# insitro/FastVim

Measured on AMD Instinct MI355X. Metric: images/sec FastVim-T 224px bs=128/GPU fwd+bwd (+all-reduce +AdamW +EMA), whole job, higher is better.
Workload: dtype bf16; 1 GPU; FastVim-T 224x224 bs=128/GPU bf16 training step, synthetic ImageNet tensors (BASELINE configs[1]); global_batch=128, parallelism=dp1, hip_graph=True, optimizer_in_step=True, final_loss_hex=0x1.779ca20000000p+0

## Files before the change

### fastvim_amd/_lib.py

```python
import ctypes
import os
import threading

import torch

_PKG = os.path.dirname(os.path.abspath(__file__))
LIB_PATH = os.path.join(_PKG, "libfastvim_hip.so")

FV_F32, FV_BF16, FV_F16 = 0, 1, 2
_DTYPES = {torch.float32: FV_F32, torch.bfloat16: FV_BF16, torch.float16: FV_F16}

_lib = None

C_ABI_SYMBOLS = (
    "fv_last_error", "fv_version",
    "fv_selective_scan_fwd", "fv_selective_scan_bwd_workspace", "fv_selective_scan_bwd",
    "fv_causal_conv1d_fwd", "fv_causal_conv1d_bwd", "fv_scan_expand_skip_fwd",
    "fv_mixer_conv_pool_fwd", "fv_mixer_scan_fwd", "fv_mixer_xproj_scan_fwd_ok", "fv_mixer_xproj_scan_fwd", "fv_mixer_combine_fwd",
    "fv_mixer_bwd_blocks", "fv_mixer_combine_bwd", "fv_mixer_scan_bwd_chunks", "fv_mixer_scan_bwd_chunks_b",
    "fv_mixer_scan_bwd_ckpt_floats", "fv_mixer_scan_bwd_partials", "fv_mixer_scan_bwd", "fv_mixer_scan_bwd_dir", "fv_mixer_scan_bwd_ckpt", "fv_mixer_scan_bwd_segments", "fv_mixer_scan_bwd_seg_floats", "fv_mixer_scan_bwd_seg_partials", "fv_mixer_scan_bwd_seg_chunks", "fv_mixer_scan_bwd_seg", "fv_mixer_scan_fwd_ckpt", "fv_mixer_scan_ckpt_floats", "fv_mixer_scan_fwd_segments", "fv_mixer_scan_fwd_seg_floats", "fv_mixer_scan_fwd_seg", "fv_rows_segment_sum", "fv_rows_gather", "fv_mixer_conv_pool_bwd", "fv_mixer_conv_pool_bwd2_ok", "fv_mixer_conv_pool_bwd2", "fv_mixer_scan_bwd_xproj_ok", "fv_mixer_scan_bwd_xproj", "fv_chunk_rows_bf16", "fv_reduce_partials", "fv_reduce_partials_multi",
    "fv_add_norm_blocks", "fv_add_norm_fwd", "fv_add_norm_bwd", "fv_gemm_bf16", "fv_gemm_bf16_tn_grouped", "fv_gemm_bf16_tn_grouped_ld", "fv_mixer_xproj_fwd", "fv_mixer_xproj_bwd_slices", "fv_mixer_xproj_bwd", "fv_mixer_xproj_bwd2", "fv_mixer_xproj_bwd3_ok", "fv_mixer_xproj_bwd3", "fv_adamw_flat", "fv_soft_target_ce",
    "fv_patch_unfold", "fv_gemm_bf16_rowbias", "fv_mean_pool_fwd", "fv_mean_pool_bwd", "fv_droppath_table", "fv_scale_cast",
    "fv_column_sum", "fv_gemm_bf16_addnorm", "fv_gemm_bf16_dgrad_addnorm_blocks", "fv_gemm_bf16_dgrad_addnorm_bwd", "fv_gemm_bf16_dgrad_addnorm_bwd2", "fv_gemm_bf16_addnorm2", "fv_mixer_combine_out_proj_addnorm_ok", "fv_mixer_combine_out_proj_addnorm", "fv_gemm_f32",
    "fv_mixer_conv_pool_bwd_dgrad_ok", "fv_mixer_conv_pool_bwd_dgrad_blocks", "fv_mixer_conv_pool_bwd_dgrad", "fv_transpose_bf16_batched", "fv_gemm_bf16_tn_grouped_wide8",
    "fv_grad_sumsq_blocks", "fv_grad_sumsq_partials", "fv_adamw_flat_groups",
)


_tls = threading.local()


class _DeviceGuarded:

    def __init__(self, cdll):
        self._cdll = cdll
        self._wrapped = {}

    def __getattr__(self, name):
        w = self._wrapped.get(name)
        if w is None:
            fn = getattr(self._cdll, name)

            def call(*args, _fn=fn):
                dev = getattr(_tls, "dev", None)
                if dev is None or dev == torch.cuda.current_device():
                    return _fn(*args)
                with torch.cuda.device(dev):
                    return _fn(*args)

            w = self._wrapped[name] = call
        return w


def lib():
    global _lib
    if _lib is None:
        if not os.path.exists(LIB_PATH):
            raise RuntimeError(
                f"{LIB_PATH} is missing: build it with `python -m fastvim_amd.build` "
                "(or __graft_entry__.build()). fastvim_amd has no CPU / eager fallback.")
        cdll = ctypes.CDLL(LIB_PATH)
        cdll.fv_last_error.restype = ctypes.c_char_p
        cdll.fv_selective_scan_bwd_workspace.restype = ctypes.c_size_t
        cdll.fv_mixer_scan_bwd_ckpt_floats.restype = ctypes.c_size_t
        cdll.fv_mixer_scan_ckpt_floats.restype = ctypes.c_size_t
        cdll.fv_mixer_scan_fwd_seg_floats.restype = ctypes.c_size_t
        cdll.fv_mixer_scan_bwd_seg_floats.restype = ctypes.c_size_t
        _lib = _DeviceGuarded(cdll)
    return _lib


def dtype_code(dt):
    try:
        return _DTYPES[dt]
    except KeyError:
        raise RuntimeError(f"fastvim_amd: unsupported dtype {dt}") from None


def ptr(t):
    return ctypes.c_void_p(0 if t is None else t.data_ptr())


def stream_of(t):
    _tls.dev = t.device.index
    return ctypes.c_void_p(torch.cuda.current_stream(t.device).cuda_stream)


def require_gpu(*tensors):
    for t in tensors:
        if t is not None and not t.is_cuda:
            raise RuntimeError("fastvim_amd ops run on the GPU only (HIP kernels); got a CPU tensor")


def check(rc, what):
    if rc != 0:
        msg = lib().fv_last_error().decode()
        raise RuntimeError(f"{what}: {msg} (code {rc})")


def i32(v):
    return ctypes.c_int(int(v))
```

### fastvim_amd/csrc/combine_gemm.hip

```cpp
#include "mixer_common.h"
#include "packed.h"

namespace {

typedef __bf16 cg_bf16x8 __attribute__((ext_vector_type(8)));
typedef float cg_f32x4 __attribute__((ext_vector_type(4)));

constexpr int CG_K = 384, CG_N = 192, CG_BM = 64, CG_NT = 256;
constexpr int CG_RSA = CG_K * 2 + 16;
constexpr int CG_RSB = CG_N * 2 + 16;
constexpr int CG_PD = 6;
constexpr int CG_KS = CG_K / 32;
#ifndef CG_DBG
#define CG_DBG 0
#endif

struct CgParams {
  const void* xz;
  const void* skip;
  const float* yc;
  const float *lnw, *lnb;
  void* g;
  float *mean, *rstd_ln;
  float ln_eps;
  Geo geo;
  int B;
  const bf16_t* W;
  long ldw;
  const float* residual;
  const float* nw;
  const float* row_scale;
  int rows_per_scale;
  float* res_out;
  bf16_t* y;
  float* rstd;
  float eps;
  int M;
  int d_in;
};

__device__ __forceinline__ float cg_hsum(f2 v) { return v.x + v.y; }

__global__ __launch_bounds__(CG_NT, 2) void combine_out_proj_addnorm_kernel(CgParams p) {
  extern __shared__ __attribute__((aligned(16))) char smem[];
  typedef PairVec<bf16_t, 3> P;
  const int tid = threadIdx.x, lane = tid & 63;
  const int wv = __builtin_amdgcn_readfirstlane(tid >> 6);
  const Geo g = p.geo;
  const int tiles = (g.rows + 3) / 4;
  const int bimg = blockIdx.x / tiles, i0 = (blockIdx.x - bimg * tiles) * 4;
  const int mimg = bimg * g.L;
  auto tok_of = [&](int rl) {
    const int w = rl >> 4, j = rl & 15;
    return (i0 + w < g.rows && j < g.cols) ? mimg + (i0 + w) * g.s_i + j * g.s_j : -1;
  };

  const int lr = lane % 16, gr = lane / 16;
  const int fn = lane & 15, fk = lane >> 4;
  const bf16_t* wrow[3];
  cg_bf16x8 fb[CG_PD][3];
  float4 ne_r[2][2][3], ne_w[3];
  float ne_sc[2][2];
  {
#pragma clang fp reassociate(off) contract(off)
    const int lc = lane * 6, voff = lc * 2;
    const int tok_x = 2 * CG_K * 2, tok_s = CG_K * 2;
    const bool has_ln = p.lnw != nullptr;
    const float inv_d = 1.f / (float)p.d_in;
    const size_t ydir = (size_t)p.B * g.rows * CG_K;
    const __amdgpu_buffer_rsrc_t bz = fv_make_buf((const bf16_t*)p.xz + CG_K, (size_t)p.M * tok_x - tok_s);
    const __amdgpu_buffer_rsrc_t bs = fv_make_buf(p.skip, (size_t)p.M * tok_s);
    const __amdgpu_buffer_rsrc_t bg = fv_make_buf(p.g, (size_t)p.M * tok_s);
    const __amdgpu_buffer_rsrc_t bmean = fv_make_buf(has_ln ? (const void*)p.mean : p.g, has_ln ? (size_t)p.M * 4 : 0);
    const __amdgpu_buffer_rsrc_t brstd = fv_make_buf(has_ln ? (const void*)p.rstd_ln : p.g, has_ln ? (size_t)p.M * 4 : 0);
    const int irow = i0 + wv;
    const bool wlive = irow < g.rows;
    const int irc = wlive ? irow : g.rows - 1;
    const int mbase = mimg + irc * g.s_i;
    char* arow = smem + (wv * 16) * CG_RSA + lane * 12;
    constexpr int TT = 2;
    const int npair = (g.cols + TT - 1) / TT;
    f2 ysum[3], ysf[3], ysb[3];
    {
      const float* yr = p.yc + ((size_t)bimg * g.rows + irc) * CG_K + lc;
#pragma unroll
      for (int q = 0; q < 3; ++q) {
        ysf[q] = *reinterpret_cast<const f2*>(yr + 2 * q);
        ysb[q] = *reinterpret_cast<const f2*>(yr + ydir + 2 * q);
      }
    }
    struct Pre { P sk[TT], z[TT]; };
    Pre pa, pb;
    auto fetch = [&](Pre& r, int j0) {
#pragma unroll
      for (int t = 0; t < TT; ++t) {
        const int m = mbase + min(j0 + t, g.cols - 1) * g.s_j;
        r.sk[t].load(bs, voff, m * tok_s);
        r.z[t].load(bz, voff, m * tok_x);
      }
    };
    fetch(pa, 0);
    fetch(pb, TT);
    __builtin_amdgcn_sched_barrier(0);
    f2 lw[3], lb[3];
    {
      const float* lwp = has_ln ? p.lnw : p.yc;
      const float* lbp = has_ln ? p.lnb : p.yc;
#pragma unroll
      for (int q = 0; q < 3; ++q) {
        lw[q] = *reinterpret_cast<const f2*>(lwp + lc + 2 * q);
        lb[q] = *reinterpret_cast<const f2*>(lbp + lc + 2 * q);
      }
    }
    __builtin_amdgcn_sched_barrier(0);
#pragma unroll
    for (int nb = 0; nb < 3; ++nb) wrow[nb] = p.W + (long)(wv * 48 + nb * 16 + fn) * p.ldw + fk * 8;
#pragma unroll
    for (int s = 0; s < CG_PD; s += 2)
#pragma unroll
      for (int nb = 0; nb < 3; ++nb)
#pragma unroll
        for (int h = 0; h < 2; ++h) fb[s + h][nb] = *reinterpret_cast<const cg_bf16x8*>(wrow[nb] + (s + h) * 32);
    __builtin_amdgcn_sched_barrier(0);
#pragma unroll
    for (int q = 0; q < 3; ++q) ysum[q] = ysf[q] + ysb[q];
    auto process = [&](Pre& r, int j0) {
      f2 o[TT][3], z[TT][3];
      float s1[TT], mean[TT], rstd[TT];
#pragma unroll
      for (int t = 0; t < TT; ++t)
#pragma unroll
        for (int q = 0; q < 3; ++q) {
          o[t][q] = r.sk[t].get(q);
          z[t][q] = r.z[t].get(q);
        }
      fetch(r, j0 + 2 * TT);
      __builtin_amdgcn_sched_barrier(0);
#pragma unroll
      for (int t = 0; t < TT; ++t) {
        f2 acc = splat(0.f);
#pragma unroll
        for (int q = 0; q < 3; ++q) {
          o[t][q] = (ysum[q] + o[t][q]) * 0.5f;
          acc += o[t][q];
        }
        s1[t] = cg_hsum(acc);
      }
      if (has_ln) {
#pragma unroll
        for (int t = 0; t < TT; ++t) s1[t] = wave_sum_uniform(s1[t]);
#pragma unroll
        for (int t = 0; t < TT; ++t) {
          mean[t] = s1[t] * inv_d;
          f2 acc = splat(0.f);
#pragma unroll
          for (int q = 0; q < 3; ++q) {
            const f2 d = o[t][q] - mean[t];
            acc = fma2(d, d, acc);
          }
          s1[t] = cg_hsum(acc);
        }
#pragma unroll
        for (int t = 0; t < TT; ++t) s1[t] = wave_sum_uniform(s1[t]);
#pragma unroll
        for (int t = 0; t < TT; ++t) rstd[t] = rsqrtf(s1[t] * inv_d + p.ln_eps);
      } else {
#pragma unroll
        for (int t = 0; t < TT; ++t) { mean[t] = 0.f; rstd[t] = 1.f; }
      }
#pragma unroll
      for (int t = 0; t < TT; ++t) {
        const bool live = wlive && j0 + t < g.cols;
        const int m = mbase + min(j0 + t, g.cols - 1) * g.s_j;
        f2 out[3];
#pragma unroll
        for (int q = 0; q < 3; ++q) {
          const f2 w_ = has_ln ? lw[q] : splat(1.f), b_ = has_ln ? lb[q] : splat(0.f);
          out[q] = fma2((o[t][q] - mean[t]) * rstd[t], w_, b_) * silu2(z[t][q]);
        }
        uint32_t pk[3];
#pragma unroll
        for (int q = 0; q < 3; ++q) pk[q] = live ? pack_bf16x2(out[q].x, out[q].y) : 0u;
        if (CG_DBG != 4) {
          fv_buf_store_words<3>(bg, live ? voff : 0x7ffffff0, m * tok_s, pk);
          const int so = (has_ln && live && lane == 0) ? 0 : 0x7ffffff0;
          const uint32_t mv[1] = {__float_as_uint(mean[t])}, rv[1] = {__float_as_uint(rstd[t])};
          fv_buf_store_words<1>(bmean, so, m * 4, mv);
          fv_buf_store_words<1>(brstd, so, m * 4, rv);
        }
        uint32_t* ar = reinterpret_cast<uint32_t*>(arow + (j0 + t) * CG_RSA);
        ar[0] = pk[0]; ar[1] = pk[1]; ar[2] = pk[2];
      }
    };
#pragma unroll 1
    for (int pr = 0; pr < (CG_DBG == 1 ? 0 : 8); pr += 2) {
      process(pa, pr * TT);
      process(pb, (pr + 1) * TT);
    }
    (void)npair;
#pragma unroll
    for (int it = 0; it < 2; ++it)
#pragma unroll
      for (int u = 0; u < 2; ++u) {
        const int m = tok_of(wv * 16 + it * 8 + u * 4 + gr), rowc = m >= 0 ? m : mimg;
#pragma unroll
        for (int k = 0; k < 3; ++k)
          ne_r[it][u][k] = *reinterpret_cast<const float4*>(p.residual + (size_t)rowc * CG_N + (k * 16 + lr) * 4);
        ne_sc[it][u] = (p.row_scale ? p.row_scale : p.nw)[p.row_scale ? rowc / p.rows_per_scale : 0];
      }
#pragma unroll
    for (int k = 0; k < 3; ++k) ne_w[k] = *reinterpret_cast<const float4*>(p.nw + (k * 16 + lr) * 4);
    __builtin_amdgcn_sched_barrier(0);
  }
  __syncthreads();

  cg_f32x4 acc[3][4];
#pragma unroll
  for (int a = 0; a < 3; ++a)
#pragma unroll
    for (int b = 0; b < 4; ++b) acc[a][b] = (cg_f32x4){0.f, 0.f, 0.f, 0.f};
  const char* afrag = smem + (lane & 15) * CG_RSA + (lane >> 4) * 16;
  static_assert(CG_PD % 2 == 0 && CG_KS % 2 == 0, "the weight ring is refilled in line pairs");
#pragma unroll
  for (int kp = 0; kp < (CG_DBG == 2 ? 0 : CG_KS); kp += 2) {
    cg_bf16x8 cur[2][3];
#pragma unroll
    for (int h = 0; h < 2; ++h)
#pragma unroll
      for (int nb = 0; nb < 3; ++nb) cur[h][nb] = fb[(kp + h) % CG_PD][nb];
    if (kp + CG_PD < CG_KS) {
#pragma unroll
      for (int nb = 0; nb < 3; ++nb)
#pragma unroll
        for (int h = 0; h < 2; ++h)
          fb[(kp + h) % CG_PD][nb] = *reinterpret_cast<const cg_bf16x8*>(wrow[nb] + (kp + h + CG_PD) * 32);
    }
    __builtin_amdgcn_sched_barrier(0);
#pragma unroll
    for (int h = 0; h < 2; ++h) {
      cg_bf16x8 fa[4];
#pragma unroll
      for (int mb = 0; mb < 4; ++mb) fa[mb] = *reinterpret_cast<const cg_bf16x8*>(afrag + mb * 16 * CG_RSA + (kp + h) * 64);
#pragma unroll
      for (int a = 0; a < 3; ++a)
#pragma unroll
        for (int b = 0; b < 4; ++b) acc[a][b] = __builtin_amdgcn_mfma_f32_16x16x32_bf16(cur[h][a], fa[b], acc[a][b], 0, 0, 0);
    }
    __builtin_amdgcn_sched_barrier(0);
  }
  __syncthreads();

#pragma unroll
  for (int b = 0; b < 4; ++b)
#pragma unroll
    for (int a = 0; a < 3; ++a) {
      const cg_f32x4 v = acc[a][b];
      uint2 pk = {pack_bf16x2(v[0], v[1]), pack_bf16x2(v[2], v[3])};
      *reinterpret_cast<uint2*>(smem + (b * 16 + (lane & 15)) * CG_RSB + (wv * 48 + a * 16 + (lane >> 4) * 4) * 2) = pk;
    }
  __syncthreads();
  if (CG_DBG == 3) return;
  constexpr int LPR = 16, RPW = 4, RU = 2, RW = CG_BM / 4;
  const float inv_n = 1.f / (float)CG_N;
  float w[3][4];
#pragma unroll
  for (int k = 0; k < 3; ++k) {
    const float4 t = ne_w[k];
    w[k][0] = t.x; w[k][1] = t.y; w[k][2] = t.z; w[k][3] = t.w;
  }
#pragma unroll
  for (int it = 0; it < RW / (RPW * RU); ++it) {
    float v[RU][3][4], r[RU][3][4], sc_u[RU];
#pragma unroll
    for (int u = 0; u < RU; ++u) {
      const int rl = wv * RW + it * (RPW * RU) + u * RPW + gr;
      sc_u[u] = p.row_scale ? ne_sc[it][u] : 1.f;
#pragma unroll
      for (int k = 0; k < 3; ++k) {
        const int c = (k * LPR + lr) * 4;
        const uint2 xb = *reinterpret_cast<const uint2*>(smem + rl * CG_RSB + c * 2);
        v[u][k][0] = __uint_as_float(xb.x << 16); v[u][k][1] = __uint_as_float(xb.x & 0xffff0000u);
        v[u][k][2] = __uint_as_float(xb.y << 16); v[u][k][3] = __uint_as_float(xb.y & 0xffff0000u);
        const float4 t = ne_r[it][u][k];
        r[u][k][0] = t.x; r[u][k][1] = t.y; r[u][k][2] = t.z; r[u][k][3] = t.w;
      }
    }
#pragma unroll
    for (int u = 0; u < RU; ++u) {
      const int row = tok_of(wv * RW + it * (RPW * RU) + u * RPW + gr);
      const bool live = row >= 0;
      const size_t base = (size_t)(live ? row : mimg) * CG_N;
      const float sc = sc_u[u];
#pragma unroll
      for (int k = 0; k < 3; ++k) {
        const int c = (k * LPR + lr) * 4;
#pragma unroll
        for (int e = 0; e < 4; ++e) v[u][k][e] = fmaf(v[u][k][e], sc, r[u][k][e]);
        if (live) *reinterpret_cast<float4*>(p.res_out + base + c) = make_float4(v[u][k][0], v[u][k][1], v[u][k][2], v[u][k][3]);
      }
      float q = 0.f;
#pragma unroll
      for (int k = 0; k < 3; ++k)
#pragma unroll
        for (int e = 0; e < 4; ++e) q = fmaf(v[u][k][e], v[u][k][e], q);
#define FV_DPP_ADD(ctrl) q += __int_as_float(__builtin_amdgcn_update_dpp(0, __float_as_int(q), ctrl, 0xf, 0xf, true))
      FV_DPP_ADD(0xB1);
      FV_DPP_ADD(0x4E);
      FV_DPP_ADD(0x141);
      FV_DPP_ADD(0x140);
#undef FV_DPP_ADD
      const float rstd = rsqrtf(q * inv_n + p.eps);
      if (lr == 0 && live) p.rstd[row] = rstd;
#pragma unroll
      for (int k = 0; k < 3; ++k) {
        const int c = (k * LPR + lr) * 4;
        float o[4];
#pragma unroll
        for (int e = 0; e < 4; ++e) {
          float t = v[u][k][e] * rstd;
          asm volatile("" : "+v"(t));
          o[e] = t * w[k][e];
        }
        uint2 pk = {pack_bf16x2(o[0], o[1]), pack_bf16x2(o[2], o[3])};
        if (live) *reinterpret_cast<uint2*>(p.y + base + c) = pk;
      }
    }
  }
}

}

extern "C" int fv_mixer_combine_out_proj_addnorm_ok(int batch, int rows, int cols, int tokens_per_patch, int d_inner,
                                                    int d_model, int dtype) {
  return dtype == FV_BF16 && d_inner == CG_K && d_model == CG_N && tokens_per_patch == 1 && batch > 0 && rows > 0 &&
         cols > 0 && cols <= 16 && (long)batch * rows * cols * CG_K * 4 < 0x7fffffffL;
}

extern "C" int fv_mixer_combine_out_proj_addnorm(const void* xz, const void* skip, const float* yc, const float* ln_w,
                                                 const float* ln_b, float ln_eps, void* g, float* mean, float* rstd_ln,
                                                 int batch, int rows, int cols, int tok_stride_row, int tok_stride_col,
                                                 const void* W, long ldw, const float* residual,
                                                 const float* norm_weight, const float* row_scale, int rows_per_scale,
                                                 void* y, float* residual_out, float* rstd, float eps,
                                                 fv_stream_t stream) {
  FV_CHECK(xz && skip && yc && g && W && residual && norm_weight && y && residual_out && rstd,
           "mixer_combine_out_proj_addnorm: null pointer");
  FV_CHECK(!ln_w || (ln_b && mean && rstd_ln), "mixer_combine_out_proj_addnorm: LayerNorm needs weight, bias, mean, rstd");
  FV_CHECK(fv_mixer_combine_out_proj_addnorm_ok(batch, rows, cols, 1, CG_K, CG_N, FV_BF16),
           "mixer_combine_out_proj_addnorm: shape not built (fv_mixer_combine_out_proj_addnorm_ok)");
  FV_CHECK((tok_stride_row == cols && tok_stride_col == 1) || (tok_stride_row == 1 && tok_stride_col == rows),
           "mixer_combine_out_proj_addnorm: token strides (%d,%d) are neither row-major nor transposed for a %dx%d grid",
           tok_stride_row, tok_stride_col, rows, cols);
  FV_CHECK(((uintptr_t)W & 15) == 0 && ldw % 8 == 0 && ldw >= CG_K, "mixer_combine_out_proj_addnorm: weight rows must be 16-byte aligned");
  FV_CHECK(((uintptr_t)residual & 15) == 0 && ((uintptr_t)residual_out & 15) == 0 && ((uintptr_t)y & 7) == 0 &&
               ((uintptr_t)norm_weight & 15) == 0, "mixer_combine_out_proj_addnorm: row operands must be 16-byte aligned");
  FV_CHECK(!row_scale || rows_per_scale > 0, "mixer_combine_out_proj_addnorm: rows_per_scale must be positive");
  CgParams p{};
  p.xz = xz; p.skip = skip; p.yc = yc; p.lnw = ln_w; p.lnb = ln_b; p.g = g; p.mean = mean; p.rstd_ln = rstd_ln;
  p.ln_eps = ln_eps;
  p.geo = make_geo(rows, cols, tok_stride_row, tok_stride_col, 1);
  p.B = batch;
  p.W = (const bf16_t*)W; p.ldw = ldw; p.residual = residual; p.nw = norm_weight; p.row_scale = row_scale;
  p.rows_per_scale = rows_per_scale; p.res_out = residual_out; p.y = (bf16_t*)y; p.rstd = rstd; p.eps = eps;
  p.M = batch * rows * cols;
  p.d_in = CG_K;
  const size_t smem = (size_t)CG_BM * CG_RSA;
  hipLaunchKernelGGL(combine_out_proj_addnorm_kernel, dim3(batch * fv_cdiv(rows, 4)), dim3(CG_NT), smem, (hipStream_t)stream, p);
  FV_LAUNCH_CHECK();
  return FV_OK;
}
```

### fastvim_amd/csrc/convpool_dgrad.hip

```cpp
#include "mixer_common.h"
#include "packed.h"
#include "gemm_tiles.h"

namespace {

constexpr int CD_DI = 384, CD_N = 192, CD_K = 2 * CD_DI, CD_BM = 64, CD_NT = 256, CD_NCH = CD_DI / 128;
constexpr int CD_RSA = CD_DI * 2 + 16;
constexpr int CD_RSB = CD_N * 2 + 16;
#ifndef CD_PDEPTH
#define CD_PDEPTH 4
#endif
#ifndef CD_SB_EVERY
#define CD_SB_EVERY 1
#endif
#ifndef CD_W2_PIPE
#define CD_W2_PIPE 1
#endif
constexpr int CD_PD = CD_PDEPTH;
constexpr int CD_KS = CD_K / 32;
constexpr int CD_ZST = CD_BM * BK * 2;
constexpr int CD_NZ = CD_DI / BK;
constexpr int CD_O_RING = CD_BM * CD_RSA;
constexpr int CD_SLOT = 12 * 128;
constexpr int CD_O_B = (CD_BM * CD_RSB + 255) / 256 * 256, CD_O_S = CD_O_B + 2 * 128 * BK * 2;
constexpr int CD_SMEM = CD_O_S + 4 * 32 * (64 * 2 + 16);
static_assert(CD_O_RING + 3 * CD_ZST <= CD_SMEM && CD_O_RING + 4 * CD_SLOT * 4 <= CD_SMEM, "LDS regions");
static_assert(2 * CD_SMEM <= 160 * 1024, "two workgroups per CU");
#ifndef CD_DBG
#define CD_DBG 0
#endif

struct CdParams {
  const void* xz;
  const void* dob;
  const float* dxc;
  const void* dxc2;
  const float *wf, *bf, *wb, *bb, *Df, *Db;
  void* dxz;
  float* part;
  float pool_scale;
  Geo geo;
  int B;
  const bf16_t* Wt;
  long ldwt;
  const float* dres_out;
  const float* r;
  const float* rstd;
  const float* nw;
  const float* row_scale;
  int rows_per_scale;
  bf16_t* dx;
  float* dres_in;
  float* pw;
  const bf16_t* W2;
  long ldw2;
  bf16_t* C2;
  int N2;
  int M;
};

__device__ __forceinline__ void cd_dma16(const void* base, uint32_t voff, uint32_t lds_dst) {
  asm volatile("s_mov_b32 m0, %2\n\ts_nop 0\n\tglobal_load_lds_dwordx4 %0, %1" ::"v"(voff), "s"(base), "s"(lds_dst) : "memory");
}

constexpr int cd_younger(int t) {
  constexpr int KX = CD_DI / 32;
  int n = 0;
  for (int q = KX + 2 * (t - 3) + 2; q < KX + 2 * t; q += 2) n += (q + CD_PD < CD_KS ? 6 : 0) + ((q - KX) / 2 + 3 < CD_NZ ? 2 : 0);
  return n;
}
static_assert(cd_younger(3) < 64 && cd_younger(4) < 64 && cd_younger(5) < 64, "vmcnt is a 6-bit counter");

template <int NT, bool X2>
__global__ __launch_bounds__(CD_NT, 2) void conv_pool_bwd_dgrad_kernel(CdParams p) {
  extern __shared__ __attribute__((aligned(16))) char smem[];
  typedef PairVec<bf16_t, 1> P;
  const int tid = threadIdx.x, lane = tid & 63;
  const int wv = __builtin_amdgcn_readfirstlane(tid >> 6);
  const Geo g = p.geo;
  const int tiles = (g.rows + 3) / 4;
  const int bimg = blockIdx.x / tiles, i0 = (blockIdx.x - bimg * tiles) * 4;
  const int mimg = bimg * g.L;
  auto tok_of = [&](int rl) {
    const int w = rl >> 4, j = rl & 15;
    return (i0 + w < g.rows && j < g.cols) ? mimg + (i0 + w) * g.s_i + j * g.s_j : -1;
  };
  const int irow = i0 + wv;
  const bool wlive = irow < g.rows;
  char* prow = smem + (wv * 16) * CD_RSA;

  {
    const int zr0 = wlive ? NT : 0;
    for (int e = lane; e < (16 - zr0) * (CD_RSA / 4); e += 64) reinterpret_cast<uint32_t*>(prow + zr0 * CD_RSA)[e] = 0u;
    const int tok_x = 2 * CD_DI * 2, tok_d = CD_DI * 2;
    const size_t dstride = (size_t)p.B * g.rows * CD_DI;
    const __amdgpu_buffer_rsrc_t bp = fv_make_buf(p.dxc, 2 * dstride * 4);
    const __amdgpu_buffer_rsrc_t bp2 = fv_make_buf(X2 ? p.dxc2 : p.dxc, X2 ? 2 * dstride * 2 : 0);
    const int irc = wlive ? irow : 0;
    const bool up = irc > 0, down = irc + 1 < g.rows;
    const int m_row = irc * g.s_i, s_up = up ? -g.s_i : 0, s_dn = down ? g.s_i : 0;
    const int pooled_off = (bimg * g.rows + irc) * CD_DI;
    const size_t img_x = (size_t)bimg * g.L * 2 * CD_DI, img_d = (size_t)bimg * g.L * CD_DI;
    const __amdgpu_buffer_rsrc_t bx = fv_make_buf((const bf16_t*)p.xz + img_x, wlive ? (size_t)g.L * tok_x : 0);
    const __amdgpu_buffer_rsrc_t bd = fv_make_buf((const bf16_t*)p.dob + img_d, wlive ? (size_t)g.L * tok_d : 0);
    const __amdgpu_buffer_rsrc_t bo = fv_make_buf((bf16_t*)p.dxz + img_x, wlive ? (size_t)g.L * tok_x : 0);
    struct Pooled {
      f2 a;
      P b;
      __device__ __forceinline__ f2 sum() const { if constexpr (X2) return a + b.get(0); else return a; }
    };
    auto pooled = [&](int r, bool backward, int c0, bool on) {
      const bool ok = r == 1 || (r == 0 ? up : down);
      uint32_t w[2];
      const int eoff = pooled_off + (ok ? (r - 1) * CD_DI : 0) + (backward ? (int)dstride : 0);
      const int lane_off = on ? c0 : 0x1ffffff0;
      fv_buf_load_words<2>(bp, lane_off * 4, eoff * 4, w);
      Pooled o;
      o.a.x = __uint_as_float(w[0]);
      o.a.y = __uint_as_float(w[1]);
      if constexpr (X2) o.b.load(bp2, lane_off * 2, eoff * 2);
      return o;
    };
    P xr[NT + 6], dr[NT + 6];
    auto fetch = [&](int k, int voff) {
      const int di = k < 3 ? -1 : (k >= NT + 3 ? 1 : 0);
      const int j = k - 3 - di * NT;
      const int m = m_row + (di < 0 ? s_up : di > 0 ? s_dn : 0) + j * g.s_j;
      xr[k].load(bx, voff, m * tok_x);
      dr[k].load(bd, voff, m * tok_d);
    };
    struct Prm { f2 wf[CW], wb[CW], bf, bb, Df, Db; };
    auto load_prm = [&](int c0) {
      Prm q;
      load_taps2(p.wf, c0, q.wf);
      load_taps2(p.wb, c0, q.wb);
      q.bf = load_f2(p.bf ? p.bf : p.wf, c0);
      q.bb = load_f2(p.bb ? p.bb : p.wf, c0);
      q.Df = load_f2(p.Df ? p.Df : p.wf, c0);
      q.Db = load_f2(p.Db ? p.Db : p.wf, c0);
      return q;
    };
    Prm pn = load_prm(lane * 2);
    __builtin_amdgcn_sched_barrier(0);
    Pooled cf_mid_raw = pooled(1, false, lane * 2, true), cb_mid_raw = pooled(1, true, lane * 2, true);
    Pooled cb_up_raw = pooled(0, true, lane * 2, true);
    __builtin_amdgcn_sched_barrier(0);
#pragma unroll
    for (int k = 0; k < NT + 6; ++k) fetch(k, lane * 4);
    __builtin_amdgcn_sched_barrier(0);
    Pooled cf_dn_raw = pooled(2, false, lane * 2, true);
    __builtin_amdgcn_sched_barrier(0);
    float* slot = reinterpret_cast<float*>(smem + CD_O_RING) + wv * CD_SLOT;
#pragma unroll 1
    for (int c = 0; c < CD_NCH; ++c) {
      const int c0 = c * 128 + lane * 2;
      const int voff = c0 * 2;
      const bool more = c + 1 < CD_NCH;
      const int c0n = c0 + 128, voffn = more ? voff + 256 : 0x3ffffff0;
      f2 a_wf[CW], a_wb[CW], a_bf = splat(0.f), a_bb = splat(0.f), a_Df = splat(0.f), a_Db = splat(0.f);
#pragma unroll
      for (int k = 0; k < CW; ++k) a_wf[k] = a_wb[k] = splat(0.f);
      if (wlive && CD_DBG != 1) {
        f2 wf[CW], wb[CW];
#pragma unroll
        for (int k = 0; k < CW; ++k) { wf[k] = pn.wf[k]; wb[k] = pn.wb[k]; }
        const f2 bf = pn.bf * (p.bf ? 1.f : 0.f), bb = pn.bb * (p.bb ? 1.f : 0.f);
        const f2 Dfh = pn.Df * (p.Df ? 0.5f : 0.f), Dbh = pn.Db * (p.Db ? 0.5f : 0.f);
        const f2 cf_mid = cf_mid_raw.sum() * p.pool_scale, cb_mid = cb_mid_raw.sum() * p.pool_scale;
        cf_mid_raw = pooled(1, false, c0n, more);
        cb_mid_raw = pooled(1, true, c0n, more);
        const f2 cb_up = cb_up_raw.sum() * (up ? p.pool_scale : 0.f);
        f2 cf_dn = splat(0.f);
        f2 x[NT + 6], dov[NT + 6], dpf[NT + 6], dpb[NT + 6];
        const float m_up = up ? 1.f : 0.f, m_dn = down ? 1.f : 0.f;
#pragma unroll
        for (int k = 0; k < 3; ++k) {
          x[k] = xr[k].get(0) * m_up;
          dov[k] = dr[k].get(0);
          dpf[k] = dpb[k] = splat(0.f);
          fetch(k, voffn);
        }
        if (more) pn = load_prm(c0n);
#pragma unroll
        for (int n = -3; n < NT; ++n) {
          const int q3 = n + 3, k0 = n + 3, k3 = n + 6;
          x[k3] = xr[k3].get(0);
          if (q3 >= NT) x[k3] *= m_dn;
          dov[k3] = dr[k3].get(0);
          fetch(k3, voffn);
          f2 pf = bf, pb = bb;
#pragma unroll
          for (int k = 0; k < CW; ++k) {
            pf = fma2(wf[k], x[k0 + k], pf);
            pb = fma2(wb[k], x[k3 - k], pb);
          }
          const f2 sgf = sigmoid2(pf), sgb = sigmoid2(pb);
          const f2 dsf = sgf * fma2(pf, 1.f - sgf, splat(1.f)), dsb = sgb * fma2(pb, 1.f - sgb, splat(1.f));
          const float e3 = q3 < NT ? 1.f : m_dn, e0 = n >= 0 ? 1.f : m_up;
          if (q3 == NT) cf_dn = cf_dn_raw.sum() * (down ? p.pool_scale : 0.f);
          const f2 nf = fma2(Dfh, dov[k3], q3 >= NT ? cf_dn : cf_mid) * dsf * e3;
          const f2 nb = fma2(Dbh, dov[k0], n < 0 ? cb_up : cb_mid) * dsb * e0;
          if (n == -1) cb_up_raw = pooled(0, true, c0n, more);
          dpf[k3] = nf;
          dpb[k0] = nb;
          if (q3 < NT) {
#pragma unroll
            for (int k = 0; k < CW; ++k) a_wf[k] = fma2(nf, x[k0 + k], a_wf[k]);
            a_bf += nf;
            a_Df = fma2(dov[k3], pf * sgf, a_Df);
          }
          if (n >= 0) {
#pragma unroll
            for (int k = 0; k < CW; ++k) a_wb[k] = fma2(nb, x[k3 - k], a_wb[k]);
            a_bb += nb;
            a_Db = fma2(dov[k0], pb * sgb, a_Db);
            f2 dx = splat(0.f);
#pragma unroll
            for (int k = 0; k < CW; ++k) {
              dx = fma2(wf[k], dpf[k3 - k], dx);
              dx = fma2(wb[k], dpb[k0 - 3 + k], dx);
            }
            const uint32_t pk[1] = {pack_bf16x2(dx.x, dx.y)};
            fv_buf_store_words<1>(bo, voff, (m_row + n * g.s_j) * tok_x, pk);
            *reinterpret_cast<uint32_t*>(prow + n * CD_RSA + voff) = pk[0];
          }
          if ((n + 3) % CD_SB_EVERY == CD_SB_EVERY - 1) __builtin_amdgcn_sched_barrier(0);
        }
        cf_dn_raw = pooled(2, false, c0n, more);
      }
      {
        const f2 hDf = a_Df * 0.5f, hDb = a_Db * 0.5f;
        float4* s4 = reinterpret_cast<float4*>(slot);
        s4[2 * lane] = make_float4(a_wf[0].x, a_wf[1].x, a_wf[2].x, a_wf[3].x);
        s4[2 * lane + 1] = make_float4(a_wf[0].y, a_wf[1].y, a_wf[2].y, a_wf[3].y);
        s4[128 + 2 * lane] = make_float4(a_wb[0].x, a_wb[1].x, a_wb[2].x, a_wb[3].x);
        s4[128 + 2 * lane + 1] = make_float4(a_wb[0].y, a_wb[1].y, a_wb[2].y, a_wb[3].y);
        f2* s2 = reinterpret_cast<f2*>(slot + 1024);
        s2[lane] = a_bf;
        s2[64 + lane] = a_bb;
        s2[128 + lane] = hDf;
        s2[192 + lane] = hDb;
      }
      __syncthreads();
      {
        const float* s0 = reinterpret_cast<const float*>(smem + CD_O_RING);
        float* dst = p.part + (size_t)blockIdx.x * 12 * CD_DI;
#pragma unroll
        for (int i = 0; i < CD_SLOT / CD_NT; ++i) {
          const int e = tid + i * CD_NT;
          const float v = ((s0[e] + s0[CD_SLOT + e]) + s0[2 * CD_SLOT + e]) + s0[3 * CD_SLOT + e];
          int gi;
          if (e < 512) gi = c * 512 + e;
          else if (e < 1024) gi = 4 * CD_DI + c * 512 + (e - 512);
          else {
            const int q = (e - 1024) >> 7, rr = (e - 1024) & 127;
            gi = (8 + q) * CD_DI + c * 128 + rr;
          }
          dst[gi] = v;
        }
      }
      __syncthreads();
    }
  }

  const int fn = lane & 15, fk = lane >> 4, lr = lane % 16, gr = lane / 16;
  const bf16_t* wrow[3];
  bf16x8 fb[CD_PD][3];
#pragma unroll
  for (int nb = 0; nb < 3; ++nb) wrow[nb] = p.Wt + (long)(wv * 48 + nb * 16 + fn) * p.ldwt + fk * 8;
  uint32_t zoff[2];
  const uint32_t ring = (uint32_t)(uintptr_t)(__attribute__((address_space(3))) const char*)(smem + CD_O_RING);
#pragma unroll
  for (int i = 0; i < 2; ++i) {
    const int e = tid + i * CD_NT, rrow = e >> 3, ch = (e & 7) ^ (rrow & 7);
    const int m = tok_of(rrow);
    zoff[i] = (uint32_t)((m >= 0 ? m : mimg) * (CD_K * 2) + (CD_DI + ch * 8) * 2);
  }
  auto issue_z = [&](int t) {
#pragma unroll
    for (int i = 0; i < 2; ++i)
      cd_dma16(p.dxz, zoff[i] + (uint32_t)t * (BK * 2), ring + (uint32_t)(t % 3) * CD_ZST + (uint32_t)(i * CD_NT + wv * 64) * 16);
  };
  issue_z(0);
  issue_z(1);
  issue_z(2);
#pragma unroll
  for (int s = 0; s < CD_PD; s += 2)
#pragma unroll
    for (int nb = 0; nb < 3; ++nb)
#pragma unroll
      for (int h = 0; h < 2; ++h) fb[s + h][nb] = *reinterpret_cast<const bf16x8*>(wrow[nb] + (s + h) * 32);
  __builtin_amdgcn_sched_barrier(0);
  float4 ne_r[2][2][3];
#pragma unroll
  for (int it = 0; it < 2; ++it)
#pragma unroll
    for (int u = 0; u < 2; ++u) {
      const int m = tok_of(wv * 16 + it * 8 + u * 4 + gr), rowc = m >= 0 ? m : mimg;
#pragma unroll
      for (int k = 0; k < 3; ++k) ne_r[it][u][k] = *reinterpret_cast<const float4*>(p.r + (size_t)rowc * CD_N + (k * 16 + lr) * 4);
    }
  __builtin_amdgcn_sched_barrier(0);
  __syncthreads();

  f32x4 acc[3][4];
#pragma unroll
  for (int a = 0; a < 3; ++a)
#pragma unroll
    for (int b = 0; b < 4; ++b) acc[a][b] = (f32x4){0.f, 0.f, 0.f, 0.f};
  const char* afrag = smem + (lane & 15) * CD_RSA + (lane >> 4) * 16;
  static_assert(CD_PD % 2 == 0 && CD_KS % 2 == 0, "the weight ring is refilled in line pairs");
  static_for<(CD_DBG == 2 ? 0 : CD_KS / 2)>([&](auto kp_c) {
    constexpr int kp = 2 * decltype(kp_c)::value;
    constexpr int KX = CD_DI / 32;
    if constexpr (kp >= KX) {
      constexpr int t = (kp - KX) / 2;
      if constexpr (t >= 3) asm volatile("s_waitcnt vmcnt(%0)" ::"n"(cd_younger(t)) : "memory");
      if (t >= 3 || kp == KX) __builtin_amdgcn_s_barrier();
    }
    bf16x8 cur[2][3];
#pragma unroll
    for (int h = 0; h < 2; ++h)
#pragma unroll
      for (int nb = 0; nb < 3; ++nb) cur[h][nb] = fb[(kp + h) % CD_PD][nb];
    if constexpr (kp + CD_PD < CD_KS) {
#pragma unroll
      for (int nb = 0; nb < 3; ++nb)
#pragma unroll
        for (int h = 0; h < 2; ++h)
          fb[(kp + h) % CD_PD][nb] = *reinterpret_cast<const bf16x8*>(wrow[nb] + (kp + h + CD_PD) * 32);
    }
    __builtin_amdgcn_sched_barrier(0);
#pragma unroll
    for (int h = 0; h < 2; ++h) {
      bf16x8 fa[4];
      if constexpr (kp < KX) {
#pragma unroll
        for (int mb = 0; mb < 4; ++mb) fa[mb] = *reinterpret_cast<const bf16x8*>(afrag + mb * 16 * CD_RSA + (kp + h) * 64);
      } else {
        constexpr int t = (kp - KX) / 2;
        const char* st = smem + CD_O_RING + (t % 3) * CD_ZST;
#pragma unroll
        for (int mb = 0; mb < 4; ++mb) fa[mb] = frag<KC, CD_BM>(st, mb, h, lane);
      }
#pragma unroll
      for (int a = 0; a < 3; ++a)
#pragma unroll
        for (int b = 0; b < 4; ++b) acc[a][b] = __builtin_amdgcn_mfma_f32_16x16x32_bf16(cur[h][a], fa[b], acc[a][b], 0, 0, 0);
    }
    if constexpr (kp >= KX) {
      constexpr int t = (kp - KX) / 2;
      if constexpr (t + 3 < CD_NZ) {
        __builtin_amdgcn_s_barrier();
        issue_z(t + 3);
      }
    }
    __builtin_amdgcn_sched_barrier(0);
  });
  float4 ne_g[2][2][3];
#pragma unroll
  for (int it = 0; it < 2; ++it)
#pragma unroll
    for (int u = 0; u < 2; ++u) {
      const int m = tok_of(wv * 16 + it * 8 + u * 4 + gr), rowc = m >= 0 ? m : mimg;
#pragma unroll
      for (int k = 0; k < 3; ++k)
        ne_g[it][u][k] = p.dres_out ? *reinterpret_cast<const float4*>(p.dres_out + (size_t)rowc * CD_N + (k * 16 + lr) * 4)
                                    : make_float4(0.f, 0.f, 0.f, 0.f);
    }
  __syncthreads();

#pragma unroll
  for (int b = 0; b < 4; ++b)
#pragma unroll
    for (int a = 0; a < 3; ++a) {
      const f32x4 v = acc[a][b];
      uint2 pk = {pack_bf16x2(v[0], v[1]), pack_bf16x2(v[2], v[3])};
      *reinterpret_cast<uint2*>(smem + (b * 16 + (lane & 15)) * CD_RSB + (wv * 48 + a * 16 + (lane >> 4) * 4) * 2) = pk;
    }
  __syncthreads();
  if (CD_DBG == 3) return;
  {
    constexpr int LPR = 16, RPW = 4, RU = 2, RW = CD_BM / 4;
    const float inv_n = 1.f / (float)CD_N;
    float w[3][4], aw[3][4];
#pragma unroll
    for (int k = 0; k < 3; ++k) {
      const float4 t = *reinterpret_cast<const float4*>(p.nw + (k * LPR + lr) * 4);
      w[k][0] = t.x; w[k][1] = t.y; w[k][2] = t.z; w[k][3] = t.w;
#pragma unroll
      for (int e = 0; e < 4; ++e) aw[k][e] = 0.f;
    }
#pragma unroll
    for (int it = 0; it < RW / (RPW * RU); ++it) {
#pragma unroll
      for (int u = 0; u < RU; ++u) {
        const int rl = wv * RW + it * (RPW * RU) + u * RPW + gr;
        const int row = tok_of(rl);
        const bool live = row >= 0;
        const int rowc = live ? row : mimg;
        const size_t base = (size_t)rowc * CD_N;
        const float rstd = p.rstd[rowc];
        const float sc = p.row_scale ? p.row_scale[rowc / p.rows_per_scale] : 1.f;
        const float lv = live ? 1.f : 0.f;
        float xh[3][4], dxh[3][4];
        float c2 = 0.f;
#pragma unroll
        for (int k = 0; k < 3; ++k) {
          const int c = (k * LPR + lr) * 4;
          const uint2 xb = *reinterpret_cast<const uint2*>(smem + rl * CD_RSB + c * 2);
          const float dyv[4] = {__uint_as_float(xb.x << 16), __uint_as_float(xb.x & 0xffff0000u),
                                __uint_as_float(xb.y << 16), __uint_as_float(xb.y & 0xffff0000u)};
          const float4 rr4 = ne_r[it][u][k];
          const float rr[4] = {rr4.x, rr4.y, rr4.z, rr4.w};
#pragma unroll
          for (int e = 0; e < 4; ++e) {
            const float dyl = dyv[e] * lv;
            xh[k][e] = (rr[e] - 0.f) * rstd;
            dxh[k][e] = dyl * w[k][e];
            aw[k][e] = fmaf(dyl, xh[k][e], aw[k][e]);
            c2 = fmaf(dxh[k][e], xh[k][e], c2);
          }
        }
#define FV_DPP_ADD(ctrl) c2 += __int_as_float(__builtin_amdgcn_update_dpp(0, __float_as_int(c2), ctrl, 0xf, 0xf, true))
        FV_DPP_ADD(0xB1);
        FV_DPP_ADD(0x4E);
        FV_DPP_ADD(0x141);
        FV_DPP_ADD(0x140);
#undef FV_DPP_ADD
        c2 = c2 * inv_n;
        const float c1 = 0.f;
#pragma unroll
        for (int k = 0; k < 3; ++k) {
          const int c = (k * LPR + lr) * 4;
          const float4 g4 = ne_g[it][u][k];
          const float gg[4] = {g4.x, g4.y, g4.z, g4.w};
          float dr[4];
#pragma unroll
          for (int e = 0; e < 4; ++e) dr[e] = rstd * (dxh[k][e] - c1 - xh[k][e] * c2) + gg[e];
          if (live) {
            *reinterpret_cast<float4*>(p.dres_in + base + c) = make_float4(dr[0], dr[1], dr[2], dr[3]);
            if (p.row_scale)
#pragma unroll
              for (int e = 0; e < 4; ++e) dr[e] *= sc;
            uint2 pk = {pack_bf16x2(dr[0], dr[1]), pack_bf16x2(dr[2], dr[3])};
            *reinterpret_cast<uint2*>(p.dx + base + c) = pk;
            *reinterpret_cast<uint2*>(smem + rl * CD_RSB + c * 2) = pk;
          } else {
            *reinterpret_cast<uint2*>(smem + rl * CD_RSB + c * 2) = make_uint2(0u, 0u);
          }
        }
      }
    }
    __syncthreads();
    float* s_acc = reinterpret_cast<float*>(smem + CD_BM * CD_RSB);
#pragma unroll
    for (int k = 0; k < 3; ++k)
#pragma unroll
      for (int e = 0; e < 4; ++e) {
        float v = aw[k][e];
        auto r1 = __builtin_amdgcn_permlane16_swap(__float_as_uint(v), __float_as_uint(v), false, false);
        v = __uint_as_float(r1[0]) + __uint_as_float(r1[1]);
        auto r2 = __builtin_amdgcn_permlane32_swap(__float_as_uint(v), __float_as_uint(v), false, false);
        v = __uint_as_float(r2[0]) + __uint_as_float(r2[1]);
        if (gr == 0) s_acc[wv * CD_N + (k * LPR + lr) * 4 + e] = v;
      }
    __syncthreads();
    float* dst = p.pw + (size_t)blockIdx.x * CD_N;
    for (int c = tid; c < CD_N; c += CD_NT) dst[c] = (s_acc[c] + s_acc[CD_N + c]) + (s_acc[2 * CD_N + c] + s_acc[3 * CD_N + c]);
  }
  if (p.W2 && CD_DBG != 4) {
    __syncthreads();
    tile_times_w2_rows<CD_BM, CD_RSB, KS, decltype(tok_of), CD_W2_PIPE != 0>(smem, smem + CD_O_B, smem + CD_O_S, p.W2, p.ldw2, p.N2,
                                                                              p.C2, tok_of, tid);
  }
}

}

extern "C" int fv_mixer_conv_pool_bwd_dgrad_ok(int batch, int rows, int cols, int tokens_per_patch, int d_inner, int d_model,
                                               int pool_max, int dtype) {
  return dtype == FV_BF16 && d_inner == CD_DI && d_model == CD_N && tokens_per_patch == 1 && !pool_max && batch > 0 &&
         rows > 0 && (cols == 14 || cols == 16) &&
         (long)batch * rows * cols * CD_K * 2 < 0x7fffffffL &&
         (long)batch * rows * CD_DI * 8 < 0x7ffff000L;
}

extern "C" int fv_mixer_conv_pool_bwd_dgrad_blocks(int batch, int rows) { return batch * fv_cdiv(rows, 4); }

extern "C" int fv_mixer_conv_pool_bwd_dgrad(
    const void* xz, const void* dskip, const float* dxc, const void* dxc2, const float* conv_w, const float* conv_b,
    const float* conv_w_b, const float* conv_b_b, const float* D, const float* D_b, void* dxz, float* conv_partials, int batch,
    int rows, int cols, int tok_stride_row, int tok_stride_col, float scaling, const void* W_in_t, long ldwt,
    const float* dresidual_out, const float* r, const float* rstd, const float* norm_weight, const float* row_scale,
    int rows_per_scale, void* dx, float* dresidual_in, float* partial_dw, const void* W2, void* C2, int N2, long ldw2,
    fv_stream_t stream) {
  FV_CHECK(xz && dskip && dxc && conv_w && conv_w_b && dxz && conv_partials && W_in_t && r && rstd && norm_weight && dx &&
               dresidual_in && partial_dw, "mixer_conv_pool_bwd_dgrad: null pointer");
  FV_CHECK(fv_mixer_conv_pool_bwd_dgrad_ok(batch, rows, cols, 1, CD_DI, CD_N, 0, FV_BF16),
           "mixer_conv_pool_bwd_dgrad: shape not built (fv_mixer_conv_pool_bwd_dgrad_ok)");
  FV_CHECK((tok_stride_row == cols && tok_stride_col == 1) || (tok_stride_row == 1 && tok_stride_col == rows),
           "mixer_conv_pool_bwd_dgrad: token strides (%d,%d) are neither row-major nor transposed for a %dx%d grid",
           tok_stride_row, tok_stride_col, rows, cols);
  FV_CHECK(((uintptr_t)W_in_t & 15) == 0 && ldwt % 8 == 0 && ldwt >= CD_K, "mixer_conv_pool_bwd_dgrad: transposed weight rows must be 16-byte aligned");
  FV_CHECK(((uintptr_t)r & 15) == 0 && ((uintptr_t)dresidual_in & 15) == 0 && ((uintptr_t)dx & 7) == 0 &&
               ((uintptr_t)norm_weight & 15) == 0 && ((uintptr_t)dresidual_out & 15) == 0 && ((uintptr_t)dxz & 15) == 0,
           "mixer_conv_pool_bwd_dgrad: row operands must be 16-byte aligned");
  FV_CHECK(!row_scale || rows_per_scale > 0, "mixer_conv_pool_bwd_dgrad: rows_per_scale must be positive");
  FV_CHECK(!W2 || (C2 && N2 > 0 && N2 % 128 == 0 && ldw2 % 8 == 0 && ldw2 >= N2 && ((uintptr_t)W2 & 15) == 0 && ((uintptr_t)C2 & 15) == 0),
           "mixer_conv_pool_bwd_dgrad: the second weight must be (192, N2) with N2 a multiple of 128, 16-byte aligned");
  CdParams p{};
  p.xz = xz; p.dob = dskip; p.dxc = dxc; p.dxc2 = dxc2; p.wf = conv_w; p.bf = conv_b; p.wb = conv_w_b; p.bb = conv_b_b;
  p.Df = D; p.Db = D_b; p.dxz = dxz; p.part = conv_partials;
  p.pool_scale = scaling / (float)cols;
  p.geo = make_geo(rows, cols, tok_stride_row, tok_stride_col, 1);
  p.B = batch;
  p.Wt = (const bf16_t*)W_in_t; p.ldwt = ldwt; p.dres_out = dresidual_out; p.r = r; p.rstd = rstd; p.nw = norm_weight;
  p.row_scale = row_scale; p.rows_per_scale = rows_per_scale > 0 ? rows_per_scale : 1; p.dx = (bf16_t*)dx;
  p.dres_in = dresidual_in; p.pw = partial_dw; p.W2 = (const bf16_t*)W2; p.ldw2 = ldw2; p.C2 = (bf16_t*)C2; p.N2 = N2;
  p.M = batch * rows * cols;
  const dim3 grid(batch * fv_cdiv(rows, 4)), block(CD_NT);
#define FV_CD(NTT, XX)                                                                                              \
  do {                                                                                                              \
    static FvOncePerDevice done;                                                                                    \
    if (done.first())                                                                                               \
      (void)hipFuncSetAttribute((const void*)conv_pool_bwd_dgrad_kernel<NTT, XX>, hipFuncAttributeMaxDynamicSharedMemorySize, CD_SMEM); \
    hipLaunchKernelGGL((conv_pool_bwd_dgrad_kernel<NTT, XX>), grid, block, CD_SMEM, (hipStream_t)stream, p);        \
  } while (0)
  if (cols == 14) { if (dxc2) FV_CD(14, true); else FV_CD(14, false); }
  else { if (dxc2) FV_CD(16, true); else FV_CD(16, false); }
#undef FV_CD
  FV_LAUNCH_CHECK();
  return FV_OK;
}
```

### fastvim_amd/csrc/glue.hip

```cpp
#include "common.h"

namespace {

typedef uint32_t u32x4 __attribute__((ext_vector_type(4)));
typedef uint32_t u32x2 __attribute__((ext_vector_type(2)));

template <typename T> struct Vec4;
template <> struct Vec4<float> {
  static __device__ __forceinline__ void ld(const float* p, float (&v)[4]) {
    const float4 t = *reinterpret_cast<const float4*>(p);
    v[0] = t.x; v[1] = t.y; v[2] = t.z; v[3] = t.w;
  }
  static __device__ __forceinline__ void st(float* p, const float (&v)[4]) {
    *reinterpret_cast<float4*>(p) = make_float4(v[0], v[1], v[2], v[3]);
  }
};
template <> struct Vec4<bf16_t> {
  static __device__ __forceinline__ void ld(const bf16_t* p, float (&v)[4]) {
    const u32x2 t = *reinterpret_cast<const u32x2*>(p);
    v[0] = __uint_as_float(t.x << 16); v[1] = __uint_as_float(t.x & 0xffff0000u);
    v[2] = __uint_as_float(t.y << 16); v[3] = __uint_as_float(t.y & 0xffff0000u);
  }
  static __device__ __forceinline__ void st(bf16_t* p, const float (&v)[4]) {
    u32x2 t;
    t.x = pack_bf16x2(v[0], v[1]);
    t.y = pack_bf16x2(v[2], v[3]);
    *reinterpret_cast<u32x2*>(p) = t;
  }
};

constexpr int UNF_GJ = 16;

template <typename TI, typename TO>
__global__ __launch_bounds__(256) void patch_unfold_kernel(const TI* __restrict__ img, TO* __restrict__ out, int C, int H,
                                                           int W, int ph, int pw, int gw) {
  extern __shared__ __attribute__((aligned(16))) char smem[];
  TO* tile = reinterpret_cast<TO*>(smem);
  const int gj0 = blockIdx.x * UNF_GJ, gi = blockIdx.y, b = blockIdx.z;
  const int gjn = min(UNF_GJ, gw - gj0);
  const int Kp = C * ph * pw;
  const int xv = gjn * pw / 4;
  const TI* src = img + ((size_t)b * C * H + (size_t)gi * ph) * W + (size_t)gj0 * pw;
  for (int e = threadIdx.x; e < C * ph * xv; e += blockDim.x) {
    const int row = e / xv, x = (e - row * xv) * 4;
    const int c = row / ph, pi = row - c * ph;
    float v[4];
    Vec4<TI>::ld(src + ((size_t)c * H + pi) * W + x, v);
    const int gj = x / pw, pj = x - gj * pw;
    Vec4<TO>::st(tile + (size_t)gj * Kp + row * pw + pj, v);
  }
  __syncthreads();
  TO* dst = out + (((size_t)b * gridDim.y + gi) * gw + gj0) * Kp;
  constexpr int EV = 16 / sizeof(TO);
  const int nv = gjn * Kp / EV;
  for (int e = threadIdx.x; e < nv; e += blockDim.x)
    reinterpret_cast<u32x4*>(dst)[e] = reinterpret_cast<const u32x4*>(tile)[e];
}

constexpr int MP_WAVES = 16;
template <typename T>
__global__ __launch_bounds__(64 * MP_WAVES) void mean_pool_fwd_kernel(const T* __restrict__ x, T* __restrict__ out, int L, int D, float inv) {
  __shared__ float s_acc[MP_WAVES][256];
  const int lane = threadIdx.x & 63, wv = threadIdx.x >> 6;
  const int d = (blockIdx.x * 64 + lane) * 4, b = blockIdx.y;
  float a[4] = {0.f, 0.f, 0.f, 0.f};
  if (d < D) {
    const T* xp = x + (size_t)b * L * D + d;
    int l = wv;
    for (; l + 3 * MP_WAVES < L; l += 4 * MP_WAVES) {
      float v[4][4];
#pragma unroll
      for (int u = 0; u < 4; ++u) Vec4<T>::ld(xp + (size_t)(l + u * MP_WAVES) * D, v[u]);
#pragma unroll
      for (int u = 0; u < 4; ++u)
#pragma unroll
        for (int k = 0; k < 4; ++k) a[k] += v[u][k];
    }
    for (; l < L; l += MP_WAVES) {
      float v[4];
      Vec4<T>::ld(xp + (size_t)l * D, v);
#pragma unroll
      for (int k = 0; k < 4; ++k) a[k] += v[k];
    }
  }
#pragma unroll
  for (int k = 0; k < 4; ++k) s_acc[wv][lane * 4 + k] = a[k];
  __syncthreads();
  if (wv == 0 && d < D) {
    float r[4];
#pragma unroll
    for (int k = 0; k < 4; ++k) {
      float t = 0.f;
#pragma unroll
      for (int w = 0; w < MP_WAVES; ++w) t += s_acc[w][lane * 4 + k];
      r[k] = t * inv;
    }
    Vec4<T>::st(out + (size_t)b * D + d, r);
  }
}

template <typename T>
__global__ __launch_bounds__(256) void mean_pool_bwd_kernel(const T* __restrict__ g, T* __restrict__ dx, int L, int D,
                                                            int rows_per_block, float inv) {
  const int b = blockIdx.y, dv = D / 4;
  const int l0 = blockIdx.x * rows_per_block, l1 = min(L, l0 + rows_per_block);
  for (int e = threadIdx.x; e < (l1 - l0) * dv; e += blockDim.x) {
    const int l = l0 + e / dv, d = (e % dv) * 4;
    float v[4];
    Vec4<T>::ld(g + (size_t)b * D + d, v);
#pragma unroll
    for (int k = 0; k < 4; ++k) v[k] *= inv;
    Vec4<T>::st(dx + ((size_t)b * L + l) * D + d, v);
  }
}

__global__ __launch_bounds__(256) void droppath_table_kernel(float* __restrict__ table, const float* __restrict__ keep,
                                                             const float* __restrict__ inv, int mods, int batch) {
  const int i = blockIdx.x * blockDim.x + threadIdx.x;
  if (i < mods * batch) {
    const int m = i / batch;
    table[i] = floorf(table[i] + keep[m]) * inv[m];
  }
}

template <typename T>
__global__ __launch_bounds__(256) void scale_cast_kernel(const float* __restrict__ x, const float* __restrict__ scale,
                                                         T* __restrict__ y, size_t n) {
  const float s = scale[0];
  for (size_t i = (size_t)blockIdx.x * blockDim.x + threadIdx.x; i < n; i += (size_t)gridDim.x * blockDim.x)
    io<T>::st(y + i, x[i] * s);
}

template <typename T>
__global__ __launch_bounds__(256) void column_sum_kernel(const T* __restrict__ x, float* __restrict__ out, int rows, int cols,
                                                         int accumulate) {
  __shared__ float s_acc[4][64];
  const int lane = threadIdx.x & 63, wv = threadIdx.x >> 6, c = blockIdx.x * 64 + lane;
  float a = 0.f;
  if (c < cols)
    for (int r = wv; r < rows; r += 4) a += io<T>::ld(x + (size_t)r * cols + c);
  s_acc[wv][lane] = a;
  __syncthreads();
  if (wv == 0 && c < cols) {
    const float t = (s_acc[0][lane] + s_acc[1][lane]) + (s_acc[2][lane] + s_acc[3][lane]);
    out[c] = accumulate ? out[c] + t : t;
  }
}

bool dt_ok(int dt) { return dt == FV_F32 || dt == FV_BF16; }


constexpr int TRJ_MAX = 64;
struct TransposeJobs {
  const uint16_t* src[TRJ_MAX];
  uint16_t* dst[TRJ_MAX];
  int rows, cols;
};
__global__ __launch_bounds__(256) void transpose_bf16_kernel(TransposeJobs J) {
  __shared__ uint16_t t[32][33];
  const uint16_t* src = J.src[blockIdx.z];
  uint16_t* dst = J.dst[blockIdx.z];
  const int r0 = blockIdx.y * 32, c0 = blockIdx.x * 32, tx = threadIdx.x & 31, ty = threadIdx.x >> 5;
#pragma unroll
  for (int i = 0; i < 4; ++i) {
    const int r = r0 + ty + 8 * i, c = c0 + tx;
    t[ty + 8 * i][tx] = (r < J.rows && c < J.cols) ? src[(size_t)r * J.cols + c] : (uint16_t)0;
  }
  __syncthreads();
#pragma unroll
  for (int i = 0; i < 4; ++i) {
    const int c = c0 + ty + 8 * i, r = r0 + tx;
    if (r < J.rows && c < J.cols) dst[(size_t)c * J.rows + r] = t[tx][ty + 8 * i];
  }
}

}

extern "C" int fv_patch_unfold(const void* img, int img_dtype, void* out, int out_dtype, int batch, int chans, int height,
                               int width, int ph, int pw, fv_stream_t stream) {
  FV_CHECK(img && out, "patch_unfold: null pointer");
  FV_CHECK(dt_ok(img_dtype) && dt_ok(out_dtype), "patch_unfold: dtypes must be fp32 or bf16");
  FV_CHECK(batch > 0 && chans > 0 && ph > 0 && pw > 0 && height >= ph && width >= pw, "patch_unfold: empty dimension");
  FV_CHECK(height % ph == 0 && width % pw == 0, "patch_unfold: image %dx%d is not whole %dx%d patches", height, width, ph, pw);
  FV_CHECK(pw % 8 == 0 && ((uintptr_t)img & 15) == 0 && ((uintptr_t)out & 15) == 0,
           "patch_unfold: patch width must be a multiple of 8 and the buffers 16-byte aligned");
  const int gh = height / ph, gw = width / pw;
  const size_t osz = out_dtype == FV_F32 ? 4 : 2;
  const size_t smem = (size_t)UNF_GJ * chans * ph * pw * osz;
  FV_CHECK(smem <= 64 * 1024, "patch_unfold: %d x %d x %d patches do not fit the staging tile", chans, ph, pw);
  FV_CHECK(gh <= 65535 && batch <= 65535, "patch_unfold: grid too large");
  const dim3 grid(fv_cdiv(gw, UNF_GJ), gh, batch), block(256);
  hipStream_t st = (hipStream_t)stream;
#define FV_UNF(TI, TO) hipLaunchKernelGGL((patch_unfold_kernel<TI, TO>), grid, block, smem, st, (const TI*)img, (TO*)out, chans, height, width, ph, pw, gw)
  if (img_dtype == FV_F32 && out_dtype == FV_BF16) FV_UNF(float, bf16_t);
  else if (img_dtype == FV_F32) FV_UNF(float, float);
  else if (out_dtype == FV_BF16) FV_UNF(bf16_t, bf16_t);
  else FV_UNF(bf16_t, float);
#undef FV_UNF
  FV_LAUNCH_CHECK();
  return FV_OK;
}

extern "C" int fv_mean_pool_fwd(const void* x, void* out, int batch, int tokens, int dim, int dtype, fv_stream_t stream) {
  FV_CHECK(x && out, "mean_pool_fwd: null pointer");
  FV_CHECK(dt_ok(dtype), "mean_pool_fwd: dtype must be fp32 or bf16");
  FV_CHECK(batch > 0 && tokens > 0 && dim > 0 && dim % 4 == 0 && batch <= 65535, "mean_pool_fwd: bad shape (%d, %d, %d)", batch, tokens, dim);
  const dim3 grid(fv_cdiv(dim, 256), batch), block(64 * MP_WAVES);
  hipStream_t st = (hipStream_t)stream;
  const float inv = 1.f / (float)tokens;
  if (dtype == FV_F32) hipLaunchKernelGGL(mean_pool_fwd_kernel<float>, grid, block, 0, st, (const float*)x, (float*)out, tokens, dim, inv);
  else hipLaunchKernelGGL(mean_pool_fwd_kernel<bf16_t>, grid, block, 0, st, (const bf16_t*)x, (bf16_t*)out, tokens, dim, inv);
  FV_LAUNCH_CHECK();
  return FV_OK;
}

extern "C" int fv_mean_pool_bwd(const void* g, void* dx, int batch, int tokens, int dim, int dtype, fv_stream_t stream) {
  FV_CHECK(g && dx, "mean_pool_bwd: null pointer");
  FV_CHECK(dt_ok(dtype), "mean_pool_bwd: dtype must be fp32 or bf16");
  FV_CHECK(batch > 0 && tokens > 0 && dim > 0 && dim % 4 == 0 && batch <= 65535, "mean_pool_bwd: bad shape (%d, %d, %d)", batch, tokens, dim);
  const int rpb = fv_cdiv(tokens, 8);
  const dim3 grid(fv_cdiv(tokens, rpb), batch), block(256);
  hipStream_t st = (hipStream_t)stream;
  const float inv = 1.f / (float)tokens;
  if (dtype == FV_F32) hipLaunchKernelGGL(mean_pool_bwd_kernel<float>, grid, block, 0, st, (const float*)g, (float*)dx, tokens, dim, rpb, inv);
  else hipLaunchKernelGGL(mean_pool_bwd_kernel<bf16_t>, grid, block, 0, st, (const bf16_t*)g, (bf16_t*)dx, tokens, dim, rpb, inv);
  FV_LAUNCH_CHECK();
  return FV_OK;
}

extern "C" int fv_droppath_table(float* table, const float* keep, const float* inv_keep, int mods, int batch, fv_stream_t stream) {
  FV_CHECK(table && keep && inv_keep && mods > 0 && batch > 0, "droppath_table: bad arguments");
  hipLaunchKernelGGL(droppath_table_kernel, dim3(fv_cdiv((long)mods * batch, 256)), dim3(256), 0, (hipStream_t)stream, table, keep,
                     inv_keep, mods, batch);
  FV_LAUNCH_CHECK();
  return FV_OK;
}

extern "C" int fv_scale_cast(const float* x, const float* scale, void* y, int y_dtype, size_t n, fv_stream_t stream) {
  FV_CHECK(x && scale && y && n > 0, "scale_cast: bad arguments");
  FV_CHECK(dt_ok(y_dtype), "scale_cast: output must be fp32 or bf16");
  const dim3 grid(fv_cdiv((long)n, 256) < 2048 ? fv_cdiv((long)n, 256) : 2048), block(256);
  hipStream_t st = (hipStream_t)stream;
  if (y_dtype == FV_F32) hipLaunchKernelGGL(scale_cast_kernel<float>, grid, block, 0, st, x, scale, (float*)y, n);
  else hipLaunchKernelGGL(scale_cast_kernel<bf16_t>, grid, block, 0, st, x, scale, (bf16_t*)y, n);
  FV_LAUNCH_CHECK();
  return FV_OK;
}

extern "C" int fv_column_sum(const void* x, int dtype, float* out, int rows, int cols, int accumulate, fv_stream_t stream) {
  FV_CHECK(x && out && rows > 0 && cols > 0, "column_sum: bad arguments");
  FV_CHECK(dt_ok(dtype), "column_sum: input must be fp32 or bf16");
  const dim3 grid(fv_cdiv(cols, 64)), block(256);
  hipStream_t st = (hipStream_t)stream;
  if (dtype == FV_F32) hipLaunchKernelGGL(column_sum_kernel<float>, grid, block, 0, st, (const float*)x, out, rows, cols, accumulate);
  else hipLaunchKernelGGL(column_sum_kernel<bf16_t>, grid, block, 0, st, (const bf16_t*)x, out, rows, cols, accumulate);
  FV_LAUNCH_CHECK();
  return FV_OK;
}

extern "C" int fv_transpose_bf16_batched(const void* const* srcs, void* const* dsts, int njobs, int rows, int cols,
                                         fv_stream_t stream) {
  FV_CHECK(srcs && dsts && njobs > 0 && njobs <= TRJ_MAX, "transpose_bf16_batched: 1..%d jobs", TRJ_MAX);
  FV_CHECK(rows > 0 && cols > 0 && fv_cdiv(rows, 32) <= 65535, "transpose_bf16_batched: bad shape (%d, %d)", rows, cols);
  TransposeJobs J{};
  for (int j = 0; j < njobs; ++j) {
    FV_CHECK(srcs[j] && dsts[j], "transpose_bf16_batched: null pointer in job %d", j);
    J.src[j] = (const uint16_t*)srcs[j];
    J.dst[j] = (uint16_t*)dsts[j];
  }
  J.rows = rows; J.cols = cols;
  hipLaunchKernelGGL(transpose_bf16_kernel, dim3(fv_cdiv(cols, 32), fv_cdiv(rows, 32), njobs), dim3(256), 0, (hipStream_t)stream, J);
  FV_LAUNCH_CHECK();
  return FV_OK;
}
```

### fastvim_amd/flat.py

```python
import ctypes
import os
import re
import warnings

import torch
import torch.distributed as dist

from . import _lib as L
from .layernorm import RMSNorm
from .mamba_simple_faster import Mamba, _GroupedWgrad, _SideStream, flush_wgrads, group_wgrads
from .mixer_ops import defer_reductions, drop_reductions, flush_reductions, pending_reductions

_LAYER_RE = re.compile(r"^((?:.*\.)?[A-Za-z_]*layers\.\d+)\.")

_MIXER_GROUPS = (
    ("conv", ("conv1d.weight", "conv1d_b.weight", "conv1d.bias", "conv1d_b.bias", "D", "D_b")),
    ("scan", ("A_log", "dt_proj.weight", "dt_proj.bias", "A_b_log", "dt_proj_b.weight", "dt_proj_b.bias")),
    ("ln", ("layernorm.weight", "layernorm.bias")),
    ("xproj", ("x_proj.weight", "x_proj_b.weight")),
)


class FlatTrainingState:
    def __init__(self, model, shadow_dtype=torch.bfloat16, process_group=None, comm_dtype=None,
                 chunk_bytes=256 << 20):
        self.group = process_group
        self.comm_dtype = comm_dtype
        self.chunk = max(1, chunk_bytes // 4)
        named = dict(model.named_parameters())
        mixers = {mname: mod for mname, mod in model.named_modules() if isinstance(mod, Mamba)}
        units, unit_of = [], {}
        for n, p in named.items():
            if not p.requires_grad:
                continue
            m_ = _LAYER_RE.match(n)
            key = m_.group(1) if m_ else None
            if key is None:
                if not units or units[-1][0] is not None:
                    units.append((None, []))
                units[-1][1].append(n)
            else:
                if key not in unit_of:
                    unit_of[key] = len(units)
                    units.append((key, []))
                units[unit_of[key]][1].append(n)
        order, regions = [], []
        self.units = []
        for key, names in units:
            front = []
            for mname, mod in mixers.items():
                if key is not None and (mname + ".").startswith(key + "."):
                    for gname, keys in _MIXER_GROUPS:
                        full = [f"{mname}.{k}" if mname else k for k in keys]
                        if all(f in named and named[f].requires_grad for f in full):
                            regions.append((mod, gname, full))
                            front += full
            rest = [n for n in names if n not in set(front)]
            self.units.append((key, len(order), len(order) + len(front) + len(rest)))
            order += front + rest
        if not any(k is not None for k, _ in units):
            for mname, mod in mixers.items():
                for gname, keys in _MIXER_GROUPS:
                    full = [f"{mname}.{k}" if mname else k for k in keys]
                    if all(f in named and named[f].requires_grad for f in full):
                        regions.append((mod, gname, full))
            front = [f for _, _, full in regions for f in full]
            order = front + [n for n in order if n not in set(front)]
            self.units = [(None, 0, len(order))]
        self.names = order
        params = [named[n] for n in order]
        dev = params[0].device
        offs, off = [], 0
        for p in params:
            offs.append(off)
            off += (p.numel() + 7) // 8 * 8
        self.param_flat = torch.zeros(off, device=dev, dtype=torch.float32)
        self.grad_flat = torch.zeros(off, device=dev, dtype=torch.float32)
        self.shadow_flat = torch.zeros(off, device=dev, dtype=shadow_dtype)
        self.offsets = dict(zip(order, offs))
        total = off
        self.unit_ranges = [(key, offs[i0] if i0 < len(offs) else total, offs[i1] if i1 < len(offs) else total)
                            for key, i0, i1 in self.units if i1 > i0]
        with torch.no_grad():
            for n, p, o in zip(order, params, offs):
                k = p.numel()
                self.param_flat[o:o + k].copy_(p.detach().reshape(-1))
                p.data = self.param_flat[o:o + k].view_as(p)
                p.grad = self.grad_flat[o:o + k].view_as(p)
                p._fv_shadow = self.shadow_flat[o:o + k].view_as(p)
                p._fv_shadow_version = -1
        self._params = params
        for mod, gname, full in regions:
            lo = self.offsets[full[0]]
            last = named[full[-1]]
            hi = self.offsets[full[-1]] + last.numel()
            contiguous = all(self.offsets[a] + named[a].numel() == self.offsets[b]
                             for a, b in zip(full[:-1], full[1:]))
            if not contiguous:
                continue
            fv = mod.__dict__.setdefault("_fv", {})
            fv[gname + "_grad"] = self.grad_flat[lo:hi]
            if gname == "xproj":
                shp = (2,) + tuple(named[full[0]].shape)
                fv["Wx2"] = self.param_flat[lo:hi].view(shp)
                fv["Wx2_shadow"] = self.shadow_flat[lo:hi].view(shp)
                fv["Wx2_grad"] = self.grad_flat[lo:hi].view(shp)
        for mod in model.modules():
            if isinstance(mod, (RMSNorm, torch.nn.LayerNorm, torch.nn.Linear, torch.nn.Conv2d)) and getattr(mod, "weight", None) is not None:
                if mod.weight.requires_grad:
                    mod.weight._fv_direct = True
                b = getattr(mod, "bias", None)
                if isinstance(mod, (torch.nn.Linear, torch.nn.Conv2d)) and b is not None and b.requires_grad:
                    b._fv_direct = True
        pe = getattr(model, "pos_embed", None)
        if isinstance(pe, torch.nn.Parameter) and pe.requires_grad:
            pe._fv_direct = True
        self._t_src, self._t_dst, self._t_params = [], [], []
        if shadow_dtype == torch.bfloat16 and dev.type == "cuda":
            for mod in mixers.values():
                w = mod.in_proj.weight
                if tuple(w.shape) == (768, 192) and w.requires_grad and getattr(w, "_fv_shadow", None) is not None:
                    wt = torch.empty(192, 768, device=dev, dtype=shadow_dtype)
                    w._fv_shadow_t = wt
                    w._fv_shadow_t_version = -1
                    self._t_src.append(w._fv_shadow)
                    self._t_dst.append(wt)
                    self._t_params.append(w)
        self._tx_src, self._tx_dst, self._tx_params = [], [], []
        if shadow_dtype == torch.bfloat16 and dev.type == "cuda":
            for mod in mixers.values():
                fv = mod.__dict__.get("_fv", {})
                ws = fv.get("Wx2_shadow")
                if ws is None or ws.dtype != torch.bfloat16:
                    continue
                _, Wd, d_in = ws.shape
                if d_in >= 768 and d_in % 64 == 0 and Wd % 8 == 0:
                    wt = torch.empty(2, d_in, Wd, device=dev, dtype=shadow_dtype)
                    fv["Wx2_shadow_t"] = wt
                    fv["Wx2_t_params"] = (mod.x_proj.weight, mod.x_proj_b.weight)
                    for k in range(2):
                        self._tx_src.append(ws[k])
                        self._tx_dst.append(wt[k])
                    for w in fv["Wx2_t_params"]:
                        w._fv_shadow_t_version = -1
                        self._tx_params.append(w)
        self.refresh_shadow()
        self._hook = model.register_load_state_dict_post_hook(lambda module, incompatible: self.refresh_shadow())
        from .mixer_ops import _Deferred
        self._saved_switches = (_Deferred.enabled, _GroupedWgrad.enabled, _SideStream.enabled)
        defer_reductions(True)
        group_wgrads(True)
        _SideStream.enabled = False

    def close(self):
        if self._saved_switches is None:
            return
        self.finish_backward()
        d, g, s_ = self._saved_switches
        defer_reductions(d)
        group_wgrads(g)
        _SideStream.enabled = s_
        self._hook.remove()
        self._saved_switches = None

    def __enter__(self):
        return self

    def __exit__(self, *exc):
        self.close()
        return False

    def zero_grad(self):
        _SideStream.join()
        n = len(_GroupedWgrad.jobs) + len(_GroupedWgrad.sums) + pending_reductions()
        if n:
            _GroupedWgrad.jobs = []
            _GroupedWgrad.sums = []
            _GroupedWgrad.rows_jobs = []
            drop_reductions()
            warnings.warn(f"FlatTrainingState.zero_grad(): {n} queued gradient jobs of an unfinished backward pass "
                          "were discarded -- call finish_backward() (or allreduce_mean_() / optimizer.step()) after "
                          "loss.backward()", RuntimeWarning, stacklevel=2)
        self.grad_flat.zero_()

    def finish_backward(self):
        flush_wgrads()
        flush_reductions()

    def refresh_shadow(self):
        self.shadow_flat.copy_(self.param_flat)
        for p in self._params:
            p._fv_shadow_version = p._version
        self.refresh_transposed()

    def refresh_transposed(self):
        from .mixer_ops import transpose_bf16_batched
        for src, dst, params in ((self._t_src, self._t_dst, self._t_params),
                                 (getattr(self, "_tx_src", []), getattr(self, "_tx_dst", []), getattr(self, "_tx_params", []))):
            if src:
                transpose_bf16_batched(src, dst)
                for p in params:
                    p._fv_shadow_t_version = p._version

    @property
    def world_size(self):
        return dist.get_world_size(self.group) if dist.is_initialized() else 1

    def buckets(self, n_buckets, taper=True):
        blocks = [(i, u) for i, u in enumerate(self.unit_ranges) if u[0] is not None]
        if not blocks:
            return [{"bounds": (0, self.grad_flat.numel()), "layers": (0, 0)}]
        first_u, last_u = blocks[0][0], blocks[-1][0]
        nb = len(blocks)
        n_buckets = max(1, min(n_buckets, nb))
        sizes = [u[2] - u[1] for _, u in blocks]
        w = [i + 2 if taper else 1 for i in range(n_buckets)]
        cum = [sum(sizes) * sum(w[:i + 1]) / sum(w) for i in range(n_buckets)]
        runs, acc, lo = [], 0, 0
        for j, sz in enumerate(sizes):
            acc += sz
            left = nb - 1 - j
            if (len(runs) < n_buckets - 1 and acc >= cum[len(runs)] - 1e-9 and left >= n_buckets - 1 - len(runs)) \
                    or j == nb - 1:
                runs.append((lo, j + 1))
                lo = j + 1
        out = []
        for k, (a, b) in enumerate(runs):
            e0 = self.unit_ranges[first_u + a][1] if k > 0 else 0
            e1 = self.unit_ranges[first_u + b - 1][2] if k < len(runs) - 1 else self.grad_flat.numel()
            out.append({"bounds": (e0, e1), "layers": (a, b)})
        return out[::-1]

    def make_exchange(self, n_buckets=1):
        from .ddp import GradExchange
        bk = self.buckets(n_buckets)
        self.exchange = GradExchange(self.grad_flat, [b["bounds"] for b in bk], self.group, self.comm_dtype, self.chunk * 4)
        self.exchange.layers = [b["layers"] for b in bk]
        return self.exchange

    def allreduce_mean_(self):
        self._allreduce(True)

    def allreduce_sum_(self):
        self._allreduce(False)

    def _allreduce(self, mean):
        self.finish_backward()
        if self.world_size == 1:
            return
        if getattr(self, "exchange", None) is None:
            self.make_exchange(1)
        self.exchange.allreduce_(mean=mean)


MAX_PARAM_GROUPS = 256


def build_group_map(names, offsets, sizes, total, groups, default_weight_decay=0.0):
    known = set(names)
    rows, table, per_name = {}, [], {}
    ids = torch.zeros(total, dtype=torch.uint8)
    for g in groups:
        key = (float(g.get("lr_scale", 1.0)), float(g.get("weight_decay", default_weight_decay)))
        for n in g["params"]:
            if n not in known:
                raise ValueError(f"param_groups: {n!r} is not a trainable parameter of the flat training state")
            if n in per_name:
                raise ValueError(f"param_groups: parameter {n!r} appears in more than one group")
            if key not in rows:
                if len(table) == MAX_PARAM_GROUPS:
                    raise ValueError(f"param_groups: more than {MAX_PARAM_GROUPS} distinct (lr_scale, weight_decay) pairs "
                                     "(the fused optimizer keeps one group byte per element)")
                rows[key] = len(table)
                table.append(key)
            per_name[n] = key
            ids[offsets[n]:offsets[n] + sizes[n]] = rows[key]
    missing = [n for n in names if n not in per_name]
    if missing:
        raise ValueError(f"param_groups: {len(missing)} trainable parameters of the flat training state are in no group: "
                         f"{missing[:4]} ...")
    return ids, table, per_name


def groups_from_named(per_name):
    out = {}
    for n, (scale, wd) in per_name.items():
        key = (float(scale), float(wd))
        out.setdefault(key, {"lr_scale": key[0], "weight_decay": key[1], "params": []})["params"].append(n)
    return list(out.values())


class FlatAdamW:

    def __init__(self, flat, model, lr=1e-3, betas=(0.9, 0.999), eps=1e-8, weight_decay=0.05, no_decay=(),
                 ema_decay=None, param_groups=None, max_grad_norm=None, skip_nonfinite=False):
        self.flat = flat
        dev = flat.param_flat.device
        n = flat.param_flat.numel()
        self.exp_avg = torch.zeros(n, device=dev, dtype=torch.float32)
        self.exp_avg_sq = torch.zeros(n, device=dev, dtype=torch.float32)
        self.ema = flat.param_flat.clone() if ema_decay is not None else None
        self.ema_decay = float(ema_decay or 0.0)
        no_decay = set(no_decay)
        self.lr = torch.full((1,), float(lr), device=dev, dtype=torch.float32)
        self.step_t = torch.zeros(1, device=dev, dtype=torch.float32)
        self.betas, self.eps, self.weight_decay = betas, eps, weight_decay
        self.skip_nonfinite = bool(skip_nonfinite)
        self._grouped = param_groups is not None or max_grad_norm is not None or self.skip_nonfinite
        self.group_ids = self.group_table = self.max_norm = self.partials = self.stats = None
        self._group_row_of = None
        self.decay_mask = None
        if not self._grouped:
            mask = torch.zeros(n, dtype=torch.uint8)
            named = dict(model.named_parameters())
            for name, off in flat.offsets.items():
                if name not in no_decay:
                    mask[off:off + named[name].numel()] = 1
            self.decay_mask = mask.to(dev)
        else:
            if param_groups is None:
                groups = [{"params": [nm for nm in flat.names if nm not in no_decay], "weight_decay": weight_decay},
                          {"params": [nm for nm in flat.names if nm in no_decay], "weight_decay": 0.0}]
                groups = [g for g in groups if g["params"]]
            else:
                name_of = {id(p): nm for nm, p in zip(flat.names, flat._params)}
                groups = []
                for g in param_groups:
                    names = []
                    for q in g["params"]:
                        nm = q if isinstance(q, str) else name_of.get(id(q))
                        if nm is None:
                            raise ValueError("param_groups: a parameter of a group is not a trainable parameter of the "
                                             "flat training state")
                        names.append(nm)
                    groups.append({**g, "params": names})
            self._group_table_full = torch.zeros(MAX_PARAM_GROUPS, 2, device=dev, dtype=torch.float32)
            self.group_ids = torch.zeros(n, device=dev, dtype=torch.uint8)
            self._set_groups(groups)
            if max_grad_norm is not None or self.skip_nonfinite:
                G = int(L.lib().fv_grad_sumsq_blocks(ctypes.c_size_t(n)))
                self.partials = torch.zeros(G, device=dev, dtype=torch.float32)
                self.stats = torch.zeros(4, device=dev, dtype=torch.float32)
            if max_grad_norm is not None:
                self.max_norm = torch.full((1,), float(max_grad_norm), device=dev, dtype=torch.float32)

    def _set_groups(self, groups):
        f = self.flat
        sizes = {nm: p.numel() for nm, p in zip(f.names, f._params)}
        ids, table, per_name = build_group_map(f.names, f.offsets, sizes, f.param_flat.numel(), groups, self.weight_decay)
        rows = {key: i for i, key in enumerate(table)}
        with torch.no_grad():
            self.group_ids.copy_(ids)
            self._group_table_full.zero_()
            self._group_table_full[:len(table)].copy_(torch.tensor(table, dtype=torch.float32).view(-1, 2))
        self._group_row_of = {nm: rows[key] for nm, key in per_name.items()}
        self.group_table = self._group_table_full[:len(table)]

    def set_lr(self, lr):
        self.lr.fill_(float(lr))

    def set_max_grad_norm(self, v):
        if self.max_norm is None:
            raise RuntimeError("FlatAdamW was built without max_grad_norm")
        self.max_norm.fill_(float(v))

    def last_stats(self):
        if self.stats is None:
            raise RuntimeError("FlatAdamW was built without max_grad_norm / skip_nonfinite: no gradient norm is computed")
        t, c, fin, sk = self.stats.tolist()
        return {"total_norm": t, "clip_coef": c, "finite": bool(fin), "skipped_steps": int(sk)}

    def _named_slices(self, buf):
        f = self.flat
        named = dict(zip(f.names, f._params))
        return {n: buf[o:o + named[n].numel()].view_as(named[n]) for n, o in f.offsets.items()}

    def state_dict(self):
        ea, es = self._named_slices(self.exp_avg), self._named_slices(self.exp_avg_sq)
        return {"state": {n: {"exp_avg": ea[n].detach().clone(), "exp_avg_sq": es[n].detach().clone()} for n in ea},
                "step": float(self.step_t.item()), "lr": float(self.lr.item()), "betas": tuple(self.betas),
                "eps": self.eps, "weight_decay": self.weight_decay, "ema_decay": self.ema_decay,
                "ema": None if self.ema is None else {n: v.detach().clone() for n, v in self._named_slices(self.ema).items()},
                **self._group_state()}

    def _group_state(self):
        if not self._grouped:
            return {"param_groups": None, "max_grad_norm": None, "skipped_steps": 0}
        tab = self.group_table.detach().cpu().double().tolist()
        return {"param_groups": {nm: tuple(tab[r]) for nm, r in self._group_row_of.items()},
                "max_grad_norm": None if self.max_norm is None else float(self.max_norm.item()),
                "skipped_steps": 0 if self.stats is None else int(self.stats[3].item())}

    def _load_group_state(self, sd):
        if not self._grouped:
            if sd.get("param_groups") is not None or sd.get("max_grad_norm") is not None:
                raise ValueError("FlatAdamW.load_state_dict: the state was saved by an optimizer with param_groups / "
                                 "max_grad_norm, this one was built without them -- pass them to the constructor")
            return
        if sd.get("max_grad_norm") is not None and self.max_norm is None:
            raise ValueError("FlatAdamW.load_state_dict: the state carries max_grad_norm, this optimizer was built without it")
        if sd.get("param_groups") is not None:
            self._set_groups(groups_from_named(sd["param_groups"]))
        if self.max_norm is not None and sd.get("max_grad_norm") is not None:
            self.max_norm.fill_(float(sd["max_grad_norm"]))
        if self.stats is not None and "skipped_steps" in sd:
            self.stats[3].fill_(float(sd["skipped_steps"]))

    def load_state_dict(self, sd):
        ea, es = self._named_slices(self.exp_avg), self._named_slices(self.exp_avg_sq)
        missing = set(ea) - set(sd["state"])
        if missing:
            raise KeyError(f"FlatAdamW.load_state_dict: no state for {sorted(missing)[:4]} ...")
        with torch.no_grad():
            for n in ea:
                ea[n].copy_(sd["state"][n]["exp_avg"])
                es[n].copy_(sd["state"][n]["exp_avg_sq"])
            self.step_t.fill_(float(sd["step"]))
            self.lr.fill_(float(sd["lr"]))
            if self.ema is not None and sd.get("ema") is not None:
                for n, v in self._named_slices(self.ema).items():
                    v.copy_(sd["ema"][n])
        self.betas, self.eps, self.weight_decay = tuple(sd["betas"]), sd["eps"], sd["weight_decay"]
        self._load_group_state(sd)

    def ema_state_dict(self, prefix=""):
        if self.ema is None:
            raise RuntimeError("FlatAdamW was built without ema_decay")
        return {prefix + n: v.detach().clone() for n, v in self._named_slices(self.ema).items()}

    def step(self, grad_scale=1.0):
        f = self.flat
        f.finish_backward()
        if self._grouped:
            return self._step_groups(grad_scale)
        rc = L.lib().fv_adamw_flat(
            L.ptr(f.param_flat), L.ptr(f.grad_flat), L.ptr(self.exp_avg), L.ptr(self.exp_avg_sq), L.ptr(self.ema),
            L.ptr(f.shadow_flat), L.ptr(self.decay_mask), L.ptr(self.lr), L.ptr(self.step_t),
            ctypes.c_float(self.betas[0]), ctypes.c_float(self.betas[1]), ctypes.c_float(self.eps),
            ctypes.c_float(self.weight_decay), ctypes.c_float(self.ema_decay), ctypes.c_float(grad_scale),
            ctypes.c_size_t(f.param_flat.numel()), L.stream_of(f.param_flat))
        L.check(rc, "adamw_flat")
        f.refresh_transposed()

    def _step_groups(self, grad_scale):
        f = self.flat
        n = f.param_flat.numel()
        st = L.stream_of(f.param_flat)
        if self.partials is not None:
            rc = L.lib().fv_grad_sumsq_partials(L.ptr(f.grad_flat), L.ptr(self.partials), ctypes.c_size_t(n), st)
            L.check(rc, "grad_sumsq_partials")
        rc = L.lib().fv_adamw_flat_groups(
            L.ptr(f.param_flat), L.ptr(f.grad_flat), L.ptr(self.exp_avg), L.ptr(self.exp_avg_sq), L.ptr(self.ema),
            L.ptr(f.shadow_flat), L.ptr(self.group_ids), L.ptr(self._group_table_full), L.i32(MAX_PARAM_GROUPS),
            L.ptr(self.lr), L.ptr(self.step_t), L.ptr(self.partials),
            L.i32(0 if self.partials is None else self.partials.numel()), L.ptr(self.max_norm), L.ptr(self.stats),
            L.i32(self.skip_nonfinite), ctypes.c_float(self.betas[0]), ctypes.c_float(self.betas[1]),
            ctypes.c_float(self.eps), ctypes.c_float(self.ema_decay), ctypes.c_float(grad_scale), ctypes.c_size_t(n), st)
        L.check(rc, "adamw_flat_groups")
        f.refresh_transposed()


def save_checkpoint(path, model, opt, prefix="backbone.", **extra):
    ck = {"state_dict": {prefix + k: v.detach().clone() for k, v in model.state_dict().items()},
          "optimizer_states": [opt.state_dict()], **extra}
    if opt.ema is not None:
        ck["state_dict_ema"] = opt.ema_state_dict("")
    torch.save(ck, path)
    return ck


def load_checkpoint(path_or_dict, model, opt=None, prefix="backbone.", use_ema=False):
    ck = torch.load(path_or_dict, map_location="cpu", weights_only=False) if isinstance(path_or_dict, (str, os.PathLike)) else path_or_dict
    sd = ck["state_dict_ema"] if (use_ema and "state_dict_ema" in ck) else ck["state_dict"]
    model.load_state_dict({(k[len(prefix):] if prefix and k.startswith(prefix) else k): v for k, v in sd.items()}, strict=True)
    if opt is not None:
        opt.load_state_dict(ck["optimizer_states"][0])
    return ck
```

### fastvim_amd/mamba_simple_faster.py

```python
import ctypes
import math

import torch
import torch.nn as nn
import torch.nn.functional as F

from . import _lib as L
from . import mixer_ops as M
from .gemm import gemm_any_bnn, gemm_any_btn, gemm_any_nn, gemm_any_nt, gemm_any_tn, gemm_nn, gemm_nt, gemm_tn


def _shadow(w, cdt):
    sh = getattr(w, "_fv_shadow", None)
    if sh is not None and sh.dtype == cdt:
        if w._version != w._fv_shadow_version:
            with torch.no_grad():
                sh.copy_(w)
            w._fv_shadow_version = w._version
        return sh
    return w.to(cdt)


def _shadow_t(w, cdt):
    wt = getattr(w, "_fv_shadow_t", None)
    if wt is not None and wt.dtype == cdt:
        if w._version != w._fv_shadow_t_version:
            with torch.no_grad():
                wt.copy_(_shadow(w, cdt).t())
            w._fv_shadow_t_version = w._version
        return wt
    return _shadow(w, cdt).t().contiguous()


def _wx2_shadow_t(fv):
    if fv is None:
        return None
    wt = fv.get("Wx2_shadow_t")
    if wt is None:
        return None
    params = fv["Wx2_t_params"]
    if any(w._version != w._fv_shadow_t_version for w in params):
        with torch.no_grad():
            for k, w in enumerate(params):
                wt[k].copy_(_shadow(w, wt.dtype).t())
                w._fv_shadow_t_version = w._version
    return wt


def _direct_grad(w):
    g = w.grad
    if getattr(w, "_fv_direct", False) and g is not None and g.is_contiguous() and g.dtype == torch.float32:
        return g
    return None


def _wgrad(X, Y, W=None, splits=16):
    M_, I = X.shape
    J = Y.shape[1]
    while splits > 1 and (M_ % splits or M_ // splits < 256):
        splits //= 2
    part = gemm_any_tn(X, Y, splits)
    g = _direct_grad(W) if W is not None else None
    if g is not None:
        M.reduce_partials(part, splits, out=g.view(-1), accumulate=True)
        return None
    return M.reduce_partials(part, splits)


def _mfma_ok(*ts):
    return all(t.dtype == torch.bfloat16 and t.stride(-1) == 1 and t.data_ptr() % 16 == 0 for t in ts)


def _any_ok(*ts):
    return all(t.is_cuda and t.dtype in (torch.float32, torch.bfloat16) and t.dim() == 2 for t in ts)


def linear_fwd(a2, w_c, bias=None):
    if _mfma_ok(a2, w_c) and a2.shape[1] % 8 == 0 and w_c.shape[0] % 8 == 0:
        return gemm_nt(a2, w_c, bias=None if bias is None else bias.float())
    if _any_ok(a2, w_c):
        return gemm_any_nt(a2, w_c, bias)
    return F.linear(a2, w_c, None if bias is None else bias.to(a2.dtype))


def linear_dgrad(g2, w_c):
    if _mfma_ok(g2, w_c) and w_c.shape[1] % 8 == 0 and g2.shape[1] % 8 == 0:
        return gemm_nn(g2, w_c)
    if _any_ok(g2, w_c):
        return gemm_any_nn(g2, w_c)
    return g2 @ w_c


class _SideStream:
    enabled = False
    stream = None
    pending = []

    @classmethod
    def run(cls, fn, *keep):
        if not cls.enabled:
            return fn()
        cur = torch.cuda.current_stream()
        if cls.stream is None:
            cls.stream = torch.cuda.Stream()
        cls.stream.wait_stream(cur)
        with torch.cuda.stream(cls.stream):
            out = fn()
        cls.pending.append(keep)
        return out

    @classmethod
    def join(cls):
        if cls.stream is not None and cls.pending:
            torch.cuda.current_stream().wait_stream(cls.stream)
        cls.pending = []


XPROJ_IN_SCAN = True


class _GroupedWgrad:
    enabled = False
    jobs = []
    chunk = 0

    @classmethod
    def add(cls, g2, a2, out):
        from .gemm import grouped_splits
        if any(j[2].data_ptr() == out.data_ptr() for j in cls.jobs):
            cls.flush()
        cls.jobs.append((g2, a2, out, grouped_splits(g2.shape[0], M=g2.shape[1], N=a2.shape[1])))
        if cls.chunk and len(cls.jobs) >= cls.chunk:
            cls.flush()

    sums = []
    rows_jobs = []

    @classmethod
    def flush(cls):
        if cls.rows_jobs:
            rj, cls.rows_jobs = cls.rows_jobs, []
            M.chunk_rows_bf16(rj)
        if cls.jobs:
            from .gemm import gemm_tn_grouped
            jobs, cls.jobs = cls.jobs, []
            if _SideStream.enabled:
                cls.sums += _SideStream.run(lambda: gemm_tn_grouped(jobs, reduce=False), jobs)
            else:
                gemm_tn_grouped(jobs)

    @classmethod
    def reduce(cls):
        sums, cls.sums = cls.sums, []
        for part, sp, out in sums:
            M.reduce_partials(part, sp, out=out, accumulate=True)


def group_wgrads(on):
    flush_wgrads()
    _GroupedWgrad.enabled = bool(on)


def flush_wgrads():
    _GroupedWgrad.flush()
    _SideStream.join()
    _GroupedWgrad.reduce()


def linear_wgrad(g2, a2, W=None, splits=None):
    if _mfma_ok(g2, a2) and g2.shape[1] % 8 == 0 and a2.shape[1] % 8 == 0 and g2.shape[0] % 64 == 0:
        gdir = _direct_grad(W) if W is not None else None
        if gdir is not None and _GroupedWgrad.enabled and splits is None and g2.is_contiguous() and a2.is_contiguous():
            _GroupedWgrad.add(g2, a2, gdir.view(-1))
            return None
        if gdir is not None:
            gemm_tn(g2, a2, splits=splits, out=gdir.view(-1), accumulate=True, defer=not _SideStream.enabled)
            return None
        return gemm_tn(g2, a2, splits=splits)
    return _wgrad(g2, a2, W)


class LinearFn(torch.autograd.Function):

    @staticmethod
    def forward(ctx, a, W, cdt, bias=None):
        with torch.autocast("cuda", enabled=False):
            a2 = a.reshape(-1, a.shape[-1]).to(cdt).contiguous()
            W2 = W.reshape(W.shape[0], -1)
            y = linear_fwd(a2, _shadow(W, cdt).reshape(W2.shape), bias)
        ctx.save_for_backward(a2, W)
        ctx.a_shape, ctx.a_dtype, ctx.cdt = a.shape, a.dtype, cdt
        ctx.need_da = a.requires_grad
        ctx.has_bias = bias is not None
        ctx.bias_ref = bias
        return y.view(*a.shape[:-1], W.shape[0])

    @staticmethod
    def backward(ctx, g):
        a2, W = ctx.saved_tensors
        cdt = ctx.cdt
        with torch.autocast("cuda", enabled=False):
            g2 = g.reshape(-1, g.shape[-1]).to(cdt).contiguous()
            W2s = _shadow(W, cdt).reshape(W.shape[0], -1)
            da = linear_dgrad(g2, W2s).view(ctx.a_shape).to(ctx.a_dtype) if ctx.need_da else None
            dW = linear_wgrad(g2, a2, W)
            if dW is not None:
                dW = dW.view(W.shape)
            db = None
            if ctx.has_bias:
                bias = ctx.bias_ref
                gd = _direct_grad(bias) if bias is not None else None
                if g2.is_cuda and g2.dtype in (torch.float32, torch.bfloat16):
                    from .glue_ops import column_sum
                    if gd is not None:
                        column_sum(g2, out=gd.view(-1), accumulate=True)
                    else:
                        db = column_sum(g2)
                else:
                    db = g2.float().sum(0)
        return da, dW, None, db


def linear_module(mod, x):
    if isinstance(mod, nn.Linear) and x.is_cuda:
        return LinearFn.apply(x, mod.weight, _compute_dtype(x), mod.bias)
    return mod(x)


class OutProjAddNormFn(torch.autograd.Function):

    @staticmethod
    def forward(ctx, g, W_out, residual, norm_w, eps, row_scale, cdt):
        L.require_gpu(g, W_out, residual, norm_w)
        B, Ltok, d_in = g.shape
        d = W_out.shape[0]
        Mrows = B * Ltok
        with torch.autocast("cuda", enabled=False):
            y, res_out, rstd, w32, row_scale, rows_per_scale = _out_proj_add_norm_fwd(g, W_out, residual, norm_w, eps, row_scale, cdt)
        ctx.save_for_backward(g, W_out, res_out, w32, rstd, row_scale)
        ctx.rows_per_scale = rows_per_scale
        ctx.cdt = cdt
        ctx.shape = (B, Ltok, d)
        ctx.w_param = norm_w
        return y.view(B, Ltok, d), res_out.view(B, Ltok, d)

    @staticmethod
    def backward(ctx, dy, dres_out):
        g, W_out, r, w32, rstd, row_scale = ctx.saved_tensors
        B, Ltok, d = ctx.shape
        Mrows, d_in = B * Ltok, g.shape[2]
        cdt, dev = ctx.cdt, g.device
        with torch.autocast("cuda", enabled=False):
            dy = dy.reshape(Mrows, d).contiguous()
            dres_out = dres_out.reshape(Mrows, d).contiguous() if dres_out is not None else None
            dx = torch.empty(Mrows, d, device=dev, dtype=cdt)
            dres_in = torch.empty(Mrows, d, device=dev, dtype=torch.float32)
            lib = L.lib()
            nb = lib.fv_add_norm_blocks(L.i32(Mrows))
            pw = torch.empty(nb, d, device=dev, dtype=torch.float32)
            rc = lib.fv_add_norm_bwd(
                L.ptr(dy), L.i32(L.dtype_code(dy.dtype)), L.ptr(dres_out),
                L.i32(L.dtype_code(dres_out.dtype) if dres_out is not None else 0), L.ptr(r), L.i32(L.FV_F32),
                L.ptr(w32), L.ptr(None), L.ptr(rstd), L.ptr(row_scale), L.i32(ctx.rows_per_scale), L.ptr(dx),
                L.i32(L.dtype_code(cdt)), L.ptr(dres_in), L.i32(L.FV_F32), L.ptr(pw), L.ptr(None), L.i32(Mrows), L.i32(d),
                L.i32(1), L.stream_of(r))
            L.check(rc, "add_norm_bwd")
            gd = _direct_grad(ctx.w_param)
            if gd is not None:
                M.reduce_partials(pw, nb, out=gd.view(-1), accumulate=True)
                dw = None
            else:
                dw = M.reduce_partials(pw, nb).to(ctx.w_param.dtype)
            g2 = g.view(Mrows, d_in)
            dg = linear_dgrad(dx, _shadow(W_out, cdt)).view(B, Ltok, d_in)
            dW_out = _SideStream.run(lambda: linear_wgrad(dx, g2, W_out), dx, g)
        return dg, dW_out, dres_in.view(B, Ltok, d), dw, None, None, None


class _Ctx:

    def save_for_backward(self, *tensors):
        self.saved_tensors = tensors


COMBINE_IN_OUT_PROJ = True
CONV_IN_DGRAD = True
XPROJ_TWO_ADDENDS = True


def resolve_combine(pack):
    if pack is not None:
        M.combine_fwd(pack["xz"], pack["skip"], pack["yc"], pack["ln_w"], pack["ln_b"], pack["eps"], pack["rows"],
                      pack["cols"], pack["transposed"], out=pack["out"])


def _out_proj_add_norm_fwd(g, W_out, residual, norm_w, eps, row_scale, cdt, W_in=None, pack=None):
    B, Ltok, d_in = g.shape
    d = W_out.shape[0]
    Mrows = B * Ltok
    g2 = g.view(Mrows, d_in)
    res2 = residual.reshape(Mrows, d).contiguous()
    w32 = norm_w.float().contiguous()
    y = torch.empty(Mrows, d, device=g.device, dtype=cdt)
    res_out = torch.empty(Mrows, d, device=g.device, dtype=torch.float32)
    rstd = torch.empty(Mrows, device=g.device, dtype=torch.float32)
    rows_per_scale = 1
    if row_scale is not None:
        row_scale = row_scale.float().contiguous()
        rows_per_scale = Mrows // row_scale.numel()
    xz = None
    if W_in is not None and W_in.shape[0] % 128 == 0:
        xz = torch.empty(Mrows, W_in.shape[0], device=g.device, dtype=cdt)
    W_out_c = _shadow(W_out, cdt)
    W_in_c = _shadow(W_in, cdt) if xz is not None else None
    lib = L.lib()
    if pack is not None:
        if xz is None and W_out_c.stride(1) == 1 and W_out_c.stride(0) % 8 == 0 and W_out_c.data_ptr() % 16 == 0:
            y, res_out, rstd = M.combine_out_proj_addnorm(pack["xz"], pack["skip"], pack["yc"], pack["ln_w"], pack["ln_b"],
                                                          pack["eps"], pack["rows"], pack["cols"], pack["transposed"],
                                                          pack["out"], W_out_c, res2, w32, row_scale, rows_per_scale, eps)
            return y, res_out, rstd, w32, row_scale, rows_per_scale
        resolve_combine(pack)
    rc = lib.fv_gemm_bf16_addnorm2(
        L.ptr(g2), L.ptr(W_out_c), L.ptr(res2), L.ptr(w32), L.ptr(row_scale), L.i32(rows_per_scale),
        L.ptr(y), L.ptr(res_out), L.ptr(rstd), L.i32(Mrows), L.i32(d), L.i32(d_in), ctypes.c_long(g2.stride(0)),
        ctypes.c_long(d_in), ctypes.c_float(eps), L.ptr(W_in_c), L.ptr(xz),
        L.i32(W_in.shape[0] if xz is not None else 0), ctypes.c_long(d), L.stream_of(g2))
    L.check(rc, "gemm_bf16_addnorm")
    if W_in is not None:
        return y, res_out, rstd, w32, row_scale, rows_per_scale, xz
    return y, res_out, rstd, w32, row_scale, rows_per_scale


class ChainedBlockFn(torch.autograd.Function):

    in_proj_in_launch = False
    pending_in = None
    pending_out = None
    defer = False

    @staticmethod
    def forward(ctx, g_prev, W_out_prev, residual, norm_w, eps, row_scale, *mixer_args):
        L.require_gpu(g_prev, W_out_prev, residual, norm_w)
        B, Ltok, _ = g_prev.shape
        d = W_out_prev.shape[0]
        cdt = mixer_args[26]
        W_in, b_in = mixer_args[0], mixer_args[1]
        pack, ChainedBlockFn.pending_in = ChainedBlockFn.pending_in, None
        assert pack is None or pack["out"][0].data_ptr() == g_prev.data_ptr()
        with torch.autocast("cuda", enabled=False):
            if pack is not None:
                y, res_out, rstd, w32, rs, rps = _out_proj_add_norm_fwd(g_prev, W_out_prev, residual, norm_w, eps, row_scale,
                                                                      cdt, pack=pack)
                xz = None
            elif ChainedBlockFn.in_proj_in_launch and b_in is None:
                y, res_out, rstd, w32, rs, rps, xz = _out_proj_add_norm_fwd(g_prev, W_out_prev, residual, norm_w, eps,
                                                                          row_scale, cdt, W_in=W_in)
            else:
                y, res_out, rstd, w32, rs, rps = _out_proj_add_norm_fwd(g_prev, W_out_prev, residual, norm_w, eps, row_scale, cdt)
                xz = None
        fctx = _Ctx()
        fctx.precomputed_xz = xz
        fctx.defer_combine = ChainedBlockFn.defer
        g = FastVimMixerFn.forward(fctx, y.view(B, Ltok, d), *mixer_args)
        mixer_saved = fctx.__dict__.pop("saved_tensors")
        fctx.__dict__.pop("precomputed_xz", None)
        fctx.__dict__.pop("defer_combine", None)
        ChainedBlockFn.pending_out = fctx.__dict__.pop("pending_combine", None)
        ctx.save_for_backward(g_prev, W_out_prev, res_out, w32, rstd, rs, *mixer_saved)
        ctx.mixer_attrs = fctx.__dict__
        ctx.rows_per_scale = rps
        ctx.cdt = cdt
        ctx.shape = (B, Ltok, d)
        ctx.w_param = norm_w
        ctx.W_in = mixer_args[0]
        ctx.n_mixer_args = len(mixer_args)
        return g, res_out.view(B, Ltok, d)

    @staticmethod
    def backward(ctx, dg, dres_out):
        g_prev, W_out_prev, r, w32, rstd, row_scale = ctx.saved_tensors[:6]
        B, Ltok, d = ctx.shape
        Mrows, cdt, dev = B * Ltok, ctx.cdt, r.device
        fctx = _Ctx()
        fctx.__dict__.update(ctx.mixer_attrs)
        fctx.saved_tensors = ctx.saved_tensors[6:]
        out = {}

        def fused_in_dgrad(dxz2):
            lib = L.lib()
            nb = lib.fv_gemm_bf16_dgrad_addnorm_blocks(L.i32(Mrows))
            dx = torch.empty(Mrows, d, device=dev, dtype=cdt)
            dres_in = torch.empty(Mrows, d, device=dev, dtype=torch.float32)
            pw = torch.empty(nb, d, device=dev, dtype=torch.float32)
            gg = dres_out.reshape(Mrows, d).contiguous() if dres_out is not None else None
            d_prev = g_prev.shape[2]
            W2 = _shadow(W_out_prev, cdt) if d_prev % 128 == 0 else None
            W_in_c = _shadow(ctx.W_in, cdt)
            dg_prev = torch.empty(Mrows, d_prev, device=dev, dtype=cdt) if W2 is not None else None
            rc = lib.fv_gemm_bf16_dgrad_addnorm_bwd2(
                L.ptr(dxz2), L.ptr(W_in_c), L.ptr(gg), L.ptr(r), L.ptr(rstd), L.ptr(w32), L.ptr(row_scale),
                L.i32(ctx.rows_per_scale), L.ptr(dx), L.ptr(dres_in), L.ptr(pw), L.i32(Mrows), L.i32(d),
                L.i32(dxz2.shape[1]), ctypes.c_long(dxz2.stride(0)), ctypes.c_long(d), L.ptr(W2), L.ptr(dg_prev),
                L.i32(d_prev if W2 is not None else 0), ctypes.c_long(d_prev), L.stream_of(dxz2))
            L.check(rc, "gemm_bf16_dgrad_addnorm_bwd")
            out.update(dx=dx, dres_in=dres_in, pw=pw, nb=nb, dg_prev=dg_prev)

        def fused_conv_dgrad(xz, d_o, dxc, dxc2, cw2, cb, cwb2, cb_b, D, D_b, dxz, rows, cols, transposed, scaling, conv_grad_out):
            gg = dres_out.reshape(Mrows, d).contiguous() if dres_out is not None else None
            d_prev = g_prev.shape[2]
            W2 = _shadow(W_out_prev, cdt) if d_prev % 128 == 0 else None
            W_in_t = _shadow_t(ctx.W_in, cdt)
            p2, dx, dres_in, pw, nb, dg_prev = M.conv_pool_bwd_dgrad(
                xz, d_o, dxc, dxc2, cw2, cb, cwb2, cb_b, D, D_b, dxz, rows, cols, transposed, scaling, W_in_t, gg, r, rstd,
                w32, row_scale, ctx.rows_per_scale, W2=W2, conv_grad_out=conv_grad_out)
            out.update(dx=dx, dres_in=dres_in, pw=pw, nb=nb, dg_prev=dg_prev)
            return p2

        fctx.fused_in_dgrad = fused_in_dgrad
        if (CONV_IN_DGRAD and cdt == torch.bfloat16 and d == 192 and ctx.W_in.shape[0] == 768 and (row_scale is None or row_scale.dtype == torch.float32)):
            fctx.fused_conv_dgrad = fused_conv_dgrad
        grads = FastVimMixerFn.backward(fctx, dg)
        with torch.autocast("cuda", enabled=False):
            gd = _direct_grad(ctx.w_param)
            if gd is not None:
                M.reduce_partials(out["pw"], out["nb"], out=gd.view(-1), accumulate=True)
                dw = None
            else:
                dw = M.reduce_partials(out["pw"], out["nb"]).to(ctx.w_param.dtype)
            dx = out["dx"]
            d_in = g_prev.shape[2]
            g2 = g_prev.view(Mrows, d_in)
            dg_prev = out["dg_prev"] if out["dg_prev"] is not None else linear_dgrad(dx, _shadow(W_out_prev, cdt))
            dg_prev = dg_prev.view(B, Ltok, d_in)
            dW_out = _SideStream.run(lambda: linear_wgrad(dx, g2, W_out_prev), dx, g_prev)
        return (dg_prev, dW_out, out["dres_in"].view(B, Ltok, d), dw, None, None) + tuple(grads[1:1 + ctx.n_mixer_args])


def out_proj_add_norm_ok(g, W_out, residual, norm_w, cdt):
    return (g.is_cuda and cdt == torch.bfloat16 and g.dtype == torch.bfloat16 and g.is_contiguous()
            and W_out.shape[0] == 192 and W_out.shape[1] % 64 == 0 and residual is not None
            and residual.dtype == torch.float32 and norm_w.dtype == torch.float32)


def _compute_dtype(t):
    if torch.is_autocast_enabled():
        dt = torch.get_autocast_dtype('cuda')
        return torch.float32 if dt == torch.float16 else dt
    return torch.float32 if t.dtype == torch.float16 else t.dtype


def half_io(t):
    if torch.is_autocast_enabled():
        return torch.get_autocast_dtype('cuda') == torch.float16
    return t.dtype == torch.float16


def mixer_apply(fn, hidden, *args):
    if any(torch.is_tensor(a) and a.dtype == torch.float16 for a in args):
        args = tuple(a.float() if torch.is_tensor(a) and a.dtype == torch.float16 else a for a in args)
    out = fn.apply(hidden, *args)
    return out.to(torch.float16) if hidden.dtype == torch.float16 else out


class FastVimMixerFn(torch.autograd.Function):

    @staticmethod
    def forward(ctx, hidden, W_in, b_in, cw, cb, cw_b, cb_b, Wx, Wx_b, Wdt, bdt, Wdt_b, bdt_b, A_log, A_b_log,
                D, D_b, ln_w, ln_b, W_out, b_out, rows, cols, transposed, pool_max, scaling, ln_eps, cdt, fv, tpp=1,
                valid=None):
        L.require_gpu(hidden)
        B, Ltok, d = hidden.shape
        if Ltok != rows * cols * tpp:
            raise RuntimeError(f"Mamba: sequence length {Ltok} != token grid {rows}x{cols}x{tpp}")
        d_in = W_in.shape[0] // 2
        with torch.autocast("cuda", enabled=False):
            h_c = hidden.to(cdt).contiguous()
            W_in_c = _shadow(W_in, cdt)
            W_out_c = _shadow(W_out, cdt) if W_out is not None else None
            xz = getattr(ctx, "precomputed_xz", None)
            if xz is None:
                xz = linear_fwd(h_c.view(B * Ltok, d), W_in_c, b_in)
            xz = xz.view(B, Ltok, 2 * d_in)
            cw2, cwb2 = cw.reshape(d_in, -1), cw_b.reshape(d_in, -1)
            amax = None
            if fv is not None and "Wx2" in fv:
                Wx2 = fv["Wx2"]
                if fv["Wx2_shadow"].dtype == cdt:
                    _shadow(Wx, cdt), _shadow(Wx_b, cdt)
                    Wx2_c = fv["Wx2_shadow"]
                else:
                    Wx2_c = Wx2.to(cdt)
            else:
                Wx2 = torch.stack([Wx, Wx_b])
                Wx2_c = Wx2.to(cdt)
            if pool_max:
                xc, skip, amax = M.conv_pool_fwd(xz, cw2, cb, cwb2, cb_b, rows, cols, transposed, pool_max, scaling, tpp,
                                                 D=D, D_b=D_b)
            else:
                xc, skip = M.conv_pool_fwd(xz, cw2, cb, cwb2, cb_b, rows, cols, transposed, pool_max, scaling, tpp,
                                           D=D, D_b=D_b)
            if valid is not None and valid < rows * tpp:
                xc[:, :, valid:].zero_()
            fused = M.xproj_scan_fwd(xc, Wx2_c, Wdt, bdt, A_log, Wdt_b, bdt_b, A_b_log)
            if fused is not None:
                x_dbl, yc = fused
            else:
                x_dbl = M.xproj_fwd(xc, Wx2_c)
                nig = getattr(ctx, "needs_input_grad", None)
                yc, ctx.scan_ckpt = M.scan_fwd(xc, x_dbl, Wdt, bdt, A_log, Wdt_b, bdt_b, A_b_log,
                                               want_ckpt=nig is None or any(nig))
            if (getattr(ctx, "defer_combine", False) and W_out is None and not pool_max and valid is None
                    and M.combine_out_proj_addnorm_ok(xz, rows, cols, tpp, d)):
                g, mean, rstd = M.combine_buffers(xz, ln_w)
                ctx.pending_combine = dict(xz=xz, skip=skip, yc=yc, ln_w=ln_w, ln_b=ln_b, eps=ln_eps, rows=rows, cols=cols,
                                           transposed=transposed, out=(g, mean, rstd))
            else:
                g, mean, rstd = M.combine_fwd(xz, skip, yc, ln_w, ln_b, ln_eps, rows, cols, transposed, tpp=tpp)
            out = g if W_out is None else linear_fwd(g.view(B * Ltok, d_in), W_out_c, b_out).view(B, Ltok, d)
        ctx.save_for_backward(h_c, W_in, cw, cb, cw_b, cb_b, Wx2, Wdt, bdt, Wdt_b, bdt_b, A_log, A_b_log, D, D_b,
                              ln_w, ln_b, W_out, xz, xc, x_dbl, g, skip, yc, mean, rstd, amax)
        ctx.geo = (rows, cols, transposed, pool_max, scaling, tpp)
        ctx.has_bias = (b_in is not None, b_out is not None)
        ctx.cdt = cdt
        ctx.in_dtype = hidden.dtype
        ctx.fv = fv
        return out

    @staticmethod
    def backward(ctx, dout):
        (h_c, W_in, cw, cb, cw_b, cb_b, Wx2, Wdt, bdt, Wdt_b, bdt_b, A_log, A_b_log, D, D_b, ln_w, ln_b, W_out,
         xz, xc, x_dbl, g, skip, yc, mean, rstd, amax) = ctx.saved_tensors
        rows, cols, transposed, pool_max, scaling, tpp = ctx.geo
        cdt = ctx.cdt
        B, Ltok, d = h_c.shape
        d_in = W_in.shape[0] // 2
        fv = ctx.fv or {}
        with torch.autocast("cuda", enabled=False):
            dout = dout.to(cdt).contiguous()
            if W_out is None:
                dg, dW_out, db_out = dout.view(B * Ltok, d_in), None, None
            else:
                do2 = dout.view(B * Ltok, d)
                dg = linear_dgrad(do2, _shadow(W_out, cdt))
                dW_out = _SideStream.run(lambda: linear_wgrad(do2, g.view(B * Ltok, d_in), W_out), do2, g)
                db_out = do2.float().sum(0) if ctx.has_bias[1] else None
            cw2, cwb2 = cw.reshape(d_in, -1), cw_b.reshape(d_in, -1)
            dxz = torch.empty_like(xz)
            d_o, dyc, p1 = M.combine_bwd(dg, xz, skip, yc, ln_w, ln_b, mean, rstd, dxz, rows, cols, transposed,
                                         grad_out=fv.get("ln_grad") if ln_w is not None else None, tpp=tpp)
            W_ = x_dbl.shape[-1]
            fused_xproj = W_ in M.XPROJ_WIDTHS
            Mrows = B * rows * tpp
            grouped_x = (fused_xproj and _GroupedWgrad.enabled and "Wx2_grad" in fv and xc.dtype == torch.bfloat16
                         and Mrows % 64 == 0 and d_in % 8 == 0)
            dxc2 = None
            if (grouped_x and XPROJ_IN_SCAN and amax is None and getattr(ctx, "scan_ckpt", None) is None
                    and M.scan_bwd_xproj_ok(xc, Wdt, pool_max, rows, cols, tpp)):
                wsh = fv.get("Wx2_shadow")
                dxc, dxc2, dx_dbl, ps = M.scan_bwd_xproj(xc, x_dbl, Wdt, bdt, A_log, Wdt_b, bdt_b, A_b_log, dyc,
                                                         Wx2[0], Wx2[1], grad_out=fv.get("scan_grad"),
                                                         Wx2_bf16=wsh if wsh is not None and wsh.dtype == torch.bfloat16 else None)
                dxb = torch.empty(2, Mrows, (W_ + 7) // 8 * 8, device=xc.device, dtype=torch.bfloat16)
                _GroupedWgrad.rows_jobs.append((dx_dbl, dxb))
                xc2 = xc.view(2, Mrows, d_in)
                for k_ in range(2):
                    _GroupedWgrad.add(dxb[k_][:, :W_], xc2[k_], fv["Wx2_grad"][k_].reshape(-1))
                dWx2 = (None, None)
            else:
                dxc, dx_dbl, ps = M.scan_bwd(xc, x_dbl, Wdt, bdt, A_log, Wdt_b, bdt_b, A_b_log, dyc,
                                             grad_out=fv.get("scan_grad"), keep_chunks=fused_xproj,
                                             ckpt=getattr(ctx, "scan_ckpt", None))
            if dxc2 is not None:
                pass
            elif grouped_x:
                wt = _wx2_shadow_t(fv)
                if (wt is not None and amax is None and XPROJ_TWO_ADDENDS and M.xproj_bwd3_ok(Mrows, d_in, W_, xc.dtype)
                        and M.conv_pool_bwd2_ok(rows, cols, tpp, d_in, pool_max)):
                    dxc2 = torch.empty(dxc.shape, device=dxc.device, dtype=xc.dtype)
                dxb = M.xproj_bwd(dx_dbl, xc, Wx2[0], Wx2[1], dxc, dw=False, Wx2_t=wt, dxc2=dxc2)
                xc2 = xc.view(2, Mrows, d_in)
                for k_ in range(2):
                    _GroupedWgrad.add(dxb[k_][:, :W_], xc2[k_], fv["Wx2_grad"][k_].reshape(-1))
                dWx2 = (None, None)
            elif fused_xproj:
                dWx2 = M.xproj_bwd(dx_dbl, xc, Wx2[0], Wx2[1], dxc, grad_out=fv.get("Wx2_grad"))
                if dWx2 is None:
                    dWx2 = (None, None)
            else:
                xc2 = xc.view(2, B * rows * tpp, d_in)
                dWx2 = gemm_any_btn(dx_dbl, xc2)
                if "Wx2_grad" in fv:
                    fv["Wx2_grad"].add_(dWx2)
                    dWx2 = (None, None)
                dxc = dxc.view(2, B * rows * tpp, d_in) + gemm_any_bnn(dx_dbl, Wx2.float(), out_dtype=torch.float32)
            conv_grad = fv.get("conv_grad") if cb is not None and cb_b is not None else None
            fused_cd = getattr(ctx, "fused_conv_dgrad", None)
            dxz2 = dxz.view(B * Ltok, 2 * d_in)
            if (fused_cd is not None and amax is None and dxc.dtype == torch.float32 and dxc.is_contiguous()
                    and M.conv_pool_bwd_dgrad_ok(xz, rows, cols, tpp, d, pool_max)):
                p2 = fused_cd(xz, d_o, dxc, dxc2, cw2, cb, cwb2, cb_b, D, D_b, dxz, rows, cols, transposed, scaling, conv_grad)
                fused_dgrad = "done"
            else:
                p2 = M.conv_pool_bwd(xz, d_o, dxc, cw2, cb, cwb2, cb_b, D, D_b, dxz, rows, cols, transposed,
                                     pool_max, scaling, grad_out=conv_grad, tpp=tpp, amax=amax, dxc2=dxc2)
                fused_dgrad = getattr(ctx, "fused_in_dgrad", None)
            if fused_dgrad == "done":
                dhidden = None
            elif fused_dgrad is not None:
                fused_dgrad(dxz2)
                dhidden = None
            else:
                dhidden = linear_dgrad(dxz2, _shadow(W_in, cdt)).view(B, Ltok, d).to(ctx.in_dtype)
            dW_in = _SideStream.run(lambda: linear_wgrad(dxz2, h_c.view(B * Ltok, d), W_in), dxz2, h_c)
            db_in = dxz2.float().sum(0) if ctx.has_bias[0] else None
        has_ln = ln_w is not None
        n4 = 4 * d_in
        N_, R_ = A_log.shape[1], Wdt.shape[1]
        if p2 is None:
            g_cw = g_cb = g_cwb = g_cbb = g_D = g_Db = None
        else:
            g_cw, g_cwb = p2[0:n4].view(cw.shape), p2[n4:2 * n4].view(cw_b.shape)
            g_cb = p2[2 * n4:2 * n4 + d_in] if cb is not None else None
            g_cbb = p2[2 * n4 + d_in:2 * n4 + 2 * d_in] if cb_b is not None else None
            g_D, g_Db = p2[2 * n4 + 2 * d_in:2 * n4 + 3 * d_in], p2[2 * n4 + 3 * d_in:2 * n4 + 4 * d_in]
        if ps is None:
            g_A = g_Wdt = g_bdt = (None, None)
        else:
            g_A = [ps[k, :d_in * N_].view(d_in, N_) for k in range(2)]
            g_Wdt = [ps[k, d_in * N_:d_in * (N_ + R_)].view(d_in, R_) for k in range(2)]
            g_bdt = [ps[k, d_in * (N_ + R_):] for k in range(2)]
        g_lw = p1[0] if (has_ln and p1 is not None) else None
        g_lb = p1[1] if (has_ln and p1 is not None) else None
        return (dhidden, dW_in, db_in, g_cw, g_cb, g_cwb, g_cbb,
                dWx2[0], dWx2[1], g_Wdt[0], g_bdt[0], g_Wdt[1], g_bdt[1], g_A[0], g_A[1],
                g_D, g_Db, g_lw, g_lb, dW_out, db_out, None, None, None, None, None, None, None, None, None, None)


class Mamba(nn.Module):
    def __init__(self, d_model, d_state=16, d_conv=4, expand=2, dt_rank="auto", dt_min=0.001, dt_max=0.1,
                 dt_init="random", dt_scale=1.0, dt_init_floor=1e-4, conv_bias=True, bias=False,
                 use_fast_path=False, layer_idx=None, device=None, dtype=None, init_layer_scale=None,
                 scanpath_type="rowwise", token_size=None, use_norm_after_ssm=True,
                 use_our_selective_scan=False, collapse_method="mean", scaling_factor=1):
        factory_kwargs = {"device": device, "dtype": dtype}
        super().__init__()
        self.d_model = d_model
        self.d_state = d_state
        self.d_conv = d_conv
        self.expand = expand
        self.d_inner = int(self.expand * self.d_model)
        self.dt_rank = math.ceil(self.d_model / 16) if dt_rank == "auto" else dt_rank
        self.use_fast_path = use_fast_path
        self.layer_idx = layer_idx
        self.use_our_selective_scan = use_our_selective_scan
        self.num_of_rows, self.num_of_col = token_size[0], token_size[1]
        self.scanpath_type = scanpath_type
        self.scaling_factor = scaling_factor
        if collapse_method not in ("mean", "max"):
            raise NotImplementedError(collapse_method)
        self.collapse_method = collapse_method
        self.init_layer_scale = init_layer_scale
        if init_layer_scale is not None:
            self.gamma = nn.Parameter(init_layer_scale * torch.ones(d_model), requires_grad=True)

        self.in_proj = nn.Linear(self.d_model, self.d_inner * 2, bias=bias, **factory_kwargs)
        self.use_norm_after_ssm = use_norm_after_ssm
        if use_norm_after_ssm:
            self.layernorm = nn.LayerNorm(self.d_inner, **factory_kwargs)

        def conv():
            return nn.Conv1d(self.d_inner, self.d_inner, bias=conv_bias, kernel_size=d_conv, groups=self.d_inner,
                             padding=d_conv - 1, **factory_kwargs)

        self.conv1d = conv()
        self.activation = "silu"
        self.act = nn.SiLU()
        self.x_proj = nn.Linear(self.d_inner, self.dt_rank + self.d_state * 2, bias=False, **factory_kwargs)
        self.dt_proj = nn.Linear(self.dt_rank, self.d_inner, bias=True, **factory_kwargs)

        dt_init_std = self.dt_rank ** -0.5 * dt_scale
        if dt_init == "constant":
            nn.init.constant_(self.dt_proj.weight, dt_init_std)
        elif dt_init == "random":
            nn.init.uniform_(self.dt_proj.weight, -dt_init_std, dt_init_std)
        else:
            raise NotImplementedError
        dt = torch.exp(torch.rand(self.d_inner, **factory_kwargs) * (math.log(dt_max) - math.log(dt_min))
                       + math.log(dt_min)).clamp(min=dt_init_floor)
        inv_dt = dt + torch.log(-torch.expm1(-dt))
        with torch.no_grad():
            self.dt_proj.bias.copy_(inv_dt)
        self.dt_proj.bias._no_reinit = True

        def s4d_real():
            A = torch.arange(1, self.d_state + 1, dtype=torch.float32, device=device).repeat(self.d_inner, 1)
            p = nn.Parameter(torch.log(A).contiguous())
            p._no_weight_decay = True
            return p

        self.A_log = s4d_real()
        self.D = nn.Parameter(torch.ones(self.d_inner, device=device))
        self.D._no_weight_decay = True
        self.A_b_log = s4d_real()
        self.conv1d_b = conv()
        self.x_proj_b = nn.Linear(self.d_inner, self.dt_rank + self.d_state * 2, bias=False, **factory_kwargs)
        self.dt_proj_b = nn.Linear(self.dt_rank, self.d_inner, bias=True, **factory_kwargs)
        self.D_b = nn.Parameter(torch.ones(self.d_inner, device=device))
        self.D_b._no_weight_decay = True
        self.out_proj = nn.Linear(self.d_inner, self.d_model, bias=bias, **factory_kwargs)
        self.pre_x_shape = (-1, self.d_inner, self.num_of_rows, self.num_of_col)

    def mixer_fn_args(self, cdt, transposed_grid=False, defer_out_proj=False):
        ln_w = self.layernorm.weight if self.use_norm_after_ssm else None
        ln_b = self.layernorm.bias if self.use_norm_after_ssm else None
        ln_eps = self.layernorm.eps if self.use_norm_after_ssm else 0.0
        return (self.in_proj.weight, self.in_proj.bias,
                self.conv1d.weight, self.conv1d.bias, self.conv1d_b.weight, self.conv1d_b.bias,
                self.x_proj.weight, self.x_proj_b.weight,
                self.dt_proj.weight, self.dt_proj.bias, self.dt_proj_b.weight, self.dt_proj_b.bias,
                self.A_log, self.A_b_log, self.D, self.D_b, ln_w, ln_b,
                None if defer_out_proj else self.out_proj.weight, None if defer_out_proj else self.out_proj.bias,
                self.num_of_rows, self.num_of_col, bool(transposed_grid), self.collapse_method == "max",
                float(self.scaling_factor), float(ln_eps), cdt, self.__dict__.get("_fv"))

    def forward(self, hidden_states, inference_params=None, transposed_grid=False, defer_out_proj=False):
        if inference_params is not None:
            raise NotImplementedError("FastVim mixers have no inference cache (reference: no step())")
        if self.d_conv != 4 or self.d_state != 16:
            raise RuntimeError("fastvim_amd kernels are built for d_conv=4, d_state=16 (the FastVim configs)")
        cdt = _compute_dtype(hidden_states)
        ln_w = self.layernorm.weight if self.use_norm_after_ssm else None
        ln_b = self.layernorm.bias if self.use_norm_after_ssm else None
        ln_eps = self.layernorm.eps if self.use_norm_after_ssm else 0.0
        out = mixer_apply(
            FastVimMixerFn, hidden_states, self.in_proj.weight, self.in_proj.bias,
            self.conv1d.weight, self.conv1d.bias, self.conv1d_b.weight, self.conv1d_b.bias,
            self.x_proj.weight, self.x_proj_b.weight,
            self.dt_proj.weight, self.dt_proj.bias, self.dt_proj_b.weight, self.dt_proj_b.bias,
            self.A_log, self.A_b_log, self.D, self.D_b, ln_w, ln_b,
            None if defer_out_proj else self.out_proj.weight, None if defer_out_proj else self.out_proj.bias,
            self.num_of_rows, self.num_of_col, bool(transposed_grid), self.collapse_method == "max",
            float(self.scaling_factor), float(ln_eps), cdt, self.__dict__.get("_fv"))
        if defer_out_proj:
            if self.init_layer_scale is not None or self.out_proj.bias is not None:
                raise RuntimeError("defer_out_proj: layer scale / out_proj bias are applied after out_proj")
            return out
        if self.init_layer_scale is not None:
            out = out * self.gamma
        return out
```

### fastvim_amd/mixer_ops.py

```python
import ctypes

import torch

from . import _lib as L

f32 = ctypes.c_float


def _geo(rows, cols, transposed):
    return (1, rows) if transposed else (cols, 1)


def conv_pool_fwd(xz, conv_w, conv_b, conv_w_b, conv_b_b, rows, cols, transposed, pool_max, scaling, tpp=1,
                  D=None, D_b=None):
    B, Ltok, two_d = xz.shape
    d_in = two_d // 2
    s_i, s_j = _geo(rows, cols, transposed)
    xc = torch.empty(2, B, rows * tpp, d_in, device=xz.device, dtype=xz.dtype)
    skip = torch.empty(B, Ltok, d_in, device=xz.device, dtype=xz.dtype) if D is not None else None
    amax = torch.empty_like(xc) if pool_max else None
    rc = L.lib().fv_mixer_conv_pool_fwd(
        L.ptr(xz), L.ptr(conv_w), L.ptr(conv_b), L.ptr(conv_w_b), L.ptr(conv_b_b), L.ptr(D), L.ptr(D_b), L.ptr(xc),
        L.ptr(skip), L.ptr(amax), L.i32(B), L.i32(rows), L.i32(cols), L.i32(s_i), L.i32(s_j), L.i32(tpp), L.i32(d_in),
        L.i32(conv_w.shape[-1]), L.i32(pool_max), f32(scaling), L.i32(L.dtype_code(xz.dtype)), L.stream_of(xz))
    L.check(rc, "mixer_conv_pool_fwd")
    if pool_max:
        return (xc, amax) if D is None else (xc, skip, amax)
    return xc if D is None else (xc, skip)


def scan_fwd(xc, x_dbl, dt_w, dt_b, A_log, dt_w_b, dt_b_b, A_log_b, want_ckpt=False):
    _, B, Lc, d_in = xc.shape
    R = dt_w.shape[1]
    N = A_log.shape[1]
    lib = L.lib()
    yc = torch.empty(2, B, Lc, d_in, device=xc.device, dtype=torch.float32)
    ckpt = None
    if want_ckpt:
        nck = lib.fv_mixer_scan_ckpt_floats(L.i32(B), L.i32(Lc), L.i32(d_in), L.i32(N), L.i32(R))
        ckpt = torch.empty(nck, device=xc.device, dtype=torch.float32) if nck else None
    nws = lib.fv_mixer_scan_fwd_seg_floats(L.i32(B), L.i32(Lc), L.i32(d_in), L.i32(N), L.i32(R))
    ws = torch.empty(nws, device=xc.device, dtype=torch.float32) if nws else None
    rc = lib.fv_mixer_scan_fwd_seg(
        L.ptr(xc), L.ptr(x_dbl), L.ptr(dt_w), L.ptr(dt_b), L.ptr(A_log), L.ptr(dt_w_b), L.ptr(dt_b_b),
        L.ptr(A_log_b), L.ptr(yc), L.ptr(ckpt), L.ptr(ws), L.i32(B), L.i32(Lc), L.i32(d_in), L.i32(R), L.i32(N),
        L.i32(L.dtype_code(xc.dtype)), L.stream_of(xc))
    L.check(rc, "mixer_scan_fwd")
    return (yc, ckpt) if want_ckpt else yc


def xproj_scan_fwd(xc, Wx2_c, dt_w, dt_b, A_log, dt_w_b, dt_b_b, A_log_b):
    _, B, Lc, d_in = xc.shape
    R, N = dt_w.shape[1], A_log.shape[1]
    W = Wx2_c.shape[1]
    lib = L.lib()
    if (xc.dtype != torch.bfloat16 or Wx2_c.dtype != torch.bfloat16 or N != 16 or W != R + 2 * N
            or not xc.is_contiguous() or not Wx2_c.is_contiguous() or xc.data_ptr() % 16 or Wx2_c.data_ptr() % 16
            or not lib.fv_mixer_xproj_scan_fwd_ok(L.i32(Lc), L.i32(d_in), L.i32(R), L.i32(L.dtype_code(xc.dtype)))):
        return None
    x_dbl = torch.empty(2, B * Lc, W, device=xc.device, dtype=xc.dtype)
    yc = torch.empty(2, B, Lc, d_in, device=xc.device, dtype=torch.float32)
    rc = lib.fv_mixer_xproj_scan_fwd(
        L.ptr(xc), L.ptr(Wx2_c), L.ptr(dt_w), L.ptr(dt_b), L.ptr(A_log), L.ptr(dt_w_b), L.ptr(dt_b_b), L.ptr(A_log_b),
        L.ptr(x_dbl), L.ptr(yc), L.i32(B), L.i32(Lc), L.i32(d_in), L.i32(R), L.i32(N), L.i32(L.dtype_code(xc.dtype)),
        L.stream_of(xc))
    L.check(rc, "mixer_xproj_scan_fwd")
    return x_dbl, yc


def combine_buffers(xz, ln_w):
    B, Ltok, two_d = xz.shape
    g = torch.empty(B, Ltok, two_d // 2, device=xz.device, dtype=xz.dtype)
    if ln_w is not None:
        return g, torch.empty(B * Ltok, device=xz.device, dtype=torch.float32), torch.empty(B * Ltok, device=xz.device, dtype=torch.float32)
    return g, None, None


def combine_fwd(xz, skip, yc, ln_w, ln_b, eps, rows, cols, transposed, tpp=1, out=None):
    B, Ltok, two_d = xz.shape
    d_in = two_d // 2
    s_i, s_j = _geo(rows, cols, transposed)
    g, mean, rstd = out if out is not None else combine_buffers(xz, ln_w)
    rc = L.lib().fv_mixer_combine_fwd(
        L.ptr(xz), L.ptr(skip), L.ptr(yc), L.ptr(ln_w), L.ptr(ln_b), f32(eps), L.ptr(g), L.ptr(mean), L.ptr(rstd),
        L.i32(B), L.i32(rows), L.i32(cols), L.i32(s_i), L.i32(s_j), L.i32(tpp), L.i32(d_in),
        L.i32(L.dtype_code(xz.dtype)), L.stream_of(xz))
    L.check(rc, "mixer_combine_fwd")
    return g, mean, rstd


class _Deferred:
    enabled = False
    max_jobs = 144
    side = False
    jobs = []
    stream = None
    pending = []

    @classmethod
    def add(cls, part, out, n_partials):
        lo, hi = out.data_ptr(), out.data_ptr() + out.numel() * 4
        if any(j[1].data_ptr() < hi and lo < j[1].data_ptr() + j[1].numel() * 4 for j in cls.jobs):
            cls.flush()
        cls.jobs.append((part, out, n_partials))
        if len(cls.jobs) >= cls.max_jobs:
            cls.flush()

    @classmethod
    def _launch(cls, jobs):
        k = len(jobs)
        ins = (ctypes.c_void_p * k)(*[j[0].data_ptr() for j in jobs])
        outs = (ctypes.c_void_p * k)(*[j[1].data_ptr() for j in jobs])
        Ss = (ctypes.c_int * k)(*[j[2] for j in jobs])
        ns = (ctypes.c_size_t * k)(*[j[0].numel() // j[2] for j in jobs])
        rc = L.lib().fv_reduce_partials_multi(ins, outs, Ss, ns, L.i32(k), L.i32(1), L.stream_of(jobs[0][0]))
        L.check(rc, "reduce_partials_multi")

    @classmethod
    def flush(cls):
        if not cls.jobs:
            return
        jobs, cls.jobs = cls.jobs, []
        if not cls.side:
            cls._launch(jobs)
            return
        cur = torch.cuda.current_stream()
        if cls.stream is None:
            cls.stream = torch.cuda.Stream()
        cls.stream.wait_stream(cur)
        with torch.cuda.stream(cls.stream):
            cls._launch(jobs)
        cls.pending.append(jobs)

    @classmethod
    def join(cls):
        if cls.pending:
            torch.cuda.current_stream().wait_stream(cls.stream)
            cls.pending = []


def defer_reductions(on):
    flush_reductions()
    _Deferred.enabled = bool(on)


def pending_reductions():
    return len(_Deferred.jobs)


def drop_reductions():
    n = len(_Deferred.jobs)
    _Deferred.jobs = []
    return n


def flush_reductions():
    _Deferred.flush()
    _Deferred.join()


def reduce_partials(part, n_partials, out=None, accumulate=False, defer=True):
    if out is not None and accumulate and defer and _Deferred.enabled:
        assert out.numel() == part.numel() // n_partials and out.is_contiguous() and out.dtype == torch.float32
        _Deferred.add(part, out, n_partials)
        return out
    if out is None:
        out = torch.empty(part.shape[1:], device=part.device, dtype=torch.float32)
    n = part.numel() // n_partials
    assert out.numel() == n and out.is_contiguous() and out.dtype == torch.float32
    rc = L.lib().fv_reduce_partials(L.ptr(part), L.ptr(out), L.i32(n_partials), ctypes.c_size_t(n),
                                    L.i32(accumulate), L.stream_of(part))
    L.check(rc, "reduce_partials")
    return out


def combine_out_proj_addnorm_ok(xz, rows, cols, tpp, d_model):
    B, Ltok, two_d = xz.shape
    return bool(xz.dtype == torch.bfloat16 and xz.is_contiguous() and
                L.lib().fv_mixer_combine_out_proj_addnorm_ok(L.i32(B), L.i32(rows), L.i32(cols), L.i32(tpp), L.i32(two_d // 2),
                                                             L.i32(d_model), L.i32(L.FV_BF16)))


def combine_out_proj_addnorm(xz, skip, yc, ln_w, ln_b, ln_eps, rows, cols, transposed, out, W_out_c, residual2, norm_w32,
                             row_scale, rows_per_scale, eps):
    B, Ltok, two_d = xz.shape
    d = W_out_c.shape[0]
    Mrows = B * Ltok
    s_i, s_j = _geo(rows, cols, transposed)
    g, mean, rstd_ln = out
    y = torch.empty(Mrows, d, device=xz.device, dtype=torch.bfloat16)
    res_out = torch.empty(Mrows, d, device=xz.device, dtype=torch.float32)
    rstd = torch.empty(Mrows, device=xz.device, dtype=torch.float32)
    rc = L.lib().fv_mixer_combine_out_proj_addnorm(
        L.ptr(xz), L.ptr(skip), L.ptr(yc), L.ptr(ln_w), L.ptr(ln_b), f32(ln_eps), L.ptr(g), L.ptr(mean), L.ptr(rstd_ln),
        L.i32(B), L.i32(rows), L.i32(cols), L.i32(s_i), L.i32(s_j), L.ptr(W_out_c), ctypes.c_long(W_out_c.stride(0)),
        L.ptr(residual2), L.ptr(norm_w32), L.ptr(row_scale), L.i32(rows_per_scale), L.ptr(y), L.ptr(res_out), L.ptr(rstd),
        f32(eps), L.stream_of(xz))
    L.check(rc, "mixer_combine_out_proj_addnorm")
    return y, res_out, rstd


def combine_bwd(dg, xz, skip, yc, ln_w, ln_b, mean, rstd, dxz, rows, cols, transposed, grad_out=None, tpp=1):
    B, Ltok, two_d = xz.shape
    d_in = two_d // 2
    s_i, s_j = _geo(rows, cols, transposed)
    lib = L.lib()
    nb = lib.fv_mixer_bwd_blocks(L.i32(B), L.i32(rows), L.i32(d_in), L.i32(tpp), L.i32(0))
    d_o = torch.empty(B, Ltok, d_in, device=xz.device, dtype=xz.dtype)
    dyc = torch.empty(B, rows * tpp, d_in, device=xz.device, dtype=torch.float32)
    part = torch.empty(nb, 2, d_in, device=xz.device, dtype=torch.float32)
    rc = lib.fv_mixer_combine_bwd(
        L.ptr(dg), L.ptr(xz), L.ptr(skip), L.ptr(yc), L.ptr(ln_w), L.ptr(ln_b), L.ptr(mean), L.ptr(rstd), L.ptr(dxz), L.ptr(d_o),
        L.ptr(dyc), L.ptr(part), L.i32(B), L.i32(rows), L.i32(cols), L.i32(s_i), L.i32(s_j), L.i32(tpp), L.i32(d_in),
        L.i32(L.dtype_code(xz.dtype)), L.stream_of(xz))
    L.check(rc, "mixer_combine_bwd")
    if grad_out is not None:
        reduce_partials(part, nb, out=grad_out, accumulate=True)
        return d_o, dyc, None
    return d_o, dyc, reduce_partials(part, nb)


def scan_bwd(xc, x_dbl, dt_w, dt_b, A_log, dt_w_b, dt_b_b, A_log_b, dyc, grad_out=None, keep_chunks=False,
             dyc_per_direction=False, ckpt=None):
    _, B, Lc, d_in = xc.shape
    assert dyc.numel() == (2 if dyc_per_direction else 1) * B * Lc * d_in and dyc.dtype == torch.float32
    R, N = dt_w.shape[1], A_log.shape[1]
    W = R + 2 * N
    dev = xc.device
    lib = L.lib()
    f32o = dict(device=dev, dtype=torch.float32)
    given = ckpt is not None
    nws = lib.fv_mixer_scan_bwd_seg_floats(L.i32(B), L.i32(Lc), L.i32(d_in), L.i32(N), L.i32(R)) if given else 0
    nchunks = lib.fv_mixer_scan_bwd_seg_chunks(L.i32(B), L.i32(d_in), L.i32(Lc), L.i32(R), L.i32(int(nws > 0)))
    dxc = torch.empty(2, B, Lc, d_in, **f32o)
    dx_dbl = torch.empty(nchunks, 2, B * Lc, W, **f32o)
    if not given:
        nck = lib.fv_mixer_scan_bwd_ckpt_floats(L.i32(B), L.i32(Lc), L.i32(d_in), L.i32(N), L.i32(R))
        ckpt = torch.empty(nck, **f32o) if nck else None
    ws = torch.empty(nws, **f32o) if nws else None
    nprt = lib.fv_mixer_scan_bwd_seg_partials(L.i32(B), L.i32(Lc), L.i32(d_in), L.i32(R)) if nws else \
        lib.fv_mixer_scan_bwd_partials(L.i32(B), L.i32(Lc), L.i32(R))
    part = torch.empty(nprt, 2 * d_in * (N + R + 1), **f32o)
    rc = lib.fv_mixer_scan_bwd_seg(
        L.ptr(xc), L.ptr(x_dbl), L.ptr(dt_w), L.ptr(dt_b), L.ptr(A_log), L.ptr(dt_w_b), L.ptr(dt_b_b),
        L.ptr(A_log_b), L.ptr(dyc), L.i32(int(dyc_per_direction)), L.ptr(dxc), L.ptr(dx_dbl), L.ptr(ckpt), L.i32(int(given)),
        L.ptr(part), L.ptr(ws), L.i32(B), L.i32(Lc), L.i32(d_in), L.i32(R), L.i32(N), L.i32(L.dtype_code(xc.dtype)),
        L.stream_of(xc))
    L.check(rc, "mixer_scan_bwd")
    if not keep_chunks:
        dx_dbl = dx_dbl[0] if nchunks == 1 else reduce_partials(dx_dbl, nchunks)
    if grad_out is not None:
        reduce_partials(part, nprt, out=grad_out, accumulate=True)
        return dxc, dx_dbl, None
    return dxc, dx_dbl, reduce_partials(part, nprt).view(2, d_in * (N + R + 1))


def scan_bwd_xproj_ok(xc, dt_w, pool_max, rows, cols, tpp):
    _, B, Lc, d_in = xc.shape
    lib = L.lib()
    return bool(xc.dtype in (torch.float32, torch.bfloat16)
                and lib.fv_mixer_scan_bwd_xproj_ok(L.i32(B), L.i32(Lc), L.i32(d_in), L.i32(dt_w.shape[1]), L.i32(L.dtype_code(xc.dtype)))
                and lib.fv_mixer_conv_pool_bwd2_ok(L.i32(rows), L.i32(cols), L.i32(tpp), L.i32(d_in), L.i32(int(bool(pool_max)))))


def scan_bwd_xproj(xc, x_dbl, dt_w, dt_b, A_log, dt_w_b, dt_b_b, A_log_b, dyc, Wx, Wx_b, grad_out=None, Wx2_bf16=None):
    _, B, Lc, d_in = xc.shape
    R, N = dt_w.shape[1], A_log.shape[1]
    W = R + 2 * N
    lib = L.lib()
    f32o = dict(device=xc.device, dtype=torch.float32)
    dxc = torch.empty(2, B, Lc, d_in, **f32o)
    dxc2 = torch.empty(2, B, Lc, d_in, device=xc.device, dtype=xc.dtype)
    dx_dbl = torch.empty(2, 2, B * Lc, W, **f32o)
    nprt = lib.fv_mixer_scan_bwd_partials(L.i32(B), L.i32(Lc), L.i32(R))
    part = torch.empty(nprt, 2 * d_in * (N + R + 1), **f32o)
    if xc.dtype == torch.bfloat16 and Wx2_bf16 is None:
        Wx2_bf16 = torch.stack([Wx, Wx_b]).to(torch.bfloat16)
    assert Wx2_bf16 is None or (Wx2_bf16.dtype == torch.bfloat16 and Wx2_bf16.is_contiguous() and Wx2_bf16.shape == (2, W, d_in))
    rc = lib.fv_mixer_scan_bwd_xproj(
        L.ptr(xc), L.ptr(x_dbl), L.ptr(dt_w), L.ptr(dt_b), L.ptr(A_log), L.ptr(dt_w_b), L.ptr(dt_b_b), L.ptr(A_log_b),
        L.ptr(dyc), L.ptr(Wx), L.ptr(Wx_b), L.ptr(Wx2_bf16), L.ptr(dxc), L.ptr(dxc2), L.ptr(dx_dbl), L.ptr(part), L.i32(B), L.i32(Lc),
        L.i32(d_in), L.i32(R), L.i32(N), L.i32(L.dtype_code(xc.dtype)), L.stream_of(xc))
    L.check(rc, "mixer_scan_bwd_xproj")
    if grad_out is not None:
        reduce_partials(part, nprt, out=grad_out, accumulate=True)
        return dxc, dxc2, dx_dbl, None
    return dxc, dxc2, dx_dbl, reduce_partials(part, nprt).view(2, d_in * (N + R + 1))


def chunk_rows_bf16(jobs):
    lib = L.lib()
    buckets = {}
    for j in jobs:
        assert j[1].dtype == torch.bfloat16 and j[1].is_contiguous() and j[0].dtype == torch.float32 and j[0].is_contiguous()
        buckets.setdefault((tuple(j[0].shape), tuple(j[1].shape)), []).append(j)
    for (ishape, _), bjobs in buckets.items():
        nchunks, _, Mrows, W = ishape
        for lo in range(0, len(bjobs), 64):
            grp = bjobs[lo:lo + 64]
            k = len(grp)
            ins = (ctypes.c_void_p * k)(*[j[0].data_ptr() for j in grp])
            outs = (ctypes.c_void_p * k)(*[j[1].data_ptr() for j in grp])
            rc = lib.fv_chunk_rows_bf16(ins, outs, L.i32(k), L.i32(nchunks), ctypes.c_long(2 * Mrows), L.i32(W), L.stream_of(grp[0][0]))
            L.check(rc, "chunk_rows_bf16")


def conv_pool_bwd(xz, d_o, dxc, conv_w, conv_b, conv_w_b, conv_b_b, D, D_b, dxz, rows, cols, transposed,
                  pool_max, scaling, grad_out=None, tpp=1, amax=None, dxc2=None):
    B, Ltok, two_d = xz.shape
    d_in = two_d // 2
    s_i, s_j = _geo(rows, cols, transposed)
    lib = L.lib()
    nb = lib.fv_mixer_bwd_blocks(L.i32(B), L.i32(rows), L.i32(d_in), L.i32(tpp), L.i32(1))
    part = torch.empty(nb, 12 * d_in, device=xz.device, dtype=torch.float32)
    assert dxc2 is None or (dxc2.dtype == xz.dtype and dxc2.shape == dxc.shape and dxc2.is_contiguous())
    rc = lib.fv_mixer_conv_pool_bwd2(
        L.ptr(xz), L.ptr(d_o), L.ptr(dxc), L.ptr(dxc2), L.ptr(conv_w), L.ptr(conv_b), L.ptr(conv_w_b), L.ptr(conv_b_b),
        L.ptr(D), L.ptr(D_b), L.ptr(amax), L.ptr(dxz), L.ptr(part), L.i32(B), L.i32(rows), L.i32(cols), L.i32(s_i),
        L.i32(s_j), L.i32(tpp), L.i32(d_in), L.i32(conv_w.shape[-1]), L.i32(pool_max), f32(scaling),
        L.i32(L.dtype_code(xz.dtype)), L.stream_of(xz))
    L.check(rc, "mixer_conv_pool_bwd")
    if grad_out is not None:
        reduce_partials(part, nb, out=grad_out, accumulate=True)
        return None
    return reduce_partials(part, nb)


def conv_pool_bwd_dgrad_ok(xz, rows, cols, tpp, d_model, pool_max):
    B, Ltok, two_d = xz.shape
    return bool(xz.dtype == torch.bfloat16 and xz.is_contiguous() and
                L.lib().fv_mixer_conv_pool_bwd_dgrad_ok(L.i32(B), L.i32(rows), L.i32(cols), L.i32(tpp), L.i32(two_d // 2),
                                                        L.i32(d_model), L.i32(int(bool(pool_max))), L.i32(L.FV_BF16)))


def conv_pool_bwd_dgrad(xz, d_o, dxc, dxc2, conv_w, conv_b, conv_w_b, conv_b_b, D, D_b, dxz, rows, cols, transposed, scaling,
                        W_in_t, dres_out, r, rstd, norm_w32, row_scale, rows_per_scale, W2=None, conv_grad_out=None):
    B, Ltok, two_d = xz.shape
    d_in = two_d // 2
    d = W_in_t.shape[0]
    Mrows = B * Ltok
    s_i, s_j = _geo(rows, cols, transposed)
    lib = L.lib()
    dev = xz.device
    nb = lib.fv_mixer_conv_pool_bwd_dgrad_blocks(L.i32(B), L.i32(rows))
    part = torch.empty(nb, 12 * d_in, device=dev, dtype=torch.float32)
    dx = torch.empty(Mrows, d, device=dev, dtype=torch.bfloat16)
    dres_in = torch.empty(Mrows, d, device=dev, dtype=torch.float32)
    pw = torch.empty(nb, d, device=dev, dtype=torch.float32)
    N2 = W2.shape[1] if W2 is not None else 0
    dg_prev = torch.empty(Mrows, N2, device=dev, dtype=torch.bfloat16) if W2 is not None else None
    assert dxc2 is None or (dxc2.dtype == xz.dtype and dxc2.shape == dxc.shape and dxc2.is_contiguous())
    assert W_in_t.dtype == torch.bfloat16 and W_in_t.stride(1) == 1 and W_in_t.shape[1] == two_d
    rc = lib.fv_mixer_conv_pool_bwd_dgrad(
        L.ptr(xz), L.ptr(d_o), L.ptr(dxc), L.ptr(dxc2), L.ptr(conv_w), L.ptr(conv_b), L.ptr(conv_w_b), L.ptr(conv_b_b),
        L.ptr(D), L.ptr(D_b), L.ptr(dxz), L.ptr(part), L.i32(B), L.i32(rows), L.i32(cols), L.i32(s_i), L.i32(s_j),
        f32(scaling), L.ptr(W_in_t), ctypes.c_long(W_in_t.stride(0)), L.ptr(dres_out), L.ptr(r), L.ptr(rstd), L.ptr(norm_w32),
        L.ptr(row_scale), L.i32(rows_per_scale), L.ptr(dx), L.ptr(dres_in), L.ptr(pw), L.ptr(W2), L.ptr(dg_prev), L.i32(N2),
        ctypes.c_long(W2.stride(0) if W2 is not None else 0), L.stream_of(xz))
    L.check(rc, "mixer_conv_pool_bwd_dgrad")
    if conv_grad_out is not None:
        reduce_partials(part, nb, out=conv_grad_out, accumulate=True)
        p2 = None
    else:
        p2 = reduce_partials(part, nb)
    return p2, dx, dres_in, pw, nb, dg_prev


def transpose_bf16_batched(srcs, dsts):
    lib = L.lib()
    rows, cols = srcs[0].shape
    for lo in range(0, len(srcs), 64):
        a, b = srcs[lo:lo + 64], dsts[lo:lo + 64]
        assert all(t.dtype == torch.bfloat16 and t.is_contiguous() and tuple(t.shape) == (rows, cols) for t in a)
        assert all(t.dtype == torch.bfloat16 and t.is_contiguous() and tuple(t.shape) == (cols, rows) for t in b)
        k = len(a)
        ins = (ctypes.c_void_p * k)(*[t.data_ptr() for t in a])
        outs = (ctypes.c_void_p * k)(*[t.data_ptr() for t in b])
        L.check(lib.fv_transpose_bf16_batched(ins, outs, L.i32(k), L.i32(rows), L.i32(cols), L.stream_of(a[0])), "transpose_bf16_batched")


XPROJ_WIDTHS = (44, 56, 80, 96, 112, 34, 36, 38, 64)


def xproj_fwd(xc, Wx2_c):
    d_in = xc.shape[-1]
    Mrows = xc.numel() // (2 * d_in)
    W = Wx2_c.shape[1]
    if (xc.dtype != torch.bfloat16 or Wx2_c.dtype != torch.bfloat16 or d_in % 32 or W > 112
            or not xc.is_contiguous() or not Wx2_c.is_contiguous() or xc.data_ptr() % 16 or Wx2_c.data_ptr() % 16):
        if xc.is_cuda and xc.dtype in (torch.float32, torch.bfloat16) and Wx2_c.dtype in (torch.float32, torch.bfloat16):
            from .gemm import gemm_any_bnt
            return gemm_any_bnt(xc.reshape(2, Mrows, d_in), Wx2_c)
        return torch.bmm(xc.view(2, Mrows, d_in), Wx2_c.transpose(1, 2))
    out = torch.empty(2, Mrows, W, device=xc.device, dtype=xc.dtype)
    rc = L.lib().fv_mixer_xproj_fwd(L.ptr(xc), L.ptr(Wx2_c), L.ptr(out), L.i32(Mrows), L.i32(d_in), L.i32(W), L.stream_of(xc))
    L.check(rc, "mixer_xproj_fwd")
    return out


_XPROJ_PRESUM = 8


def xproj_bwd3_ok(Mrows, d_in, W, dtype):
    return bool(dtype == torch.bfloat16 and L.lib().fv_mixer_xproj_bwd3_ok(L.i32(Mrows), L.i32(d_in), L.i32(W), L.i32(L.dtype_code(dtype))))


def conv_pool_bwd2_ok(rows, cols, tpp, d_in, pool_max):
    return bool(L.lib().fv_mixer_conv_pool_bwd2_ok(L.i32(rows), L.i32(cols), L.i32(tpp), L.i32(d_in), L.i32(int(pool_max))))


def xproj_bwd(dx_dbl_chunks, xc, Wx, Wx_b, dxc, grad_out=None, dw=True, Wx2_t=None, dxc2=None):
    nchunks, _, Mrows, W = dx_dbl_chunks.shape
    d_in = xc.shape[-1]
    lib = L.lib()
    if nchunks >= _XPROJ_PRESUM:
        dx_dbl_chunks = reduce_partials(dx_dbl_chunks, nchunks, defer=False).view(1, 2, Mrows, W)
        nchunks = 1
    if not dw:
        WP = (W + 7) // 8 * 8
        dxb = torch.empty(2, Mrows, WP, device=xc.device, dtype=torch.bfloat16)
        if Wx2_t is not None:
            assert Wx2_t.dtype == torch.bfloat16 and Wx2_t.is_contiguous() and tuple(Wx2_t.shape) == (2, d_in, W)
            assert dxc2 is None or (dxc2.dtype == torch.bfloat16 and dxc2.is_contiguous() and dxc2.numel() == dxc.numel())
            rc = lib.fv_mixer_xproj_bwd3(L.ptr(dx_dbl_chunks), L.i32(nchunks), L.ptr(xc), L.ptr(Wx), L.ptr(Wx_b), L.ptr(Wx2_t),
                                         L.ptr(dxc), L.ptr(dxc2), L.ptr(dxb), L.i32(Mrows), L.i32(d_in), L.i32(W),
                                         L.i32(L.dtype_code(xc.dtype)), L.stream_of(xc))
        else:
            assert dxc2 is None
            rc = lib.fv_mixer_xproj_bwd2(L.ptr(dx_dbl_chunks), L.i32(nchunks), L.ptr(xc), L.ptr(Wx), L.ptr(Wx_b), L.ptr(dxc),
                                         None, L.ptr(dxb), L.i32(Mrows), L.i32(d_in), L.i32(W),
                                         L.i32(L.dtype_code(xc.dtype)), L.stream_of(xc))
        L.check(rc, "mixer_xproj_bwd")
        return dxb
    ns = lib.fv_mixer_xproj_bwd_slices(L.i32(Mrows))
    part = torch.empty(ns, 2, W, d_in, device=xc.device, dtype=torch.float32)
    rc = lib.fv_mixer_xproj_bwd(L.ptr(dx_dbl_chunks), L.i32(nchunks), L.ptr(xc), L.ptr(Wx), L.ptr(Wx_b), L.ptr(dxc),
                                L.ptr(part), L.i32(Mrows), L.i32(d_in), L.i32(W), L.i32(L.dtype_code(xc.dtype)),
                                L.stream_of(xc))
    L.check(rc, "mixer_xproj_bwd")
    if grad_out is not None:
        reduce_partials(part, ns, out=grad_out.view(-1), accumulate=True)
        return None
    return reduce_partials(part, ns)


def rows_segment_sum(x, idx, rows, scale=1.0, out_dtype=None):
    per_dir = x.dim() == 4
    B, Lk, d = x.shape[-3:]
    assert idx.shape == (2, B, Lk) and idx.dtype == torch.int32 and idx.is_contiguous() and x.is_contiguous()
    out = torch.empty(2, B, rows, d, device=x.device, dtype=out_dtype or x.dtype)
    rc = L.lib().fv_rows_segment_sum(L.ptr(x), L.i32(L.dtype_code(x.dtype)), L.i32(int(per_dir)), L.ptr(idx), L.ptr(out),
                                     L.i32(L.dtype_code(out.dtype)), L.i32(B), L.i32(Lk), L.i32(rows), L.i32(d),
                                     f32(scale), L.stream_of(x))
    L.check(rc, "rows_segment_sum")
    return out


def rows_gather(x, idx, scale=1.0, out_dtype=None):
    _, B, rows, d = x.shape
    Lk = idx.shape[-1]
    assert idx.shape == (2, B, Lk) and idx.dtype == torch.int32 and idx.is_contiguous() and x.is_contiguous()
    out = torch.empty(2, B, Lk, d, device=x.device, dtype=out_dtype or x.dtype)
    rc = L.lib().fv_rows_gather(L.ptr(x), L.i32(L.dtype_code(x.dtype)), L.ptr(idx), L.ptr(out),
                                L.i32(L.dtype_code(out.dtype)), L.i32(B), L.i32(Lk), L.i32(rows), L.i32(d), f32(scale),
                                L.stream_of(x))
    L.check(rc, "rows_gather")
    return out
```

### fastvim_amd/pipeline.py

```python
import warnings

import torch
import torch.distributed as dist


class SegmentedTrainStep:

    def __init__(self, model, flat, opt, loss_fn, x, target, n_segments=3, amp_dtype=torch.bfloat16, use_graph=True,
                 warmup=2):
        self.model, self.flat, self.opt, self.loss_fn = model, flat, opt, loss_fn
        self.x, self.target, self.amp_dtype = x, target, amp_dtype
        self.exchange = flat.make_exchange(n_segments)
        self.runs = self.exchange.layers
        self.K = len(self.runs)
        self._gscale = 1.0 / self.exchange.world_size
        self.use_graph = use_graph
        self.loss = None
        self._seed = torch.ones((), device=x.device, dtype=torch.float32)
        self._cuts = None
        self._exposed = []
        self.graphs = None
        if use_graph:
            self._capture(warmup)

    def _forward(self):
        m = self.model
        self.flat.zero_grad()
        cuts = []
        with torch.autocast("cuda", dtype=self.amp_dtype, enabled=self.amp_dtype != torch.float32):
            h, _ = m._embed(self.x)
            res, pend = None, None
            fwd_runs = self.runs[::-1]
            open_runs = hasattr(m, "_run_layers_open")
            for i, (lo, hi) in enumerate(fwd_runs):
                if i > 0:
                    res = res.detach().requires_grad_()
                    if pend is not None:
                        pend = (pend[0].detach().requires_grad_(), pend[1])
                        ins = (pend[0], res)
                    else:
                        h = h.detach().requires_grad_()
                        ins = (h, res)
                else:
                    ins = None
                if open_runs:
                    h, res, pend = m._run_layers_open(h, res, lo, hi, pend=pend)
                else:
                    h, res = m._run_layers(h, res, lo, hi)
                cuts.append([ins, (h if pend is None else pend[0], res)])
            if pend is not None:
                h = m._close_run(pend)
            logits = m._head(m._final(h, res))
        loss = self.loss_fn(logits, self.target)
        cuts[-1][1] = (loss,)
        self._cuts = cuts
        return loss.detach()

    def _backward(self, k):
        i = self.K - 1 - k
        outs = self._cuts[i][1]
        if k == 0:
            seed = self._seed if (outs[0].dim() == 0 and outs[0].dtype == self._seed.dtype and outs[0].device == self._seed.device) else None
            torch.autograd.backward(outs[0], seed)
        else:
            nxt = self._cuts[i + 1][0]
            torch.autograd.backward(list(outs), [t.grad for t in nxt])
        self.flat.finish_backward()
        self._cuts[i][1] = None

    def _eager_step(self):
        loss = self._forward()
        for k in range(self.K):
            self._backward(k)
            self.exchange.launch(k)
        self.exchange.finish(mean=False)
        self.opt.step(grad_scale=self._gscale)
        return loss

    def _snapshot(self):
        f, o = self.flat, self.opt
        bufs = [f.param_flat, f.shadow_flat] + list(getattr(f, "_t_dst", [])) + list(getattr(f, "_tx_dst", []))
        for v in vars(o).values():
            if torch.is_tensor(v) and v.is_cuda and all(v is not b for b in bufs):
                bufs.append(v)
        dev = f.param_flat.device
        return ([(b, b.clone()) for b in bufs], torch.get_rng_state(), torch.cuda.get_rng_state(dev), dev)

    @staticmethod
    def _restore(snap):
        bufs, cpu_rng, gpu_rng, dev = snap
        with torch.no_grad():
            for b, saved in bufs:
                b.copy_(saved)
        torch.set_rng_state(cpu_rng)
        torch.cuda.set_rng_state(gpu_rng, dev)

    def _capture(self, warmup):
        from . import graph_capture_safe
        if not graph_capture_safe():
            warnings.warn("SegmentedTrainStep: HIP was initialised before `import fastvim_amd` could switch graph packet "
                          "capture off (DEBUG_CLR_GRAPH_PACKET_CAPTURE=0): on ROCm 7.2 some captured training steps replay "
                          "wrongly (DESIGN.md section 5) -- running this step EAGERLY instead.  Import fastvim_amd first, or "
                          "export the variable, to get graph replay.", RuntimeWarning, stacklevel=3)
            self.use_graph = False
            return
        snap = self._snapshot()
        side = torch.cuda.Stream()
        side.wait_stream(torch.cuda.current_stream())
        with torch.cuda.stream(side):
            for _ in range(warmup):
                self._eager_step()
        torch.cuda.current_stream().wait_stream(side)
        torch.cuda.synchronize()
        self._restore(snap)
        torch.cuda.synchronize()
        pool = torch.cuda.graph_pool_handle()
        mode = "thread_local" if (dist.is_available() and dist.is_initialized()) else "global"
        g_fwd = torch.cuda.CUDAGraph()
        with torch.cuda.graph(g_fwd, pool=pool, capture_error_mode=mode):
            self.loss = self._forward()
        g_bwd = []
        for k in range(self.K):
            g = torch.cuda.CUDAGraph()
            with torch.cuda.graph(g, pool=pool, capture_error_mode=mode):
                self._backward(k)
            g_bwd.append(g)
        g_opt = torch.cuda.CUDAGraph()
        with torch.cuda.graph(g_opt, pool=pool, capture_error_mode=mode):
            self.opt.step(grad_scale=self._gscale)
        self.graphs = (g_fwd, g_bwd, g_opt)

    def step(self, time_exposed=False):
        if not self.use_graph:
            self.loss = self._eager_step()
            return self.loss
        g_fwd, g_bwd, g_opt = self.graphs
        g_fwd.replay()
        for k in range(self.K):
            g_bwd[k].replay()
            self.exchange.launch(k)
        if time_exposed:
            e0, e1 = torch.cuda.Event(enable_timing=True), torch.cuda.Event(enable_timing=True)
            e0.record()
        self.exchange.finish(mean=False)
        if time_exposed:
            e1.record()
            self._exposed.append((e0, e1))
        g_opt.replay()
        return self.loss

    def exposed_ms(self):
        if not self._exposed:
            return None
        t = [a.elapsed_time(b) for a, b in self._exposed]
        self._exposed = []
        return sum(t) / len(t)
```

### include/fastvim_hip.h

```cpp
#ifndef FASTVIM_HIP_H
#define FASTVIM_HIP_H

#include <stddef.h>
#include <stdint.h>

#ifdef __cplusplus
extern "C" {
#endif

typedef void* fv_stream_t;

enum { FV_F32 = 0, FV_BF16 = 1, FV_F16 = 2 };
enum { FV_OK = 0, FV_ERR_INVALID = -1, FV_ERR_HIP = -2, FV_ERR_UNSUPPORTED = -3 };

const char* fv_last_error(void);
#define FV_ABI_VERSION 3
int fv_version(void);

int fv_selective_scan_fwd(const void* u, const void* delta, const float* A, const void* B,
                          const void* C, const float* D, const void* z, const float* delta_bias,
                          void* out, float* last_state, int batch, int dim, int seqlen, int dstate,
                          int n_groups, int B_variable, int C_variable, int delta_softplus,
                          int dtype, fv_stream_t stream);

size_t fv_selective_scan_bwd_workspace(int batch, int dim, int seqlen, int dstate, int n_groups,
                                       int B_variable, int C_variable);

int fv_selective_scan_bwd(const void* u, const void* delta, const float* A, const void* B,
                          const void* C, const float* D, const void* z, const float* delta_bias,
                          const void* dout, void* du, void* ddelta, float* dA, float* dB, float* dC,
                          float* dD, void* dz, float* ddelta_bias, void* workspace, int batch, int dim,
                          int seqlen, int dstate, int n_groups, int B_variable, int C_variable,
                          int delta_softplus, int dtype, fv_stream_t stream);

int fv_causal_conv1d_fwd(const void* x, const float* weight, const float* bias, void* y, int batch, int dim,
                         int seqlen, int width, int silu, int dtype, fv_stream_t stream);
int fv_causal_conv1d_bwd(const void* x, const float* weight, const float* bias, const void* dy, void* dx,
                         float* partials, int batch, int dim, int seqlen, int width, int silu, int dtype,
                         fv_stream_t stream);

int fv_scan_expand_skip_fwd(const void* yc, const void* u_full, const float* D, void* out, int batch, int dim,
                            int seqlen, int seqlen_compressed, int dtype, fv_stream_t stream);

int fv_mixer_conv_pool_fwd(const void* xz, const float* conv_w, const float* conv_b,
                           const float* conv_w_b, const float* conv_b_b, const float* D, const float* D_b,
                           void* xc, void* skip, void* amax, int batch, int rows, int cols, int tok_stride_row,
                           int tok_stride_col, int tokens_per_patch, int d_inner, int d_conv, int pool_max,
                           float scaling_factor, int dtype, fv_stream_t stream);

int fv_mixer_scan_fwd(const void* xc, const void* x_dbl, const float* dt_w, const float* dt_bias,
                      const float* A_log, const float* dt_w_b, const float* dt_bias_b,
                      const float* A_log_b, float* yc, int batch, int Lc, int d_inner, int dt_rank,
                      int d_state, int dtype, fv_stream_t stream);
size_t fv_mixer_scan_ckpt_floats(int batch, int Lc, int d_inner, int d_state, int dt_rank);
int fv_mixer_scan_fwd_ckpt(const void* xc, const void* x_dbl, const float* dt_w, const float* dt_bias,
                           const float* A_log, const float* dt_w_b, const float* dt_bias_b,
                           const float* A_log_b, float* yc, float* ckpt, int batch, int Lc, int d_inner, int dt_rank,
                           int d_state, int dtype, fv_stream_t stream);
int fv_mixer_scan_fwd_segments(int batch, int Lc, int d_inner, int dt_rank);
size_t fv_mixer_scan_fwd_seg_floats(int batch, int Lc, int d_inner, int d_state, int dt_rank);
int fv_mixer_scan_fwd_seg(const void* xc, const void* x_dbl, const float* dt_w, const float* dt_bias,
                          const float* A_log, const float* dt_w_b, const float* dt_bias_b, const float* A_log_b,
                          float* yc, float* ckpt, float* seg_ws, int batch, int Lc, int d_inner, int dt_rank,
                          int d_state, int dtype, fv_stream_t stream);

int fv_mixer_xproj_scan_fwd_ok(int Lc, int d_inner, int dt_rank, int dtype);
int fv_mixer_xproj_scan_fwd(const void* xc, const void* x_proj_w2, const float* dt_w, const float* dt_bias,
                            const float* A_log, const float* dt_w_b, const float* dt_bias_b, const float* A_log_b,
                            void* x_dbl, float* yc, int batch, int Lc, int d_inner, int dt_rank, int d_state,
                            int dtype, fv_stream_t stream);

int fv_mixer_combine_fwd(const void* xz, const void* skip, const float* yc, const float* ln_w,
                         const float* ln_b, float ln_eps, void* g, float* mean, float* rstd, int batch,
                         int rows, int cols, int tok_stride_row, int tok_stride_col, int tokens_per_patch,
                         int d_inner, int dtype, fv_stream_t stream);

int fv_mixer_bwd_blocks(int batch, int rows, int d_inner, int tokens_per_patch, int which);

int fv_mixer_combine_bwd(const void* dg, const void* xz, const void* skip, const float* yc,
                         const float* ln_w, const float* ln_b, const float* mean, const float* rstd,
                         void* dxz, void* d_o, float* dyc, float* partials, int batch, int rows, int cols, int tok_stride_row,
                         int tok_stride_col, int tokens_per_patch, int d_inner, int dtype, fv_stream_t stream);

int fv_mixer_scan_bwd_chunks(int d_inner, int Lc, int dt_rank);
int fv_mixer_scan_bwd_chunks_b(int batch, int d_inner, int Lc, int dt_rank);
int fv_mixer_scan_bwd_partials(int batch, int Lc, int dt_rank);
size_t fv_mixer_scan_bwd_ckpt_floats(int batch, int Lc, int d_inner, int d_state, int dt_rank);
int fv_mixer_scan_bwd(const void* xc, const void* x_dbl, const float* dt_w, const float* dt_bias,
                      const float* A_log, const float* dt_w_b, const float* dt_bias_b, const float* A_log_b,
                      const float* dyc, float* dxc, float* dx_dbl, float* ckpt, float* partials, int batch,
                      int Lc, int d_inner, int dt_rank, int d_state, int dtype, fv_stream_t stream);
int fv_mixer_scan_bwd_dir(const void* xc, const void* x_dbl, const float* dt_w, const float* dt_bias,
                          const float* A_log, const float* dt_w_b, const float* dt_bias_b, const float* A_log_b,
                          const float* dyc, int dyc_per_direction, float* dxc, float* dx_dbl, float* ckpt,
                          float* partials, int batch, int Lc, int d_inner, int dt_rank, int d_state, int dtype,
                          fv_stream_t stream);
int fv_mixer_scan_bwd_ckpt(const void* xc, const void* x_dbl, const float* dt_w, const float* dt_bias,
                           const float* A_log, const float* dt_w_b, const float* dt_bias_b, const float* A_log_b,
                           const float* dyc, int dyc_per_direction, float* dxc, float* dx_dbl, float* ckpt,
                           int ckpt_given, float* partials, int batch, int Lc, int d_inner, int dt_rank, int d_state,
                           int dtype, fv_stream_t stream);
int fv_mixer_scan_bwd_segments(int batch, int Lc, int d_inner, int dt_rank);
size_t fv_mixer_scan_bwd_seg_floats(int batch, int Lc, int d_inner, int d_state, int dt_rank);
int fv_mixer_scan_bwd_seg_partials(int batch, int Lc, int d_inner, int dt_rank);
int fv_mixer_scan_bwd_seg_chunks(int batch, int d_inner, int Lc, int dt_rank, int seg_ws_given);
int fv_mixer_scan_bwd_seg(const void* xc, const void* x_dbl, const float* dt_w, const float* dt_bias, const float* A_log,
                          const float* dt_w_b, const float* dt_bias_b, const float* A_log_b, const float* dyc,
                          int dyc_per_direction, float* dxc, float* dx_dbl, float* ckpt, int ckpt_given, float* partials,
                          float* seg_ws, int batch, int Lc, int d_inner, int dt_rank, int d_state, int dtype,
                          fv_stream_t stream);

int fv_mixer_scan_bwd_xproj_ok(int batch, int Lc, int d_inner, int dt_rank, int dtype);
int fv_mixer_scan_bwd_xproj(const void* xc, const void* x_dbl, const float* dt_w, const float* dt_bias, const float* A_log,
                            const float* dt_w_b, const float* dt_bias_b, const float* A_log_b, const float* dyc,
                            const float* x_proj_w, const float* x_proj_w_b, const void* x_proj_w2_bf16, float* dxc,
                            void* dxc2, float* dx_dbl, float* partials, int batch, int Lc, int d_inner, int dt_rank,
                            int d_state, int dtype, fv_stream_t stream);
int fv_chunk_rows_bf16(const float* const* partials, void* const* outs, int njobs, int nchunks, long rows, int width,
                       fv_stream_t stream);

int fv_rows_segment_sum(const void* in, int in_dtype, int in_per_direction, const int* idx, void* out, int out_dtype,
                        int batch, int n_tokens, int rows, int d_inner, float scale, fv_stream_t stream);
int fv_rows_gather(const void* in, int in_dtype, const int* idx, void* out, int out_dtype, int batch, int n_tokens,
                   int rows, int d_inner, float scale, fv_stream_t stream);

int fv_mixer_conv_pool_bwd(const void* xz, const void* d_o, const float* dxc, const float* conv_w,
                           const float* conv_b, const float* conv_w_b, const float* conv_b_b, const float* D,
                           const float* D_b, const void* amax, void* dxz, float* partials, int batch, int rows,
                           int cols, int tok_stride_row, int tok_stride_col, int tokens_per_patch, int d_inner,
                           int d_conv, int pool_max, float scaling_factor, int dtype, fv_stream_t stream);

int fv_mixer_conv_pool_bwd2_ok(int rows, int cols, int tokens_per_patch, int d_inner, int pool_max);
int fv_mixer_conv_pool_bwd2(const void* xz, const void* d_o, const float* dxc, const void* dxc2, const float* conv_w,
                            const float* conv_b, const float* conv_w_b, const float* conv_b_b, const float* D,
                            const float* D_b, const void* amax, void* dxz, float* partials, int batch, int rows,
                            int cols, int tok_stride_row, int tok_stride_col, int tokens_per_patch, int d_inner,
                            int d_conv, int pool_max, float scaling_factor, int dtype, fv_stream_t stream);

int fv_reduce_partials(const float* partials, float* out, int n_partials, size_t n, int accumulate,
                       fv_stream_t stream);
int fv_reduce_partials_multi(const float* const* partials, float* const* outs, const int* n_partials,
                             const size_t* ns, int njobs, int accumulate, fv_stream_t stream);

int fv_add_norm_blocks(int M);
int fv_add_norm_fwd(const void* x, int x_dtype, const void* residual, int residual_dtype,
                    const float* weight, const float* bias, const float* row_scale, int rows_per_scale,
                    void* y, int y_dtype, void* residual_out, int residual_out_dtype, float* mean,
                    float* rstd, int M, int N, float eps, int is_rms_norm, fv_stream_t stream);
int fv_add_norm_bwd(const void* dy, int dy_dtype, const void* dresidual_out, int dresidual_out_dtype,
                    const void* r, int r_dtype, const float* weight, const float* mean, const float* rstd,
                    const float* row_scale, int rows_per_scale, void* dx, int dx_dtype, void* dresidual_in,
                    int dresidual_in_dtype, float* partial_dw, float* partial_db, int M, int N,
                    int is_rms_norm, fv_stream_t stream);

int fv_gemm_bf16(const void* A, const void* B, void* C, const float* bias, int M, int N, int K, long lda,
                 long ldb, long ldc, int a_k_slow, int b_k_slow, int c_fp32, int splits, fv_stream_t stream);

int fv_gemm_f32(const void* A, int a_dtype, const void* B, int b_dtype, void* C, int c_dtype, const float* bias, int M,
                int N, int K, long lda, long ldb, long ldc, int a_k_slow, int b_k_slow, int batch, long strideA,
                long strideB, long strideC, fv_stream_t stream);

int fv_gemm_bf16_addnorm(const void* A, const void* W, const float* residual, const float* norm_weight,
                         const float* row_scale, int rows_per_scale, void* y, float* residual_out, float* rstd, int M,
                         int N, int K, long lda, long ldw, float eps, fv_stream_t stream);

int fv_gemm_bf16_dgrad_addnorm_blocks(int M);
int fv_gemm_bf16_dgrad_addnorm_bwd(const void* A, const void* W, const float* dresidual_out, const float* r,
                                   const float* rstd, const float* norm_weight, const float* row_scale,
                                   int rows_per_scale, void* dx, float* dresidual_in, float* partial_dw, int M, int N,
                                   int K, long lda, long ldw, fv_stream_t stream);

int fv_gemm_bf16_dgrad_addnorm_bwd2(const void* A, const void* W, const float* dresidual_out, const float* r,
                                    const float* rstd, const float* norm_weight, const float* row_scale,
                                    int rows_per_scale, void* dx, float* dresidual_in, float* partial_dw, int M, int N,
                                    int K, long lda, long ldw, const void* W2, void* C2, int N2, long ldw2,
                                    fv_stream_t stream);

int fv_mixer_combine_out_proj_addnorm_ok(int batch, int rows, int cols, int tokens_per_patch, int d_inner, int d_model,
                                         int dtype);
int fv_mixer_combine_out_proj_addnorm(const void* xz, const void* skip, const float* yc, const float* ln_w,
                                      const float* ln_b, float ln_eps, void* g, float* mean, float* rstd_ln, int batch,
                                      int rows, int cols, int tok_stride_row, int tok_stride_col, const void* W, long ldw,
                                      const float* residual, const float* norm_weight, const float* row_scale,
                                      int rows_per_scale, void* y, float* residual_out, float* rstd, float eps,
                                      fv_stream_t stream);

int fv_mixer_conv_pool_bwd_dgrad_ok(int batch, int rows, int cols, int tokens_per_patch, int d_inner, int d_model,
                                    int pool_max, int dtype);
int fv_mixer_conv_pool_bwd_dgrad_blocks(int batch, int rows);
int fv_mixer_conv_pool_bwd_dgrad(const void* xz, const void* dskip, const float* dxc, const void* dxc2,
                                 const float* conv_w, const float* conv_b, const float* conv_w_b, const float* conv_b_b,
                                 const float* D, const float* D_b, void* dxz, float* conv_partials, int batch, int rows,
                                 int cols, int tok_stride_row, int tok_stride_col, float scaling, const void* W_in_t,
                                 long ldwt, const float* dresidual_out, const float* r, const float* rstd,
                                 const float* norm_weight, const float* row_scale, int rows_per_scale, void* dx,
                                 float* dresidual_in, float* partial_dw, const void* W2, void* C2, int N2, long ldw2,
                                 fv_stream_t stream);

int fv_transpose_bf16_batched(const void* const* srcs, void* const* dsts, int njobs, int rows, int cols,
                              fv_stream_t stream);

int fv_gemm_bf16_addnorm2(const void* A, const void* W, const float* residual, const float* norm_weight,
                          const float* row_scale, int rows_per_scale, void* y, float* residual_out, float* rstd, int M,
                          int N, int K, long lda, long ldw, float eps, const void* W2, void* C2, int N2, long ldw2,
                          fv_stream_t stream);

int fv_gemm_bf16_tn_grouped(const void* const* x, const void* const* y, float* const* parts, const int* Kd,
                            const int* M, const int* N, const int* splits, int count, fv_stream_t stream);
int fv_gemm_bf16_tn_grouped_ld(const void* const* x, const void* const* y, float* const* parts, const int* Kd,
                               const int* M, const int* N, const int* ldx, const int* ldy, const int* splits, int count,
                               fv_stream_t stream);

int fv_gemm_bf16_tn_grouped_wide8(int M, int N, int Kd);

int fv_mixer_xproj_fwd(const void* xc, const void* x_proj_w2, void* x_dbl, int M, int d_inner, int width,
                       fv_stream_t stream);

int fv_mixer_xproj_bwd_slices(int M);
int fv_mixer_xproj_bwd(const float* dx_dbl_partials, int nchunks, const void* xc, const float* x_proj_w,
                       const float* x_proj_w_b, float* dxc, float* dW_partials, int M, int d_inner, int width,
                       int dtype, fv_stream_t stream);
int fv_mixer_xproj_bwd2(const float* dx_dbl_partials, int nchunks, const void* xc, const float* x_proj_w,
                        const float* x_proj_w_b, float* dxc, float* dW_partials, void* dx_dbl_bf16, int M, int d_inner,
                        int width, int dtype, fv_stream_t stream);
int fv_mixer_xproj_bwd3_ok(int M, int d_inner, int width, int dtype);
int fv_mixer_xproj_bwd3(const float* dx_dbl_partials, int nchunks, const void* xc, const float* x_proj_w,
                        const float* x_proj_w_b, const void* x_proj_w_t_bf16, float* dxc, void* dxc2_bf16,
                        void* dx_dbl_bf16, int M, int d_inner, int width, int dtype, fv_stream_t stream);

int fv_soft_target_ce(const void* logits, int logits_dtype, const float* target, float* loss_rows, float* loss,
                      float* dlogits, int batch, int classes, fv_stream_t stream);

int fv_patch_unfold(const void* img, int img_dtype, void* out, int out_dtype, int batch, int chans, int height,
                    int width, int ph, int pw, fv_stream_t stream);
int fv_gemm_bf16_rowbias(const void* A, const void* B, float* C, const float* table, int period, int M, int N, int K,
                         long lda, long ldb, long ldc, fv_stream_t stream);
int fv_mean_pool_fwd(const void* x, void* out, int batch, int tokens, int dim, int dtype, fv_stream_t stream);
int fv_mean_pool_bwd(const void* g, void* dx, int batch, int tokens, int dim, int dtype, fv_stream_t stream);
int fv_droppath_table(float* table, const float* keep, const float* inv_keep, int mods, int batch, fv_stream_t stream);
int fv_scale_cast(const float* x, const float* scale, void* y, int y_dtype, size_t n, fv_stream_t stream);
int fv_column_sum(const void* x, int dtype, float* out, int rows, int cols, int accumulate, fv_stream_t stream);

int fv_adamw_flat(float* params, const float* grads, float* exp_avg, float* exp_avg_sq, float* ema,
                  void* shadow_bf16, const uint8_t* decay_mask, const float* lr, float* step, float beta1,
                  float beta2, float eps, float weight_decay, float ema_decay, float grad_scale, size_t n,
                  fv_stream_t stream);

int fv_grad_sumsq_blocks(size_t n);
int fv_grad_sumsq_partials(const float* grads, float* partials, size_t n, fv_stream_t stream);
int fv_adamw_flat_groups(float* params, const float* grads, float* exp_avg, float* exp_avg_sq, float* ema,
                         void* shadow_bf16, const uint8_t* group_ids, const float* group_table, int n_groups,
                         const float* lr, float* step, const float* partials, int n_partials, const float* max_norm,
                         float* stats, int skip_nonfinite, float beta1, float beta2, float eps, float ema_decay,
                         float grad_scale, size_t n, fv_stream_t stream);

#ifdef __cplusplus
}
#endif
#endif
```

Baseline: 24900 images/sec.

## Pre-pack GEMM weights into MFMA fragment order for combine and conv-pool dgrad kernels

Adds a batched kernel that repacks the bf16 weight shadows (out_proj 192x384 and transposed in_proj 192x768) into per-wave, per-lane fragment order after each optimizer update. The fused combine/out_proj/addnorm and conv-pool dgrad kernels get packed variants that read each weight fragment as one contiguous 16-byte load per lane at a fixed offset, replacing strided row-pointer loads. The aim is coalesced weight fetches and fewer address registers in the inner GEMM loop. The cost is an extra pack pass each step, extra buffers, and cache invalidation of the derived shadows.

```diff
diff --git a/fastvim_amd/_lib.py b/fastvim_amd/_lib.py
--- a/fastvim_amd/_lib.py
+++ b/fastvim_amd/_lib.py
@@ -24,6 +24,7 @@
     "fv_column_sum", "fv_gemm_bf16_addnorm", "fv_gemm_bf16_dgrad_addnorm_blocks", "fv_gemm_bf16_dgrad_addnorm_bwd", "fv_gemm_bf16_dgrad_addnorm_bwd2", "fv_gemm_bf16_addnorm2", "fv_mixer_combine_out_proj_addnorm_ok", "fv_mixer_combine_out_proj_addnorm", "fv_gemm_f32",
     "fv_mixer_conv_pool_bwd_dgrad_ok", "fv_mixer_conv_pool_bwd_dgrad_blocks", "fv_mixer_conv_pool_bwd_dgrad", "fv_transpose_bf16_batched", "fv_gemm_bf16_tn_grouped_wide8",
     "fv_grad_sumsq_blocks", "fv_grad_sumsq_partials", "fv_adamw_flat_groups",
+    "fv_pack_weight_frags_batched", "fv_mixer_conv_pool_bwd_dgrad_pk", "fv_mixer_combine_out_proj_addnorm_pk",
 )
 
 
diff --git a/fastvim_amd/csrc/combine_gemm.hip b/fastvim_amd/csrc/combine_gemm.hip
--- a/fastvim_amd/csrc/combine_gemm.hip
+++ b/fastvim_amd/csrc/combine_gemm.hip
@@ -11,6 +11,9 @@
 constexpr int CG_RSB = CG_N * 2 + 16;
 constexpr int CG_PD = 6;
 constexpr int CG_KS = CG_K / 32;
+#ifndef CG_FORCE_PK
+#define CG_FORCE_PK 0
+#endif
 #ifndef CG_DBG
 #define CG_DBG 0
 #endif
@@ -41,6 +44,7 @@
 
 __device__ __forceinline__ float cg_hsum(f2 v) { return v.x + v.y; }
 
+template <bool PK>
 __global__ __launch_bounds__(CG_NT, 2) void combine_out_proj_addnorm_kernel(CgParams p) {
   extern __shared__ __attribute__((aligned(16))) char smem[];
   typedef PairVec<bf16_t, 3> P;
@@ -59,6 +63,12 @@
   const int fn = lane & 15, fk = lane >> 4;
   const bf16_t* wrow[3];
   cg_bf16x8 fb[CG_PD][3];
+  const char* wpk = reinterpret_cast<const char*>(p.W) + wv * (CG_KS * 3 * 1024);
+  const uint32_t wpk_lane = (uint32_t)lane * 16;
+  auto wfrag = [&](int nb, int ks) {
+    if constexpr (PK) return *reinterpret_cast<const cg_bf16x8*>(wpk + (ks * 3 + nb) * 1024 + wpk_lane);
+    else return *reinterpret_cast<const cg_bf16x8*>(wrow[nb] + ks * 32);
+  };
   float4 ne_r[2][2][3], ne_w[3];
   float ne_sc[2][2];
   {
@@ -114,13 +124,13 @@
     }
     __builtin_amdgcn_sched_barrier(0);
 #pragma unroll
-    for (int nb = 0; nb < 3; ++nb) wrow[nb] = p.W + (long)(wv * 48 + nb * 16 + fn) * p.ldw + fk * 8;
+    for (int nb = 0; nb < 3; ++nb) wrow[nb] = PK ? nullptr : p.W + (long)(wv * 48 + nb * 16 + fn) * p.ldw + fk * 8;
 #pragma unroll
     for (int s = 0; s < CG_PD; s += 2)
 #pragma unroll
       for (int nb = 0; nb < 3; ++nb)
 #pragma unroll
-        for (int h = 0; h < 2; ++h) fb[s + h][nb] = *reinterpret_cast<const cg_bf16x8*>(wrow[nb] + (s + h) * 32);
+        for (int h = 0; h < 2; ++h) fb[s + h][nb] = wfrag(nb, s + h);
     __builtin_amdgcn_sched_barrier(0);
 #pragma unroll
     for (int q = 0; q < 3; ++q) ysum[q] = ysf[q] + ysb[q];
@@ -233,7 +243,7 @@
       for (int nb = 0; nb < 3; ++nb)
 #pragma unroll
         for (int h = 0; h < 2; ++h)
-          fb[(kp + h) % CG_PD][nb] = *reinterpret_cast<const cg_bf16x8*>(wrow[nb] + (kp + h + CG_PD) * 32);
+          fb[(kp + h) % CG_PD][nb] = wfrag(nb, kp + h + CG_PD);
     }
     __builtin_amdgcn_sched_barrier(0);
 #pragma unroll
@@ -336,7 +346,7 @@
          cols > 0 && cols <= 16 && (long)batch * rows * cols * CG_K * 4 < 0x7fffffffL;
 }
 
-extern "C" int fv_mixer_combine_out_proj_addnorm(const void* xz, const void* skip, const float* yc, const float* ln_w,
+static int cg_launch(bool packed, const void* xz, const void* skip, const float* yc, const float* ln_w,
                                                  const float* ln_b, float ln_eps, void* g, float* mean, float* rstd_ln,
                                                  int batch, int rows, int cols, int tok_stride_row, int tok_stride_col,
                                                  const void* W, long ldw, const float* residual,
@@ -352,6 +362,7 @@
            "mixer_combine_out_proj_addnorm: token strides (%d,%d) are neither row-major nor transposed for a %dx%d grid",
            tok_stride_row, tok_stride_col, rows, cols);
   FV_CHECK(((uintptr_t)W & 15) == 0 && ldw % 8 == 0 && ldw >= CG_K, "mixer_combine_out_proj_addnorm: weight rows must be 16-byte aligned");
+  FV_CHECK(!packed || ldw == CG_K, "mixer_combine_out_proj_addnorm_pk: the packed weight has no row padding (ldw = %d)", CG_K);
   FV_CHECK(((uintptr_t)residual & 15) == 0 && ((uintptr_t)residual_out & 15) == 0 && ((uintptr_t)y & 7) == 0 &&
                ((uintptr_t)norm_weight & 15) == 0, "mixer_combine_out_proj_addnorm: row operands must be 16-byte aligned");
   FV_CHECK(!row_scale || rows_per_scale > 0, "mixer_combine_out_proj_addnorm: rows_per_scale must be positive");
@@ -365,7 +376,22 @@
   p.M = batch * rows * cols;
   p.d_in = CG_K;
   const size_t smem = (size_t)CG_BM * CG_RSA;
-  hipLaunchKernelGGL(combine_out_proj_addnorm_kernel, dim3(batch * fv_cdiv(rows, 4)), dim3(CG_NT), smem, (hipStream_t)stream, p);
+  const dim3 grid(batch * fv_cdiv(rows, 4)), block(CG_NT);
+  if (packed || CG_FORCE_PK) hipLaunchKernelGGL(combine_out_proj_addnorm_kernel<true>, grid, block, smem, (hipStream_t)stream, p);
+  else hipLaunchKernelGGL(combine_out_proj_addnorm_kernel<false>, grid, block, smem, (hipStream_t)stream, p);
   FV_LAUNCH_CHECK();
   return FV_OK;
 }
+
+#define CG_ARGS_DECL                                                                                                          \
+  const void *xz, const void *skip, const float *yc, const float *ln_w, const float *ln_b, float ln_eps, void *g,             \
+      float *mean, float *rstd_ln, int batch, int rows, int cols, int tok_stride_row, int tok_stride_col, const void *W,      \
+      long ldw, const float *residual, const float *norm_weight, const float *row_scale, int rows_per_scale, void *y,         \
+      float *residual_out, float *rstd, float eps, fv_stream_t stream
+#define CG_ARGS                                                                                                               \
+  xz, skip, yc, ln_w, ln_b, ln_eps, g, mean, rstd_ln, batch, rows, cols, tok_stride_row, tok_stride_col, W, ldw, residual,    \
+      norm_weight, row_scale, rows_per_scale, y, residual_out, rstd, eps, stream
+
+extern "C" int fv_mixer_combine_out_proj_addnorm(CG_ARGS_DECL) { return cg_launch(false, CG_ARGS); }
+
+extern "C" int fv_mixer_combine_out_proj_addnorm_pk(CG_ARGS_DECL) { return cg_launch(true, CG_ARGS); }
diff --git a/fastvim_amd/csrc/convpool_dgrad.hip b/fastvim_amd/csrc/convpool_dgrad.hip
--- a/fastvim_amd/csrc/convpool_dgrad.hip
+++ b/fastvim_amd/csrc/convpool_dgrad.hip
@@ -26,6 +26,9 @@
 constexpr int CD_SMEM = CD_O_S + 4 * 32 * (64 * 2 + 16);
 static_assert(CD_O_RING + 3 * CD_ZST <= CD_SMEM && CD_O_RING + 4 * CD_SLOT * 4 <= CD_SMEM, "LDS regions");
 static_assert(2 * CD_SMEM <= 160 * 1024, "two workgroups per CU");
+#ifndef CD_FORCE_PK
+#define CD_FORCE_PK 0
+#endif
 #ifndef CD_DBG
 #define CD_DBG 0
 #endif
@@ -71,7 +74,7 @@
 }
 static_assert(cd_younger(3) < 64 && cd_younger(4) < 64 && cd_younger(5) < 64, "vmcnt is a 6-bit counter");
 
-template <int NT, bool X2>
+template <int NT, bool X2, bool PK>
 __global__ __launch_bounds__(CD_NT, 2) void conv_pool_bwd_dgrad_kernel(CdParams p) {
   extern __shared__ __attribute__((aligned(16))) char smem[];
   typedef PairVec<bf16_t, 1> P;
@@ -267,7 +270,13 @@
   const bf16_t* wrow[3];
   bf16x8 fb[CD_PD][3];
 #pragma unroll
-  for (int nb = 0; nb < 3; ++nb) wrow[nb] = p.Wt + (long)(wv * 48 + nb * 16 + fn) * p.ldwt + fk * 8;
+  for (int nb = 0; nb < 3; ++nb) wrow[nb] = PK ? nullptr : p.Wt + (long)(wv * 48 + nb * 16 + fn) * p.ldwt + fk * 8;
+  const char* wpk = reinterpret_cast<const char*>(p.Wt) + wv * (CD_KS * 3 * 1024);
+  const uint32_t wpk_lane = (uint32_t)lane * 16;
+  auto wfrag = [&](int nb, int ks) {
+    if constexpr (PK) return *reinterpret_cast<const bf16x8*>(wpk + (ks * 3 + nb) * 1024 + wpk_lane);
+    else return *reinterpret_cast<const bf16x8*>(wrow[nb] + ks * 32);
+  };
   uint32_t zoff[2];
   const uint32_t ring = (uint32_t)(uintptr_t)(__attribute__((address_space(3))) const char*)(smem + CD_O_RING);
 #pragma unroll
@@ -289,7 +298,7 @@
 #pragma unroll
     for (int nb = 0; nb < 3; ++nb)
 #pragma unroll
-      for (int h = 0; h < 2; ++h) fb[s + h][nb] = *reinterpret_cast<const bf16x8*>(wrow[nb] + (s + h) * 32);
+      for (int h = 0; h < 2; ++h) fb[s + h][nb] = wfrag(nb, s + h);
   __builtin_amdgcn_sched_barrier(0);
   float4 ne_r[2][2][3];
 #pragma unroll
@@ -328,7 +337,7 @@
       for (int nb = 0; nb < 3; ++nb)
 #pragma unroll
         for (int h = 0; h < 2; ++h)
-          fb[(kp + h) % CD_PD][nb] = *reinterpret_cast<const bf16x8*>(wrow[nb] + (kp + h + CD_PD) * 32);
+          fb[(kp + h) % CD_PD][nb] = wfrag(nb, kp + h + CD_PD);
     }
     __builtin_amdgcn_sched_barrier(0);
 #pragma unroll
@@ -488,8 +497,8 @@
 
 extern "C" int fv_mixer_conv_pool_bwd_dgrad_blocks(int batch, int rows) { return batch * fv_cdiv(rows, 4); }
 
-extern "C" int fv_mixer_conv_pool_bwd_dgrad(
-    const void* xz, const void* dskip, const float* dxc, const void* dxc2, const float* conv_w, const float* conv_b,
+static int cd_launch(
+    bool packed, const void* xz, const void* dskip, const float* dxc, const void* dxc2, const float* conv_w, const float* conv_b,
     const float* conv_w_b, const float* conv_b_b, const float* D, const float* D_b, void* dxz, float* conv_partials, int batch,
     int rows, int cols, int tok_stride_row, int tok_stride_col, float scaling, const void* W_in_t, long ldwt,
     const float* dresidual_out, const float* r, const float* rstd, const float* norm_weight, const float* row_scale,
@@ -503,6 +512,7 @@
            "mixer_conv_pool_bwd_dgrad: token strides (%d,%d) are neither row-major nor transposed for a %dx%d grid",
            tok_stride_row, tok_stride_col, rows, cols);
   FV_CHECK(((uintptr_t)W_in_t & 15) == 0 && ldwt % 8 == 0 && ldwt >= CD_K, "mixer_conv_pool_bwd_dgrad: transposed weight rows must be 16-byte aligned");
+  FV_CHECK(!packed || ldwt == CD_K, "mixer_conv_pool_bwd_dgrad_pk: the packed weight has no row padding (ldwt = %d)", CD_K);
   FV_CHECK(((uintptr_t)r & 15) == 0 && ((uintptr_t)dresidual_in & 15) == 0 && ((uintptr_t)dx & 7) == 0 &&
                ((uintptr_t)norm_weight & 15) == 0 && ((uintptr_t)dresidual_out & 15) == 0 && ((uintptr_t)dxz & 15) == 0,
            "mixer_conv_pool_bwd_dgrad: row operands must be 16-byte aligned");
@@ -520,16 +530,34 @@
   p.dres_in = dresidual_in; p.pw = partial_dw; p.W2 = (const bf16_t*)W2; p.ldw2 = ldw2; p.C2 = (bf16_t*)C2; p.N2 = N2;
   p.M = batch * rows * cols;
   const dim3 grid(batch * fv_cdiv(rows, 4)), block(CD_NT);
-#define FV_CD(NTT, XX)                                                                                              \
+#define FV_CD(NTT, XX, PP)                                                                                          \
   do {                                                                                                              \
     static FvOncePerDevice done;                                                                                    \
     if (done.first())                                                                                               \
-      (void)hipFuncSetAttribute((const void*)conv_pool_bwd_dgrad_kernel<NTT, XX>, hipFuncAttributeMaxDynamicSharedMemorySize, CD_SMEM); \
-    hipLaunchKernelGGL((conv_pool_bwd_dgrad_kernel<NTT, XX>), grid, block, CD_SMEM, (hipStream_t)stream, p);        \
+      (void)hipFuncSetAttribute((const void*)conv_pool_bwd_dgrad_kernel<NTT, XX, PP>, hipFuncAttributeMaxDynamicSharedMemorySize, CD_SMEM); \
+    hipLaunchKernelGGL((conv_pool_bwd_dgrad_kernel<NTT, XX, PP>), grid, block, CD_SMEM, (hipStream_t)stream, p);    \
   } while (0)
-  if (cols == 14) { if (dxc2) FV_CD(14, true); else FV_CD(14, false); }
-  else { if (dxc2) FV_CD(16, true); else FV_CD(16, false); }
+#define FV_CD2(NTT, XX) do { if (packed || CD_FORCE_PK) FV_CD(NTT, XX, true); else FV_CD(NTT, XX, false); } while (0)
+  if (cols == 14) { if (dxc2) FV_CD2(14, true); else FV_CD2(14, false); }
+  else { if (dxc2) FV_CD2(16, true); else FV_CD2(16, false); }
+#undef FV_CD2
 #undef FV_CD
   FV_LAUNCH_CHECK();
   return FV_OK;
 }
+
+#define CD_ARGS_DECL                                                                                                          \
+  const void *xz, const void *dskip, const float *dxc, const void *dxc2, const float *conv_w, const float *conv_b,            \
+      const float *conv_w_b, const float *conv_b_b, const float *D, const float *D_b, void *dxz, float *conv_partials,        \
+      int batch, int rows, int cols, int tok_stride_row, int tok_stride_col, float scaling, const void *W_in_t, long ldwt,    \
+      const float *dresidual_out, const float *r, const float *rstd, const float *norm_weight, const float *row_scale,        \
+      int rows_per_scale, void *dx, float *dresidual_in, float *partial_dw, const void *W2, void *C2, int N2, long ldw2,      \
+      fv_stream_t stream
+#define CD_ARGS                                                                                                               \
+  xz, dskip, dxc, dxc2, conv_w, conv_b, conv_w_b, conv_b_b, D, D_b, dxz, conv_partials, batch, rows, cols, tok_stride_row,    \
+      tok_stride_col, scaling, W_in_t, ldwt, dresidual_out, r, rstd, norm_weight, row_scale, rows_per_scale, dx,              \
+      dresidual_in, partial_dw, W2, C2, N2, ldw2, stream
+
+extern "C" int fv_mixer_conv_pool_bwd_dgrad(CD_ARGS_DECL) { return cd_launch(false, CD_ARGS); }
+
+extern "C" int fv_mixer_conv_pool_bwd_dgrad_pk(CD_ARGS_DECL) { return cd_launch(true, CD_ARGS); }
diff --git a/fastvim_amd/csrc/glue.hip b/fastvim_amd/csrc/glue.hip
--- a/fastvim_amd/csrc/glue.hip
+++ b/fastvim_amd/csrc/glue.hip
@@ -174,6 +174,21 @@
   }
 }
 
+
+constexpr int PKW_ROWS = 192;
+struct PackJobs {
+  const uint4* src[TRJ_MAX];
+  uint4* dst[TRJ_MAX];
+  int ks_n;
+};
+__global__ __launch_bounds__(256) void pack_weight_frags_kernel(PackJobs J) {
+  const int u = blockIdx.x * 256 + threadIdx.x;
+  if (u >= PKW_ROWS * J.ks_n * 4) return;
+  const int lane = u & 63, t = u >> 6, nb = t % 3, ks = (t / 3) % J.ks_n, wv = t / (3 * J.ks_n);
+  const int row = 48 * wv + 16 * nb + (lane & 15), unit_in_row = 4 * ks + (lane >> 4);
+  J.dst[blockIdx.y][u] = J.src[blockIdx.y][row * (J.ks_n * 4) + unit_in_row];
+}
+
 }
 
 extern "C" int fv_patch_unfold(const void* img, int img_dtype, void* out, int out_dtype, int batch, int chans, int height,
@@ -273,3 +288,19 @@
   FV_LAUNCH_CHECK();
   return FV_OK;
 }
+
+extern "C" int fv_pack_weight_frags_batched(const void* const* srcs, void* const* dsts, int njobs, int K, fv_stream_t stream) {
+  FV_CHECK(srcs && dsts && njobs > 0 && njobs <= TRJ_MAX, "pack_weight_frags_batched: 1..%d jobs", TRJ_MAX);
+  FV_CHECK(K == 384 || K == 768, "pack_weight_frags_batched: K = %d is not a built reduction length (384, 768)", K);
+  PackJobs J{};
+  for (int j = 0; j < njobs; ++j) {
+    FV_CHECK(srcs[j] && dsts[j] && srcs[j] != dsts[j], "pack_weight_frags_batched: null or aliased pointer in job %d", j);
+    FV_CHECK(((uintptr_t)srcs[j] & 15) == 0 && ((uintptr_t)dsts[j] & 15) == 0, "pack_weight_frags_batched: job %d is not 16-byte aligned", j);
+    J.src[j] = (const uint4*)srcs[j];
+    J.dst[j] = (uint4*)dsts[j];
+  }
+  J.ks_n = K / 32;
+  hipLaunchKernelGGL(pack_weight_frags_kernel, dim3(fv_cdiv(PKW_ROWS * J.ks_n * 4, 256), njobs), dim3(256), 0, (hipStream_t)stream, J);
+  FV_LAUNCH_CHECK();
+  return FV_OK;
+}
diff --git a/fastvim_amd/flat.py b/fastvim_amd/flat.py
--- a/fastvim_amd/flat.py
+++ b/fastvim_amd/flat.py
@@ -21,12 +21,26 @@
 )
 
 
+def _drop_derived_shadows(model):
+    for p in model.parameters():
+        for a in ("_fv_shadow_t", "_fv_shadow_t_version", "_fv_shadow_pk", "_fv_shadow_pk_version"):
+            if hasattr(p, a):
+                delattr(p, a)
+    for mod in model.modules():
+        fv = mod.__dict__.get("_fv")
+        if isinstance(fv, dict):
+            fv.pop("Wx2_shadow_t", None)
+            fv.pop("Wx2_t_params", None)
+
+
 class FlatTrainingState:
     def __init__(self, model, shadow_dtype=torch.bfloat16, process_group=None, comm_dtype=None,
                  chunk_bytes=256 << 20):
         self.group = process_group
         self.comm_dtype = comm_dtype
         self.chunk = max(1, chunk_bytes // 4)
+        self._model = model
+        _drop_derived_shadows(model)
         named = dict(model.named_parameters())
         mixers = {mname: mod for mname, mod in model.named_modules() if isinstance(mod, Mamba)}
         units, unit_of = [], {}
@@ -126,6 +140,15 @@
                     self._t_src.append(w._fv_shadow)
                     self._t_dst.append(wt)
                     self._t_params.append(w)
+        self._pk_jobs = {768: ([], [], []), 384: ([], [], [])}
+        if shadow_dtype == torch.bfloat16 and dev.type == "cuda":
+            for w, wt in zip(self._t_params, self._t_dst):
+                self._add_packed(768, w, wt)
+            for mod in mixers.values():
+                w = getattr(getattr(mod, "out_proj", None), "weight", None)
+                if w is not None and tuple(w.shape) == (192, 384) and w.requires_grad and getattr(w, "_fv_shadow", None) is not None:
+                    self._add_packed(384, w, w._fv_shadow)
+        self._pk_dst = self._pk_jobs[768][1] + self._pk_jobs[384][1]
         self._tx_src, self._tx_dst, self._tx_params = [], [], []
         if shadow_dtype == torch.bfloat16 and dev.type == "cuda":
             for mod in mixers.values():
@@ -152,6 +175,15 @@
         group_wgrads(True)
         _SideStream.enabled = False
 
+    def _add_packed(self, K, w, src):
+        pk = torch.empty(192 * K, device=src.device, dtype=src.dtype)
+        w._fv_shadow_pk = pk
+        w._fv_shadow_pk_version = -1
+        srcs, dsts, params = self._pk_jobs[K]
+        srcs.append(src)
+        dsts.append(pk)
+        params.append(w)
+
     def close(self):
         if self._saved_switches is None:
             return
@@ -162,6 +194,7 @@
         _SideStream.enabled = s_
         self._hook.remove()
         self._saved_switches = None
+        _drop_derived_shadows(self._model)
 
     def __enter__(self):
         return self
@@ -194,13 +227,18 @@
         self.refresh_transposed()
 
     def refresh_transposed(self):
-        from .mixer_ops import transpose_bf16_batched
+        from .mixer_ops import pack_weight_frags, transpose_bf16_batched
         for src, dst, params in ((self._t_src, self._t_dst, self._t_params),
                                  (getattr(self, "_tx_src", []), getattr(self, "_tx_dst", []), getattr(self, "_tx_params", []))):
             if src:
                 transpose_bf16_batched(src, dst)
                 for p in params:
                     p._fv_shadow_t_version = p._version
+        for srcs, dsts, params in getattr(self, "_pk_jobs", {}).values():
+            if srcs:
+                pack_weight_frags(srcs, dsts)
+                for p in params:
+                    p._fv_shadow_pk_version = p._version
 
     @property
     def world_size(self):
diff --git a/fastvim_amd/mamba_simple_faster.py b/fastvim_amd/mamba_simple_faster.py
--- a/fastvim_amd/mamba_simple_faster.py
+++ b/fastvim_amd/mamba_simple_faster.py
@@ -30,6 +30,29 @@
             w._fv_shadow_t_version = w._version
         return wt
     return _shadow(w, cdt).t().contiguous()
+
+
+class _PackedWeights:
+    enabled = True
+
+
+def use_packed_weights(on):
+    was = _PackedWeights.enabled
+    _PackedWeights.enabled = bool(on)
+    return was
+
+
+def _shadow_pk(w, cdt, plain):
+    pk = getattr(w, "_fv_shadow_pk", None)
+    if pk is None or pk.dtype != cdt or not _PackedWeights.enabled:
+        return None
+    if w._version != w._fv_shadow_pk_version:
+        if not (plain.is_contiguous() and plain.numel() == pk.numel()):
+            return None
+        with torch.no_grad():
+            M.pack_weight_frags([plain], [pk])
+        w._fv_shadow_pk_version = w._version
+    return pk
 
 
 def _wx2_shadow_t(fv):
@@ -318,7 +341,8 @@
         if xz is None and W_out_c.stride(1) == 1 and W_out_c.stride(0) % 8 == 0 and W_out_c.data_ptr() % 16 == 0:
             y, res_out, rstd = M.combine_out_proj_addnorm(pack["xz"], pack["skip"], pack["yc"], pack["ln_w"], pack["ln_b"],
                                                           pack["eps"], pack["rows"], pack["cols"], pack["transposed"],
-                                                          pack["out"], W_out_c, res2, w32, row_scale, rows_per_scale, eps)
+                                                          pack["out"], W_out_c, res2, w32, row_scale, rows_per_scale, eps,
+                                                          W_out_pk=_shadow_pk(W_out, cdt, W_out_c))
             return y, res_out, rstd, w32, row_scale, rows_per_scale
         resolve_combine(pack)
     rc = lib.fv_gemm_bf16_addnorm2(
@@ -413,7 +437,7 @@
             W_in_t = _shadow_t(ctx.W_in, cdt)
             p2, dx, dres_in, pw, nb, dg_prev = M.conv_pool_bwd_dgrad(
                 xz, d_o, dxc, dxc2, cw2, cb, cwb2, cb_b, D, D_b, dxz, rows, cols, transposed, scaling, W_in_t, gg, r, rstd,
-                w32, row_scale, ctx.rows_per_scale, W2=W2, conv_grad_out=conv_grad_out)
+                w32, row_scale, ctx.rows_per_scale, W2=W2, conv_grad_out=conv_grad_out, W_in_pk=_shadow_pk(ctx.W_in, cdt, W_in_t))
             out.update(dx=dx, dres_in=dres_in, pw=pw, nb=nb, dg_prev=dg_prev)
             return p2
 
diff --git a/fastvim_amd/mixer_ops.py b/fastvim_amd/mixer_ops.py
--- a/fastvim_amd/mixer_ops.py
+++ b/fastvim_amd/mixer_ops.py
@@ -182,7 +182,7 @@
 
 
 def combine_out_proj_addnorm(xz, skip, yc, ln_w, ln_b, ln_eps, rows, cols, transposed, out, W_out_c, residual2, norm_w32,
-                             row_scale, rows_per_scale, eps):
+                             row_scale, rows_per_scale, eps, W_out_pk=None):
     B, Ltok, two_d = xz.shape
     d = W_out_c.shape[0]
     Mrows = B * Ltok
@@ -191,9 +191,14 @@
     y = torch.empty(Mrows, d, device=xz.device, dtype=torch.bfloat16)
     res_out = torch.empty(Mrows, d, device=xz.device, dtype=torch.float32)
     rstd = torch.empty(Mrows, device=xz.device, dtype=torch.float32)
-    rc = L.lib().fv_mixer_combine_out_proj_addnorm(
+    if W_out_pk is not None:
+        assert W_out_pk.dtype == torch.bfloat16 and W_out_pk.is_contiguous() and W_out_pk.numel() == d * (two_d // 2)
+        fn, W_arg, ldw = L.lib().fv_mixer_combine_out_proj_addnorm_pk, W_out_pk, two_d // 2
+    else:
+        fn, W_arg, ldw = L.lib().fv_mixer_combine_out_proj_addnorm, W_out_c, W_out_c.stride(0)
+    rc = fn(
         L.ptr(xz), L.ptr(skip), L.ptr(yc), L.ptr(ln_w), L.ptr(ln_b), f32(ln_eps), L.ptr(g), L.ptr(mean), L.ptr(rstd_ln),
-        L.i32(B), L.i32(rows), L.i32(cols), L.i32(s_i), L.i32(s_j), L.ptr(W_out_c), ctypes.c_long(W_out_c.stride(0)),
+        L.i32(B), L.i32(rows), L.i32(cols), L.i32(s_i), L.i32(s_j), L.ptr(W_arg), ctypes.c_long(ldw),
         L.ptr(residual2), L.ptr(norm_w32), L.ptr(row_scale), L.i32(rows_per_scale), L.ptr(y), L.ptr(res_out), L.ptr(rstd),
         f32(eps), L.stream_of(xz))
     L.check(rc, "mixer_combine_out_proj_addnorm")
@@ -334,7 +339,8 @@
 
 
 def conv_pool_bwd_dgrad(xz, d_o, dxc, dxc2, conv_w, conv_b, conv_w_b, conv_b_b, D, D_b, dxz, rows, cols, transposed, scaling,
-                        W_in_t, dres_out, r, rstd, norm_w32, row_scale, rows_per_scale, W2=None, conv_grad_out=None):
+                        W_in_t, dres_out, r, rstd, norm_w32, row_scale, rows_per_scale, W2=None, conv_grad_out=None,
+                        W_in_pk=None):
     B, Ltok, two_d = xz.shape
     d_in = two_d // 2
     d = W_in_t.shape[0]
@@ -351,10 +357,15 @@
     dg_prev = torch.empty(Mrows, N2, device=dev, dtype=torch.bfloat16) if W2 is not None else None
     assert dxc2 is None or (dxc2.dtype == xz.dtype and dxc2.shape == dxc.shape and dxc2.is_contiguous())
     assert W_in_t.dtype == torch.bfloat16 and W_in_t.stride(1) == 1 and W_in_t.shape[1] == two_d
-    rc = lib.fv_mixer_conv_pool_bwd_dgrad(
+    if W_in_pk is not None:
+        assert W_in_pk.dtype == torch.bfloat16 and W_in_pk.is_contiguous() and W_in_pk.numel() == d * two_d
+        fn, W_arg, ldwt = lib.fv_mixer_conv_pool_bwd_dgrad_pk, W_in_pk, two_d
+    else:
+        fn, W_arg, ldwt = lib.fv_mixer_conv_pool_bwd_dgrad, W_in_t, W_in_t.stride(0)
+    rc = fn(
         L.ptr(xz), L.ptr(d_o), L.ptr(dxc), L.ptr(dxc2), L.ptr(conv_w), L.ptr(conv_b), L.ptr(conv_w_b), L.ptr(conv_b_b),
         L.ptr(D), L.ptr(D_b), L.ptr(dxz), L.ptr(part), L.i32(B), L.i32(rows), L.i32(cols), L.i32(s_i), L.i32(s_j),
-        f32(scaling), L.ptr(W_in_t), ctypes.c_long(W_in_t.stride(0)), L.ptr(dres_out), L.ptr(r), L.ptr(rstd), L.ptr(norm_w32),
+        f32(scaling), L.ptr(W_arg), ctypes.c_long(ldwt), L.ptr(dres_out), L.ptr(r), L.ptr(rstd), L.ptr(norm_w32),
         L.ptr(row_scale), L.i32(rows_per_scale), L.ptr(dx), L.ptr(dres_in), L.ptr(pw), L.ptr(W2), L.ptr(dg_prev), L.i32(N2),
         ctypes.c_long(W2.stride(0) if W2 is not None else 0), L.stream_of(xz))
     L.check(rc, "mixer_conv_pool_bwd_dgrad")
@@ -377,6 +388,40 @@
         ins = (ctypes.c_void_p * k)(*[t.data_ptr() for t in a])
         outs = (ctypes.c_void_p * k)(*[t.data_ptr() for t in b])
         L.check(lib.fv_transpose_bf16_batched(ins, outs, L.i32(k), L.i32(rows), L.i32(cols), L.stream_of(a[0])), "transpose_bf16_batched")
+
+
+PACK_ROWS = 192
+
+
+def pack_index(K):
+    assert K % 32 == 0
+    KS = K // 32
+    u = torch.arange(PACK_ROWS * K // 8)
+    lane, t = u % 64, u // 64
+    nb, ks, wv = t % 3, (t // 3) % KS, t // (3 * KS)
+    return torch.stack([48 * wv + 16 * nb + (lane % 16), 32 * ks + 8 * (lane // 16)], dim=1)
+
+
+def pack_weight_frags_ref(W):
+    rows, K = W.shape
+    assert rows == PACK_ROWS
+    idx = pack_index(K).to(W.device)
+    cols = idx[:, 1:2] + torch.arange(8, device=W.device)
+    return W[idx[:, 0:1], cols].reshape(rows, K)
+
+
+def pack_weight_frags(srcs, dsts):
+    lib = L.lib()
+    rows, K = srcs[0].shape
+    for lo in range(0, len(srcs), 64):
+        a, b = srcs[lo:lo + 64], dsts[lo:lo + 64]
+        assert all(t.dtype == torch.bfloat16 and t.is_contiguous() and tuple(t.shape) == (rows, K) for t in a)
+        assert all(t.dtype == torch.bfloat16 and t.is_contiguous() and t.numel() == rows * K for t in b)
+        assert rows == PACK_ROWS
+        k = len(a)
+        ins = (ctypes.c_void_p * k)(*[t.data_ptr() for t in a])
+        outs = (ctypes.c_void_p * k)(*[t.data_ptr() for t in b])
+        L.check(lib.fv_pack_weight_frags_batched(ins, outs, L.i32(k), L.i32(K), L.stream_of(a[0])), "pack_weight_frags_batched")
 
 
 XPROJ_WIDTHS = (44, 56, 80, 96, 112, 34, 36, 38, 64)
diff --git a/fastvim_amd/pipeline.py b/fastvim_amd/pipeline.py
--- a/fastvim_amd/pipeline.py
+++ b/fastvim_amd/pipeline.py
@@ -79,7 +79,7 @@
 
     def _snapshot(self):
         f, o = self.flat, self.opt
-        bufs = [f.param_flat, f.shadow_flat] + list(getattr(f, "_t_dst", [])) + list(getattr(f, "_tx_dst", []))
+        bufs = [f.param_flat, f.shadow_flat] + list(getattr(f, "_t_dst", [])) + list(getattr(f, "_tx_dst", [])) + list(getattr(f, "_pk_dst", []))
         for v in vars(o).values():
             if torch.is_tensor(v) and v.is_cuda and all(v is not b for b in bufs):
                 bufs.append(v)
diff --git a/include/fastvim_hip.h b/include/fastvim_hip.h
--- a/include/fastvim_hip.h
+++ b/include/fastvim_hip.h
@@ -184,6 +184,12 @@
                                       const float* residual, const float* norm_weight, const float* row_scale,
                                       int rows_per_scale, void* y, float* residual_out, float* rstd, float eps,
                                       fv_stream_t stream);
+int fv_mixer_combine_out_proj_addnorm_pk(const void* xz, const void* skip, const float* yc, const float* ln_w,
+                                         const float* ln_b, float ln_eps, void* g, float* mean, float* rstd_ln, int batch,
+                                         int rows, int cols, int tok_stride_row, int tok_stride_col, const void* W,
+                                         long ldw, const float* residual, const float* norm_weight,
+                                         const float* row_scale, int rows_per_scale, void* y, float* residual_out,
+                                         float* rstd, float eps, fv_stream_t stream);
 
 int fv_mixer_conv_pool_bwd_dgrad_ok(int batch, int rows, int cols, int tokens_per_patch, int d_inner, int d_model,
                                     int pool_max, int dtype);
@@ -196,9 +202,20 @@
                                  const float* norm_weight, const float* row_scale, int rows_per_scale, void* dx,
                                  float* dresidual_in, float* partial_dw, const void* W2, void* C2, int N2, long ldw2,
                                  fv_stream_t stream);
+int fv_mixer_conv_pool_bwd_dgrad_pk(const void* xz, const void* dskip, const float* dxc, const void* dxc2,
+                                    const float* conv_w, const float* conv_b, const float* conv_w_b,
+                                    const float* conv_b_b, const float* D, const float* D_b, void* dxz,
+                                    float* conv_partials, int batch, int rows, int cols, int tok_stride_row,
+                                    int tok_stride_col, float scaling, const void* W_in_t, long ldwt,
+                                    const float* dresidual_out, const float* r, const float* rstd,
+                                    const float* norm_weight, const float* row_scale, int rows_per_scale, void* dx,
+                                    float* dresidual_in, float* partial_dw, const void* W2, void* C2, int N2, long ldw2,
+                                    fv_stream_t stream);
 
 int fv_transpose_bf16_batched(const void* const* srcs, void* const* dsts, int njobs, int rows, int cols,
                               fv_stream_t stream);
+
+int fv_pack_weight_frags_batched(const void* const* srcs, void* const* dsts, int njobs, int K, fv_stream_t stream);
 
 int fv_gemm_bf16_addnorm2(const void* A, const void* W, const float* residual, const float* norm_weight,
                           const float* row_scale, int rows_per_scale, void* y, float* residual_out, float* rstd, int M,
```

Result: faster. 25990 images/sec, median of 6 (+4.4%).
